# bowang-lab/BioReason

Measured on AMD Instinct MI355X. Metric: GRPO samples/sec (NT-500M+Qwen3-1.7B, DNA 2x1024, prompt 2180, gen 256), higher is better.
Workload: dtype bf16

## Files before the change

### bioreason_amd/csrc/k_gemm.hip

```cpp
#include <type_traits>

#include "bra_device.h"
#include "bra_api_internal.h"

namespace bra {

enum : int {
    EPI_BF16 = 0,
    EPI_F32 = 1,
    EPI_LSE = 2,
    EPI_DLOGIT = 3,
    EPI_ATOMIC = 4,
    EPI_SWIGLU = 5,
};

struct GemmArgs {
    const bf16_t* A;  long lda;
    const bf16_t* B;  long ldb;
    const bf16_t* A2; long lda2;
    const bf16_t* B2; long ldb2;
    void* C;          long ldc;
    int M, N, K, K2;
    float alpha;
    const bf16_t* bias;
    const bf16_t* res;
    long ldres;
    int accumulate;
    int split_k;
    const int* tgt;
    float* part_max;
    float* part_sum;
    float* tgt_logit;
    const float* lse;
    const float* coef;
    int nchunk;
    int swiglu_F;
};

template <int BK>
__device__ __forceinline__ int swz_chunk(int row, int c) {
    return BK == 64 ? (c ^ (row & 7)) : (c ^ ((row >> 2) & 3));
}

#ifdef BRA_EMU
__device__ __forceinline__ void epi_pin(u32x2&) {}
#else
__device__ __forceinline__ void epi_pin(u32x2& v) { asm volatile("" : "+v"(v)); }
#endif
template <bool BIAS>
__device__ __forceinline__ float epi_scale_bias(float a, float alpha, float b) {
    float t = a * alpha;
    if (BIAS) {
#ifndef BRA_EMU
        asm volatile("" : "+v"(t));
#endif
        t = t + b;
    }
    return t;
}
template <int MI, bool BIAS>
__device__ __forceinline__ void epi_bf16_interior_b(const GemmArgs& g, f32x4 (&acc)[4][MI], int mw0, int nw0, int lane) {
    const int fr = lane & 15, fq = lane >> 4;
    const float alpha = g.alpha;
    const int col = nw0 + 4 * fq;
    bf16_t* cp = (bf16_t*)g.C + ((long)(mw0 + fr) * g.ldc + col);
    const long cstep = 16 * g.ldc;
    float bz[4][4];
#pragma unroll
    for (int ni = 0; ni < 4; ++ni)
#pragma unroll
        for (int r = 0; r < 4; ++r) bz[ni][r] = 0.f;
    if (BIAS) {
#pragma unroll
        for (int ni = 0; ni < 4; ++ni) {
            const u32x2 b = ld8(g.bias + col + 16 * ni);
            bz[ni][0] = bf_lo(b.x); bz[ni][1] = bf_hi(b.x); bz[ni][2] = bf_lo(b.y); bz[ni][3] = bf_hi(b.y);
        }
    }
    if (g.res) {
        const bf16_t* rp = g.res + ((long)(mw0 + fr) * g.ldres + col);
        const long rstep = 16 * g.ldres;
        u32x2 rv[MI][4];
#pragma unroll
        for (int mi = 0; mi < MI; ++mi)
#pragma unroll
            for (int ni = 0; ni < 4; ++ni) rv[mi][ni] = ld8(rp + mi * rstep + ni * 16);
#pragma unroll
        for (int mi = 0; mi < MI; ++mi)
#pragma unroll
            for (int ni = 0; ni < 4; ++ni) epi_pin(rv[mi][ni]);
// ... 284 lines not shown
            const bool full = (n + 3 < g.N);
            if (EPI == EPI_BF16 || EPI == EPI_DLOGIT) {
                if (EPI == EPI_BF16) {
                    if (g.bias) {
#pragma unroll
                        for (int r = 0; r < 4; ++r) if (n + r < g.N) v[r] += bf2f(g.bias[n + r]);
                    }
                    if (g.res) {
                        if (full && !(g.ldres & 3)) {
                            const u32x2 rv = ld8(g.res + (long)m * g.ldres + n);
                            v[0] = round_bf(v[0]) + bf_lo(rv.x); v[1] = round_bf(v[1]) + bf_hi(rv.x);
                            v[2] = round_bf(v[2]) + bf_lo(rv.y); v[3] = round_bf(v[3]) + bf_hi(rv.y);
                        } else {
                            for (int r = 0; r < 4; ++r)
                                if (n + r < g.N) v[r] = round_bf(v[r]) + bf2f(g.res[(long)m * g.ldres + n + r]);
                        }
                    }
                } else {
#pragma unroll
                    for (int r = 0; r < 4; ++r) {
                        float p = __expf(round_bf(v[r]) - lse_m);
                        v[r] = coef_m * (((n + r) == tgt_m ? 1.f : 0.f) - p);
                    }
                }
                bf16_t* cp = (bf16_t*)g.C + (long)m * g.ldc + n;
                if (full) {
                    u32x2 o; o.x = pack_bf2(v[0], v[1]); o.y = pack_bf2(v[2], v[3]);
                    st8(cp, o);
                } else {
                    for (int r = 0; r < 4; ++r) if (n + r < g.N) cp[r] = f2bf(v[r]);
                }
            } else if (EPI == EPI_F32) {
                float* cp = (float*)g.C + (long)m * g.ldc + n;
                if (g.bias) {
#pragma unroll
                    for (int r = 0; r < 4; ++r) if (n + r < g.N) v[r] += bf2f(g.bias[n + r]);
                }
                if (full) {
                    f32x4 o = {v[0], v[1], v[2], v[3]};
                    if (g.accumulate) o += *reinterpret_cast<const f32x4*>(cp);
                    *reinterpret_cast<f32x4*>(cp) = o;
                } else {
                    for (int r = 0; r < 4; ++r)
                        if (n + r < g.N) cp[r] = g.accumulate ? cp[r] + v[r] : v[r];
                }
            } else {
                float* cp = (float*)g.C + (long)m * g.ldc + n;
                for (int r = 0; r < 4; ++r) if (n + r < g.N) atomicAdd(cp + r, v[r]);
            }
        }
    }
}

template <int BM, int BK, int EPI, int PF>
__global__ __launch_bounds__(BM * 2) void gemm_nt_kernel(GemmArgs g) {
    constexpr int BN = 128, NT = BM * 2;
    constexpr int CH = BK / 8;
    constexpr int LPTA = (BM * CH) / NT;
    constexpr int LPTB = (BN * CH) / NT;
    constexpr int A_BYTES = BM * BK * 2, B_BYTES = BN * BK * 2, STAGE = A_BYTES + B_BYTES;
    BRA_DYN_SMEM(smem);

    const int tid = (int)threadIdx.x;
    const int lane = tid & 63, wave = tid >> 6;
    const int wm = wave >> 1, wn = wave & 1;

    const int tiles_m = (g.M + BM - 1) / BM, tiles_n = (g.N + BN - 1) / BN;
    const int ntiles = tiles_m * tiles_n;
    int bid = (int)blockIdx.x;
    int kslice = 0;
    if (EPI == EPI_ATOMIC) { kslice = bid / ntiles; bid -= kslice * ntiles; }
    bid = (int)xcd_remap((unsigned)bid, (unsigned)ntiles);
    constexpr int GROUP = 8;
    const int per_group = GROUP * tiles_n;
    const int gid = bid / per_group;
    const int first_m = gid * GROUP;
    const int gsize = (tiles_m - first_m) < GROUP ? (tiles_m - first_m) : GROUP;
    const int tile_m = first_m + (bid % per_group) % gsize;
    const int tile_n = (bid % per_group) / gsize;
    const int m0 = tile_m * BM, n0 = tile_n * BN;

    const int nk1 = g.K / BK, nk2 = g.K2 / BK;
    int kt_begin = 0, kt_end = nk1 + nk2;
    if (EPI == EPI_ATOMIC && g.split_k > 1) {
        int per = (kt_end + g.split_k - 1) / g.split_k;
        kt_begin = kslice * per;
        kt_end = kt_begin + per < kt_end ? kt_begin + per : kt_end;
        if (kt_begin >= kt_end) return;
    }

    u32x4 ra[PF][LPTA], rb[PF][LPTB];

    auto issue_loads = [&](auto S, int kt) {
        constexpr int s = decltype(S)::value;
        const bf16_t* Ap; const bf16_t* Bp; long la, lb; int k0;
        if (kt < nk1) { Ap = g.A; Bp = g.B; la = g.lda; lb = g.ldb; k0 = kt * BK; }
        else { Ap = g.A2; Bp = g.B2; la = g.lda2; lb = g.ldb2; k0 = (kt - nk1) * BK; }
#pragma unroll
        for (int i = 0; i < LPTA; ++i) {
            const int q = tid + NT * i;
            int rm = m0 + q / CH; rm = rm < g.M ? rm : g.M - 1;
            ra[s][i] = ld16(Ap + (long)rm * la + k0 + (q % CH) * 8);
        }
#pragma unroll
        for (int i = 0; i < LPTB; ++i) {
            const int q = tid + NT * i;
            int rn = n0 + q / CH; rn = rn < g.N ? rn : g.N - 1;
            rb[s][i] = ld16(Bp + (long)rn * lb + k0 + (q % CH) * 8);
        }
    };
    auto write_lds = [&](auto S, int buf) {
        constexpr int s = decltype(S)::value;
        char* sa = smem + buf * STAGE;
        char* sb = sa + A_BYTES;
#pragma unroll
        for (int i = 0; i < LPTA; ++i) {
            const int q = tid + NT * i;
            st16(sa + (q / CH) * (BK * 2) + swz_chunk<BK>(q / CH, q % CH) * 16, ra[s][i]);
        }
#pragma unroll
        for (int i = 0; i < LPTB; ++i) {
            const int q = tid + NT * i;
            st16(sb + (q / CH) * (BK * 2) + swz_chunk<BK>(q / CH, q % CH) * 16, rb[s][i]);
        }
    };

    f32x4 acc[4][4];
#pragma unroll
    for (int i = 0; i < 4; ++i)
#pragma unroll
        for (int j = 0; j < 4; ++j) acc[i][j] = f32x4{0.f, 0.f, 0.f, 0.f};

    const int fr = lane & 15, fq = lane >> 4;
    auto compute = [&](int buf) {
        const char* sa = smem + buf * STAGE;
        const char* sb = sa + A_BYTES;
#pragma unroll
        for (int kk = 0; kk < BK / 32; ++kk) {
            u32x4 fa[4], fb[4];
            const int c = kk * 4 + fq;
#pragma unroll
            for (int i = 0; i < 4; ++i) {
                int rowa = wm * 64 + i * 16 + fr;
                int rowb = wn * 64 + i * 16 + fr;
                fa[i] = ld16(sa + rowa * (BK * 2) + swz_chunk<BK>(rowa, c) * 16);
                fb[i] = ld16(sb + rowb * (BK * 2) + swz_chunk<BK>(rowb, c) * 16);
            }
#pragma unroll
            for (int ni = 0; ni < 4; ++ni)
#pragma unroll
                for (int mi = 0; mi < 4; ++mi) acc[ni][mi] = mfma_16x16x32(fb[ni], fa[mi], acc[ni][mi]);
        }
    };
    using S0 = std::integral_constant<int, 0>;
    using S1 = std::integral_constant<int, PF - 1>;
    if (PF == 1) {
        issue_loads(S0{}, kt_begin);
        write_lds(S0{}, 0);
        __syncthreads();
        for (int kt = kt_begin; kt < kt_end; ++kt) {
            const int buf = (kt - kt_begin) & 1;
            const bool more = (kt + 1 < kt_end);
            if (more) issue_loads(S0{}, kt + 1);
            compute(buf);
            if (more) write_lds(S0{}, buf ^ 1);
            __syncthreads();
        }
    } else {
        issue_loads(S0{}, kt_begin);
        if (kt_begin + 1 < kt_end) issue_loads(S1{}, kt_begin + 1);
        write_lds(S0{}, 0);
        __syncthreads();
        for (int kt = kt_begin; kt < kt_end; kt += 2) {
            if (kt + 2 < kt_end) issue_loads(S0{}, kt + 2);
            compute(0);
            if (kt + 1 < kt_end) write_lds(S1{}, 1);
            __syncthreads();
            if (kt + 1 < kt_end) {
                if (kt + 3 < kt_end) issue_loads(S1{}, kt + 3);
                compute(1);
                if (kt + 2 < kt_end) write_lds(S0{}, 0);
                __syncthreads();
            }
        }
    }

    gemm_epilogue<EPI>(g, acc, m0, n0, wm, wn, lane, tile_n);
}

template <int EPI, int SKEW, int MI = 4>
__global__ __launch_bounds__(512, 2) void gemm_glds_kernel(GemmArgs g) {
    constexpr int BM = 64 * MI, BN = 128, BK = 64;
    constexpr int A_BYTES = BM * BK * 2, B_BYTES = BN * BK * 2, STAGE = A_BYTES + B_BYTES;
    BRA_DYN_SMEM(smem);
    const int tid = (int)threadIdx.x;
    const int lane = tid & 63, wave = uniform_i(tid >> 6);
    const int wm = wave >> 1, wn = wave & 1;

    const int tiles_m = (g.M + BM - 1) / BM, tiles_n = (g.N + BN - 1) / BN;
    const int ntiles = tiles_m * tiles_n;
    int bid = (int)blockIdx.x;
    int kslice = 0;
    if (EPI == EPI_ATOMIC) { kslice = bid / ntiles; bid -= kslice * ntiles; }
    bid = (int)xcd_remap((unsigned)bid, (unsigned)ntiles);
    constexpr int GROUP = 8;
    const int per_group = GROUP * tiles_n;
    const int gid = bid / per_group;
    const int first_m = gid * GROUP;
    const int gsize = (tiles_m - first_m) < GROUP ? (tiles_m - first_m) : GROUP;
    const int tile_m = first_m + (bid % per_group) % gsize;
    const int tile_n = (bid % per_group) / gsize;
    const int m0 = tile_m * BM, n0 = tile_n * BN;

    const int nk1 = g.K / BK, nk2 = g.K2 / BK;
    int kt_begin = 0, kt_end = nk1 + nk2;
    if (EPI == EPI_ATOMIC && g.split_k > 1) {
        int per = (kt_end + g.split_k - 1) / g.split_k;
        kt_begin = kslice * per;
        kt_end = kt_begin + per < kt_end ? kt_begin + per : kt_end;
        if (kt_begin >= kt_end) return;
    }
    const int nt = kt_end - kt_begin;

    const int prow = lane >> 3, lchunk = ((lane & 7) ^ (lane >> 3)) * 8;
    int rowA[MI], rowB[2];
#pragma unroll
    for (int j = 0; j < MI; ++j) { int r = m0 + wave * (8 * MI) + j * 8 + prow; rowA[j] = r < g.M ? r : g.M - 1; }
#pragma unroll
    for (int j = 0; j < 2; ++j) { int r = n0 + wave * 16 + j * 8 + prow; rowB[j] = r < g.N ? r : g.N - 1; }
    auto issue = [&](int kt, int stage) {
        char* sa = smem + stage * STAGE + wave * (8 * MI * 128);
        char* sb = smem + stage * STAGE + A_BYTES + wave * (16 * 128);
        const bool main = kt < nk1;
        const bf16_t* Ap = (main ? g.A : g.A2) + (long)(main ? kt : kt - nk1) * BK + lchunk;
        const bf16_t* Bp = (main ? g.B : g.B2) + (long)(main ? kt : kt - nk1) * BK + lchunk;
        const long la = main ? g.lda : g.lda2, lb = main ? g.ldb : g.ldb2;
#pragma unroll
        for (int j = 0; j < MI; ++j) glds16(Ap + (long)rowA[j] * la, sa + j * 1024);
#pragma unroll
        for (int j = 0; j < 2; ++j) glds16(Bp + (long)rowB[j] * lb, sb + j * 1024);
    };
    constexpr int NDMA = MI + 2;

    f32x4 acc[4][MI];
#pragma unroll
    for (int i = 0; i < 4; ++i)
#pragma unroll
        for (int j = 0; j < MI; ++j) acc[i][j] = f32x4{0.f, 0.f, 0.f, 0.f};
    const int fr = lane & 15, fq = lane >> 4;
    auto compute = [&](int stage) {
        const char* sa = smem + stage * STAGE;
        const char* sb = sa + A_BYTES;
#pragma unroll
        for (int kk = 0; kk < BK / 32; ++kk) {
            u32x4 fa[MI], fb[4];
            const int c = kk * 4 + fq;
#pragma unroll
            for (int i = 0; i < MI; ++i) {
                int rowa = wm * (16 * MI) + i * 16 + fr;
                fa[i] = ld16(sa + rowa * 128 + swz_chunk<64>(rowa, c) * 16);
            }
#pragma unroll
            for (int i = 0; i < 4; ++i) {
                int rowb = wn * 64 + i * 16 + fr;
                fb[i] = ld16(sb + rowb * 128 + swz_chunk<64>(rowb, c) * 16);
            }
#pragma unroll
            for (int ni = 0; ni < 4; ++ni)
#pragma unroll
                for (int mi = 0; mi < MI; ++mi) acc[ni][mi] = mfma_16x16x32(fb[ni], fa[mi], acc[ni][mi]);
        }
    };

    issue(kt_begin, 0);
    if (nt > 1) { issue(kt_begin + 1, 1); wait_vmcnt<NDMA>(); } else { wait_vmcnt<0>(); }
    raw_barrier();
    int stage = 0;
    if (!SKEW) {
        for (int t = 0; t < nt; ++t) {
            int s2 = stage + 2; s2 = s2 >= 3 ? s2 - 3 : s2;
            const bool ahead = t + 2 < nt;
            if (ahead) issue(kt_begin + t + 2, s2);
            compute(stage);
            if (ahead) wait_vmcnt<NDMA>(); else wait_vmcnt<0>();
            raw_barrier();
            stage = stage + 1 == 3 ? 0 : stage + 1;
        }
    } else {
        auto read_frags = [&](int stg, int kk, u32x4 (&fa)[MI], u32x4 (&fb)[4]) {
            const char* sa = smem + stg * STAGE;
            const char* sb = sa + A_BYTES;
// ... 125 lines not shown
    int stage = 0;
    u32x4 fa[MI][2], fb0[2][2], fb1[2][2];
    read_a(0, fa);
    read_b(0, 0, fb0);
    for (int t = 0; t < nt; ++t) {
        int s2 = stage + 2; s2 = s2 >= 3 ? s2 - 3 : s2;
        const int s1 = stage + 1 == 3 ? 0 : stage + 1;
        const bool ahead = t + 2 < nt;
        if (ahead) issue(t + 2, s2);
        read_b(stage, 1, fb1);
        mma(0, fa, fb0);
        mma(1, fa, fb1);
        if (ahead) wait_vmcnt<NDMA>(); else wait_vmcnt<0>();
        raw_barrier();
        if (t + 1 < nt) { read_a(s1, fa); read_b(s1, 0, fb0); }
        stage = s1;
    }
    const int mw0 = m0 + wm * (16 * MI), nw0 = n0 + wn * 64;
    float sm[MI];
#pragma unroll
    for (int mi = 0; mi < MI; ++mi) { const int m = mw0 + mi * 16 + fr; sm[mi] = g8.sa[m < g.M ? m : g.M - 1]; }
#pragma unroll
    for (int ni = 0; ni < 4; ++ni) {
        float sn[4];
#pragma unroll
        for (int r = 0; r < 4; ++r) { const int n = nw0 + ni * 16 + 4 * fq + r; sn[r] = g8.sb[n < g.N ? n : g.N - 1]; }
#pragma unroll
        for (int mi = 0; mi < MI; ++mi)
#pragma unroll
            for (int r = 0; r < 4; ++r) acc[ni][mi][r] *= sm[mi] * sn[r];
    }
    gemm_epilogue_w<EPI, MI>(g, acc, mw0, nw0, lane, smem + wave * (16 * MI * EPI_RS));
}

template <int ND, int NR, int NM>
__device__ __forceinline__ void sched_pipe() {
#ifndef BRA_EMU
    static_assert(ND + NR <= NM, "one memory instruction per MFMA gap");
#pragma unroll
    for (int i = 0; i < ND; ++i) {
        __builtin_amdgcn_sched_group_barrier(0x8, 1, 0);
        __builtin_amdgcn_sched_group_barrier(0x20, 1, 0);
        __builtin_amdgcn_sched_group_barrier(0x2, 2, 0);
    }
#pragma unroll
    for (int i = 0; i < NR; ++i) {
        __builtin_amdgcn_sched_group_barrier(0x8, 1, 0);
        __builtin_amdgcn_sched_group_barrier(0x100, 1, 0);
    }
    if constexpr (NM - ND - NR > 0) __builtin_amdgcn_sched_group_barrier(0x8, NM - ND - NR, 0);
#endif
}

template <int EPI, int WM, int WN>
__global__ __launch_bounds__(256) void gemm_w4_kernel(GemmArgs g) {
    static_assert(WN % 4 == 0, "the wave epilogue works on 64-column groups");
    constexpr int BM = 32 * WM, BN = 32 * WN, BK = 64;
    constexpr int A_BYTES = BM * BK * 2, STAGE = (BM + BN) * BK * 2;
    constexpr int NS = (160 * 1024) / STAGE >= 4 ? 4 : 3, LOOK = NS - 1;
    constexpr int NDMA = WM + WN;
    BRA_DYN_SMEM(smem);
    const int tid = (int)threadIdx.x;
    const int lane = tid & 63, wave = uniform_i(tid >> 6);
    const int wm = wave >> 1, wn = wave & 1;

    const int tiles_m = (g.M + BM - 1) / BM, tiles_n = (g.N + BN - 1) / BN;
    const int ntiles = tiles_m * tiles_n;
    int bid = (int)xcd_remap(blockIdx.x, (unsigned)ntiles);
    constexpr int GROUP = 8;
    const int per_group = GROUP * tiles_n;
    const int gid = bid / per_group;
    const int first_m = gid * GROUP;
    const int gsize = (tiles_m - first_m) < GROUP ? (tiles_m - first_m) : GROUP;
    const int tile_m = first_m + (bid % per_group) % gsize;
    const int tile_n = (bid % per_group) / gsize;
    const int m0 = tile_m * BM, n0 = tile_n * BN;

    const int nk1 = g.K / BK, nk2 = g.K2 / BK;
    const int nt = nk1 + nk2;

    const int prow = lane >> 3, lchunk = ((lane & 7) ^ (lane >> 3)) * 8;
    const bf16_t* src[NDMA];
    auto src_init = [&](bool main) {
#pragma unroll
        for (int j = 0; j < NDMA; ++j) {
            const int r = (wave * NDMA + j) * 8 + prow;
            if (r < BM) { int m = m0 + r; m = m < g.M ? m : g.M - 1; src[j] = (main ? g.A : g.A2) + (long)m * (main ? g.lda : g.lda2) + lchunk; }
            else { int n = n0 + r - BM; n = n < g.N ? n : g.N - 1; src[j] = (main ? g.B : g.B2) + (long)n * (main ? g.ldb : g.ldb2) + lchunk; }
        }
    };
    src_init(nk1 > 0);
    auto issue = [&](int kt, int stage) {
        if (kt == nk1 && kt > 0) src_init(false);
        char* dst = smem + stage * STAGE + wave * (NDMA * 1024);
#pragma unroll
        for (int j = 0; j < NDMA; ++j) { glds16(src[j], dst + j * 1024); src[j] += BK; }
    };
    auto wait_tiles = [&](int fly) {
        if (fly >= 2 && LOOK >= 3) wait_vmcnt<2 * NDMA>();
        else if (fly >= 1) wait_vmcnt<NDMA>();
        else wait_vmcnt<0>();
    };

    f32x4 acc[WN][WM];
#pragma unroll
    for (int i = 0; i < WN; ++i)
#pragma unroll
        for (int j = 0; j < WM; ++j) acc[i][j] = f32x4{0.f, 0.f, 0.f, 0.f};
    const int fr = lane & 15, fq = lane >> 4;
    auto read_frags = [&](int stg, int kk, u32x4 (&fa)[WM], u32x4 (&fb)[WN]) {
        const char* sa = smem + stg * STAGE;
        const char* sb = sa + A_BYTES;
        const int c = kk * 4 + fq;
#pragma unroll
        for (int i = 0; i < WM; ++i) {
            const int rowa = wm * (16 * WM) + i * 16 + fr;
            fa[i] = ld16(sa + rowa * 128 + swz_chunk<64>(rowa, c) * 16);
        }
#pragma unroll
        for (int i = 0; i < WN; ++i) {
            const int rowb = wn * (16 * WN) + i * 16 + fr;
            fb[i] = ld16(sb + rowb * 128 + swz_chunk<64>(rowb, c) * 16);
        }
    };
    auto mma = [&](const u32x4 (&fa)[WM], const u32x4 (&fb)[WN]) {
#pragma unroll
        for (int ni = 0; ni < WN; ++ni)
#pragma unroll
            for (int mi = 0; mi < WM; ++mi) acc[ni][mi] = mfma_16x16x32(fb[ni], fa[mi], acc[ni][mi]);
    };

#pragma unroll
    for (int j = 0; j < LOOK; ++j)
        if (j < nt) issue(j, j);
    wait_tiles((nt < LOOK ? nt : LOOK) - 1);
    raw_barrier();
    u32x4 fa0[WM], fb0[WN], fa1[WM], fb1[WN];
    read_frags(0, 0, fa0, fb0);
    int stage = 0;
    auto body = [&](int t, auto ISSUE) {
// ... 17 lines not shown
        sched_fence();
        if (t + 1 < nt) read_frags(s1, 0, fa0, fb0);
        mma(fa1, fb1);
        sched_pipe<0, NDMA, WM * WN>();
        sched_fence();
        stage = s1;
    };
    int t = 0;
    for (; t + LOOK < nt; ++t) body(t, std::true_type{});
    for (; t < nt; ++t) body(t, std::false_type{});
    auto epi_group = [&](auto HC) {
        constexpr int hcol = decltype(HC)::value;
        gemm_epilogue_w<EPI, WM>(g, *reinterpret_cast<f32x4 (*)[4][WM]>(&acc[4 * hcol]), m0 + wm * (16 * WM), n0 + wn * (16 * WN) + 64 * hcol, lane,
                                 smem + wave * (16 * WM * EPI_RS));
    };
    epi_group(std::integral_constant<int, 0>{});
    if constexpr (WN / 4 > 1) epi_group(std::integral_constant<int, 1>{});
    static_assert(WN / 4 <= 2, "two 64-column groups per wave at most");
}

constexpr int SWG_RS = 80;
__device__ __forceinline__ float silu_epi(float x) { return x / (1.f + __expf(-x)); }
__device__ __forceinline__ void ring_epilogue_swiglu(const GemmArgs& g, f32x4 (&acc)[4][8], int mw0, int f0, int lane, char* lw) {
    const int fr = lane & 15, fq = lane >> 4;
    const float alpha = g.alpha;
    char* wp = lw + fr * SWG_RS + 8 * fq;
#pragma unroll
    for (int mi = 0; mi < 8; ++mi)
#pragma unroll
        for (int j = 0; j < 2; ++j) {
            float v[4];
#pragma unroll
            for (int r = 0; r < 4; ++r) {
                const float gb = round_bf(acc[2 * j][mi][r] * alpha), ub = round_bf(acc[2 * j + 1][mi][r] * alpha);
                v[r] = round_bf(silu_epi(gb)) * ub;
            }
            u32x2 o; o.x = pack_bf2(v[0], v[1]); o.y = pack_bf2(v[2], v[3]);
            st8(wp + mi * (16 * SWG_RS) + j * 32, o);
        }
    wave_lds_sync();
    sched_fence();
    const int rrow = lane >> 2, rch = lane & 3;
    const char* rdp = lw + rrow * SWG_RS + 16 * rch;
    bf16_t* cp = (bf16_t*)g.C + ((long)(mw0 + rrow) * g.ldc + f0 + 8 * rch);
    const long cstep = 16 * g.ldc;
    const bool full = mw0 + 128 <= g.M;
#pragma unroll
    for (int jj = 0; jj < 8; ++jj) {
        const u32x4 xv = ld16(rdp + jj * (16 * SWG_RS));
        if (full || mw0 + rrow + 16 * jj < g.M) st16(cp + jj * cstep, xv);
    }
}

template <int EPI, int PH2 = 0>
__global__ __launch_bounds__(512, 2) void gemm_ring_kernel(GemmArgs g) {
    constexpr int BM = 256, BN = 256, BK = 64, HALF = 128 * BK * 2, NSLOT = 10;
    BRA_DYN_SMEM(smem);
    const int tid = (int)threadIdx.x;
    const int lane = tid & 63, wave = uniform_i(tid >> 6);
    const int wr = wave >> 2, wc = wave & 3;

    const int tiles_m = (g.M + BM - 1) / BM, tiles_n = (g.N + BN - 1) / BN;
    const int ntiles = tiles_m * tiles_n;
    int bid = (int)blockIdx.x;
    int kslice = 0;
    if (EPI == EPI_ATOMIC) { kslice = bid / ntiles; bid -= kslice * ntiles; }
    bid = (int)xcd_remap((unsigned)bid, (unsigned)ntiles);
    constexpr int GROUP = 8;
    const int per_group = GROUP * tiles_n;
    const int gid = bid / per_group;
    const int first_m = gid * GROUP;
    const int gsize = (tiles_m - first_m) < GROUP ? (tiles_m - first_m) : GROUP;
    const int tile_m = first_m + (bid % per_group) % gsize;
    const int tile_n = (bid % per_group) / gsize;
    const int m0 = tile_m * BM, n0 = tile_n * BN;

    const int nk1 = g.K / BK, nk2 = g.K2 / BK;
    int kt_begin = 0, kt_end = nk1 + nk2;
    if (EPI == EPI_ATOMIC && g.split_k > 1) {
        int per = (kt_end + g.split_k - 1) / g.split_k;
        kt_begin = kslice * per;
        kt_end = kt_begin + per < kt_end ? kt_begin + per : kt_end;
        if (kt_begin >= kt_end) return;
    }
    const int nt = kt_end - kt_begin;
    const int nstream = 4 * nt;

    const int prow = lane >> 3, lchunk = ((lane & 7) ^ (lane >> 3)) * 8;
    int rowB[4], rowA[4];
#pragma unroll
    for (int i = 0; i < 4; ++i) {
        const int loc = (i >> 1) * 128 + wave * 16 + (i & 1) * 8 + prow;
        int rb = n0 + loc;
        if (EPI == EPI_SWIGLU) rb = tile_n * 128 + (loc >> 5) * 16 + (loc & 15) + ((loc & 16) ? g.swiglu_F : 0);
        rowB[i] = rb < g.N ? rb : g.N - 1;
        int ra = m0 + loc; rowA[i] = ra < g.M ? ra : g.M - 1;
    }
    const bf16_t* src[8];
    auto src_init = [&](int h, int kt) {
        const bool main = kt < nk1;
        const long kcol = (long)(main ? kt : kt - nk1) * BK + lchunk;
#pragma unroll
        for (int pc = 0; pc < 2; ++pc) {
            if (h < 2) src[h * 2 + pc] = (main ? g.B : g.B2) + kcol + (long)rowB[h * 2 + pc] * (main ? g.ldb : g.ldb2);
            else src[h * 2 + pc] = (main ? g.A : g.A2) + kcol + (long)rowA[(h - 2) * 2 + pc] * (main ? g.lda : g.lda2);
        }
    };
#pragma unroll
    for (int h = 0; h < 4; ++h) src_init(h, kt_begin);
    auto issue = [&](int tt, auto H, int slot) {
        constexpr int h = decltype(H)::value;
        if (tt >= nt) return;
        if (kt_begin + tt == nk1 && tt > 0) src_init(h, nk1);
        char* dst = smem + slot * HALF + wave * 2048;
        glds16(src[h * 2], dst);
        glds16(src[h * 2 + 1], dst + 1024);
        src[h * 2] += BK;
        src[h * 2 + 1] += BK;
    };
    auto wrap = [&](int sl) { return sl >= NSLOT ? sl - NSLOT : sl; };
    auto wait_phase = [&](int gph) {
        const int fly = nstream - 5 - gph;
        if (fly >= 3) wait_vmcnt<6>(); else if (fly == 2) wait_vmcnt<4>(); else if (fly == 1) wait_vmcnt<2>(); else wait_vmcnt<0>();
    };

    f32x4 acc[4][8];
#pragma unroll
    for (int i = 0; i < 4; ++i)
#pragma unroll
        for (int j = 0; j < 8; ++j) acc[i][j] = f32x4{0.f, 0.f, 0.f, 0.f};
    const int fr = lane & 15, fq = lane >> 4;
    const int sw0 = ((fq ^ (fr & 7)) * 16), sw1 = (((4 + fq) ^ (fr & 7)) * 16);
    const int offA = fr * 128;
    const int offB = ((wc & 1) * 64 + fr) * 128;
    u32x4 fa[4][2], fb[2][2][2];
    auto read_a = [&](int slotA, int s) {
        const char* base = smem + slotA * HALF + offA + s * (64 * 128);
#pragma unroll
        for (int i = 0; i < 4; ++i) { fa[i][0] = ld16(base + i * 2048 + sw0); fa[i][1] = ld16(base + i * 2048 + sw1); }
    };
    auto read_b = [&](int slotB, auto S) {
        constexpr int s = decltype(S)::value;
        const char* base = smem + slotB * HALF + offB + s * (32 * 128);
#pragma unroll
        for (int i = 0; i < 2; ++i) { fb[s][i][0] = ld16(base + i * 2048 + sw0); fb[s][i][1] = ld16(base + i * 2048 + sw1); }
    };
    auto mma = [&](auto SA, auto SB) {
        constexpr int sa = decltype(SA)::value, sb = decltype(SB)::value;
        setprio(1);
#pragma unroll
        for (int kk = 0; kk < 2; ++kk)
#pragma unroll
            for (int ib = 0; ib < 2; ++ib)
#pragma unroll
                for (int ia = 0; ia < 4; ++ia)
                    acc[sb * 2 + ib][sa * 4 + ia] = mfma_16x16x32(fb[sb][ib][kk], fa[ia][kk], acc[sb * 2 + ib][sa * 4 + ia]);
        setprio(0);
    };
// ... 20 lines not shown
            issue(t + 1, I2{}, wrap(rb2 + 6)); issue(t + 1, I3{}, wrap(rb2 + 7)); wait2(gp); ++gp;
            sched_fence(); bare_barrier(); wait_lds(); sched_fence();
            mma(I0{}, I0{}); mma(I0{}, I1{});
            sched_fence(); bare_barrier();
            read_a(sA, 1);
            issue(t + 2, I0{}, wrap(rb2 + 8)); issue(t + 2, I1{}, wrap(rb2 + 9)); wait2(gp); ++gp;
            sched_fence(); bare_barrier(); wait_lds(); sched_fence();
            mma(I1{}, I1{}); mma(I1{}, I0{});
            sched_fence(); bare_barrier();
            rb2 = rb2 + 4 >= NSLOT ? rb2 + 4 - NSLOT : rb2 + 4;
        }
        if (wr == 0) bare_barrier();
        if constexpr (EPI == EPI_SWIGLU) ring_epilogue_swiglu(g, acc, m0 + wr * 128, tile_n * 128 + wc * 32, lane, smem + wave * (128 * SWG_RS));
        else gemm_epilogue_w<EPI, 8>(g, acc, m0 + wr * 128, n0 + wc * 64, lane, smem + wave * (128 * EPI_RS));
        return;
    }
    issue(0, I0{}, 0); issue(0, I1{}, 1); issue(0, I2{}, 2); issue(0, I3{}, 3);
    issue(1, I0{}, 4); issue(1, I1{}, 5); issue(1, I2{}, 6);
    wait_phase(-1);
    bare_barrier();
    if (wr == 1) bare_barrier();
    int rbase = 0;
    int gph = 0;
#pragma unroll 1
    for (int t = 0; t < nt; ++t) {
        const int sB = wrap(rbase + (wc >> 1)), sA = wrap(rbase + 2 + wr);
        read_b(sB, I0{}); sched_fence(); read_a(sA, 0);
        issue(t + 1, I3{}, wrap(rbase + 7)); wait_phase(gph); ++gph;
        sched_fence(); bare_barrier(); wait_lds(); sched_fence();
        mma(I0{}, I0{});
        sched_fence(); bare_barrier();
        read_b(sB, I1{});
        issue(t + 2, I0{}, wrap(rbase + 8)); wait_phase(gph); ++gph;
        sched_fence(); bare_barrier(); wait_lds(); sched_fence();
        mma(I0{}, I1{});
        sched_fence(); bare_barrier();
        read_a(sA, 1);
        issue(t + 2, I1{}, wrap(rbase + 9)); wait_phase(gph); ++gph;
        sched_fence(); bare_barrier(); wait_lds(); sched_fence();
        mma(I1{}, I1{});
        sched_fence(); bare_barrier();
        issue(t + 2, I2{}, rbase); wait_phase(gph); ++gph;
        sched_fence(); bare_barrier(); sched_fence();
        mma(I1{}, I0{});
        sched_fence(); bare_barrier();
        rbase = rbase + 4 >= NSLOT ? rbase + 4 - NSLOT : rbase + 4;
    }
    if (wr == 0) bare_barrier();

    if constexpr (EPI == EPI_SWIGLU) ring_epilogue_swiglu(g, acc, m0 + wr * 128, tile_n * 128 + wc * 32, lane, smem + wave * (128 * SWG_RS));
    else gemm_epilogue_w<EPI, 8>(g, acc, m0 + wr * 128, n0 + wc * 64, lane, smem + wave * (128 * EPI_RS));
}

template <int OUTF32>
__global__ __launch_bounds__(256) void gemm_skinny_kernel(GemmArgs g) {
    __shared__ float red[4][64][4];
    const int tid = (int)threadIdx.x, lane = tid & 63, wave = tid >> 6;
    const int fr = lane & 15, fq = lane >> 4;
    const int n0 = (int)blockIdx.x * 16;
    int rn = n0 + fr; rn = rn < g.N ? rn : g.N - 1;
    int rm = fr < g.M ? fr : g.M - 1;
    f32x4 acc = {0.f, 0.f, 0.f, 0.f};
    {
        const bf16_t* wp = g.B + (long)rn * g.ldb + fq * 8;
        const bf16_t* xp = g.A + (long)rm * g.lda + fq * 8;
        const int nk = g.K / 32;
        int kt = wave;
        for (; kt + 28 < nk; kt += 32) {
            u32x4 w[8], x[8];
#pragma unroll
            for (int u = 0; u < 8; ++u) { w[u] = ld16(wp + (long)(kt + 4 * u) * 32); x[u] = ld16(xp + (long)(kt + 4 * u) * 32); }
#pragma unroll
            for (int u = 0; u < 8; ++u) acc = mfma_16x16x32(w[u], x[u], acc);
        }
        for (; kt < nk; kt += 4) acc = mfma_16x16x32(ld16(wp + (long)kt * 32), ld16(xp + (long)kt * 32), acc);
    }
    if (g.K2 > 0) {
        const bf16_t* wp = g.B2 + (long)rn * g.ldb2 + fq * 8;
        const bf16_t* xp = g.A2 + (long)rm * g.lda2 + fq * 8;
        const int nk = g.K2 / 32;
        for (int kt = wave; kt < nk; kt += 4) acc = mfma_16x16x32(ld16(wp + (long)kt * 32), ld16(xp + (long)kt * 32), acc);
    }
#pragma unroll
    for (int r = 0; r < 4; ++r) red[wave][lane][r] = acc[r];
    __syncthreads();
    if (wave != 0) return;
    float v[4];
#pragma unroll
    for (int r = 0; r < 4; ++r) v[r] = (red[0][lane][r] + red[1][lane][r] + red[2][lane][r] + red[3][lane][r]) * g.alpha;
    const int m = fr, n = n0 + 4 * fq;
    if (m >= g.M || n >= g.N) return;
    if (g.bias) {
#pragma unroll
        for (int r = 0; r < 4; ++r) if (n + r < g.N) v[r] += bf2f(g.bias[n + r]);
    }
    if (OUTF32) {
        float* cp = (float*)g.C + (long)m * g.ldc + n;
        for (int r = 0; r < 4; ++r) if (n + r < g.N) cp[r] = g.accumulate ? cp[r] + v[r] : v[r];
    } else {
        if (g.res) {
#pragma unroll
            for (int r = 0; r < 4; ++r) if (n + r < g.N) v[r] = round_bf(v[r]) + bf2f(g.res[(long)m * g.ldres + n + r]);
        }
        bf16_t* cp = (bf16_t*)g.C + (long)m * g.ldc + n;
        if (n + 3 < g.N) { u32x2 o; o.x = pack_bf2(v[0], v[1]); o.y = pack_bf2(v[2], v[3]); st8(cp, o); }
        else for (int r = 0; r < 4; ++r) if (n + r < g.N) cp[r] = f2bf(v[r]);
    }
}

static int launch_skinny(const GemmArgs& g, int out_f32, bra_stream_t stream) {
    const int grid = (g.N + 15) / 16;
    if (out_f32) BRA_LAUNCH((gemm_skinny_kernel<1>), dim3(grid), dim3(256), 0, stream, g);
    else BRA_LAUNCH((gemm_skinny_kernel<0>), dim3(grid), dim3(256), 0, stream, g);
    return BRA_LAUNCH_STATUS();
}

#ifdef BRA_EMU
template <typename T> struct knob_t { T v; explicit knob_t(T x) : v(x) {} operator T() const { return v; } knob_t& operator=(T x) { v = x; return *this; } };
#else
template <typename T> struct knob_t {
    std::atomic<T> v;
    explicit knob_t(T x) : v(x) {}
    operator T() const { return v.load(std::memory_order_relaxed); }
    knob_t& operator=(T x) { v.store(x, std::memory_order_relaxed); return *this; }
};
#endif
static knob_t<int> g_forced_variant(-1);
static knob_t<int> g_forced_w4(0);
static knob_t<int> ring_min_fill_pct(60);
static knob_t<int> ring_two_phase(1);
static knob_t<int> ring_row_split(1);

static int pick_variant(const GemmArgs& g) {
    { const int fv = g_forced_variant; if (fv >= 0) return fv >= 6 ? 6 : fv; }
    const long tiles256 = (long)((g.M + 255) / 256) * ((g.N + 127) / 128) * (g.split_k > 1 ? g.split_k : 1);
    if (g.K % 64 == 0 && g.K2 % 64 == 0 && g.split_k <= 1) {
        const long t = (long)((g.M + 255) / 256) * ((g.N + 255) / 256);
        const long rounds = (t + 255) / 256;
        if (t >= 140 && (t <= 256 || 100 * t >= ring_min_fill_pct * rounds * 256)) return 6;
    }
    if (g.K % 64 == 0 && g.K2 % 64 == 0 && tiles256 >= 128) return 5;
    const long tiles128 = (long)((g.M + 127) / 128) * ((g.N + 127) / 128) * (g.split_k > 1 ? g.split_k : 1);
    if (g.K % 64 == 0 && g.K2 % 64 == 0 && tiles128 >= 128) return 5;
    return 0;
}

template <int BM, int BK, int EPI, int PF>
static int launch_gemm_v(const GemmArgs& g, bra_stream_t stream) {
    const int tiles = ((g.M + BM - 1) / BM) * ((g.N + 127) / 128);
    int grid = tiles;
    if (EPI == EPI_ATOMIC) grid = tiles * (g.split_k > 0 ? g.split_k : 1);
    const size_t smem = 2 * (size_t)(BM + 128) * BK * 2;
    BRA_ALLOW_SMEM((gemm_nt_kernel<BM, BK, EPI, PF>), smem);
    BRA_LAUNCH((gemm_nt_kernel<BM, BK, EPI, PF>), dim3(grid), dim3(BM * 2), smem, stream, g);
    return BRA_LAUNCH_STATUS();
}

static knob_t<int> g_forced_glds_rows(0);
static int pick_glds_rows(const GemmArgs& g) {
    { const int fr = g_forced_glds_rows; if (fr) return fr; }
    if (g_forced_variant >= 0) return 256;
    const long tn = (g.N + 127) / 128, sk = g.split_k > 1 ? g.split_k : 1;
    const int bms[3] = {256, 192, 128};
    const double eff[3] = {1.0, 0.95, 0.86};
    int best = 256;
    double best_cost = 1e30;
    for (int i = 0; i < 3; ++i) {
        const long t = ((g.M + bms[i] - 1) / bms[i]) * tn * sk;
        const double cost = (double)((t + 255) / 256) * bms[i] / eff[i];
        if (cost < best_cost * 0.97) { best_cost = cost; best = bms[i]; }
    }
    return best;
}

template <int EPI, int MI>
static int launch_glds_mi(const GemmArgs& g, bra_stream_t stream, bool skew) {
    constexpr int BM = 64 * MI;
    const int tiles = ((g.M + BM - 1) / BM) * ((g.N + 127) / 128);
    int grid = tiles;
    if (EPI == EPI_ATOMIC) grid = tiles * (g.split_k > 0 ? g.split_k : 1);
    const size_t smem = 3 * (size_t)(BM + 128) * 64 * 2;
    if (skew) {
        BRA_ALLOW_SMEM((gemm_glds_kernel<EPI, 1, MI>), smem);
        BRA_LAUNCH((gemm_glds_kernel<EPI, 1, MI>), dim3(grid), dim3(512), smem, stream, g);
    } else {
        BRA_ALLOW_SMEM((gemm_glds_kernel<EPI, 0, MI>), smem);
        BRA_LAUNCH((gemm_glds_kernel<EPI, 0, MI>), dim3(grid), dim3(512), smem, stream, g);
    }
    return BRA_LAUNCH_STATUS();
}

template <int EPI>
static int launch_glds(const GemmArgs& g, bra_stream_t stream) {
    const bool skew = pick_variant(g) >= 5;
    const int rows = pick_glds_rows(g);
    if (rows == 128) return launch_glds_mi<EPI, 2>(g, stream, skew);
    if (rows == 192) return launch_glds_mi<EPI, 3>(g, stream, skew);
    return launch_glds_mi<EPI, 4>(g, stream, skew);
}

static knob_t<int> g_w4_auto(1);
static int pick_w4(const GemmArgs& g) {
    { const int f = g_forced_w4; if (f) return f; }
    if (!g_w4_auto || g_forced_variant >= 0 || g_forced_glds_rows) return 0;
    if (g.K % 64 || g.K2 % 64 || g.split_k > 1 || g.M < 128 || g.N < 128 || g.K + g.K2 < 256) return 0;
    if ((long)((g.M + 255) / 256) * ((g.N + 255) / 256) > 256) return 0;
    struct Cand { int bm, bn; double rate; int w4; };
    static const Cand cands[8] = {{256, 256, 5.9, 0}, {256, 128, 4.27, 0}, {192, 128, 4.56, 0}, {128, 128, 3.75, 0},
                                  {160, 256, 4.5, 1}, {128, 256, 4.5, 2}, {160, 128, 4.5, 3}, {128, 128, 4.5, 4}};
    const double kk = 2.0e-6 * (double)(g.K + g.K2);
    int best = 0;
    double best_t = 1e30;
    for (const Cand& c : cands) {
        const long tiles = (long)((g.M + c.bm - 1) / c.bm) * ((g.N + c.bn - 1) / c.bn);
        const double t = (double)((tiles + 255) / 256) * (kk * c.bm * c.bn / c.rate + 3.5);
        if (t < best_t) { best_t = t; best = c.w4; }
    }
    return best;
}

template <int EPI, int WM, int WN>
static int launch_w4_t(const GemmArgs& g, bra_stream_t stream) {
    constexpr int BM = 32 * WM, BN = 32 * WN, STAGE = (BM + BN) * 128, NS = (160 * 1024) / STAGE >= 4 ? 4 : 3;
    const int tiles = ((g.M + BM - 1) / BM) * ((g.N + BN - 1) / BN);
    const size_t smem = (size_t)NS * STAGE;
    BRA_ALLOW_SMEM((gemm_w4_kernel<EPI, WM, WN>), smem);
    BRA_LAUNCH((gemm_w4_kernel<EPI, WM, WN>), dim3(tiles), dim3(256), smem, stream, g);
    return BRA_LAUNCH_STATUS();
}
template <int EPI>
static int launch_w4(const GemmArgs& g, bra_stream_t stream, int cfg) {
    if constexpr (EPI == EPI_BF16 || EPI == EPI_F32) {
        switch (cfg) {
            case 1: return launch_w4_t<EPI, 5, 8>(g, stream);
            case 2: return launch_w4_t<EPI, 4, 8>(g, stream);
            case 3: return launch_w4_t<EPI, 5, 4>(g, stream);
            default: return launch_w4_t<EPI, 4, 4>(g, stream);
        }
    }
    return BRA_ERR_UNSUPPORTED;
}

template <int EPI>
static int launch_ring(const GemmArgs& g, bra_stream_t stream) {
    const int tiles = ((g.M + 255) / 256) * ((g.N + 255) / 256);
    const size_t smem = 10 * (size_t)128 * 64 * 2;
    if (ring_two_phase) {
        BRA_ALLOW_SMEM((gemm_ring_kernel<EPI, 1>), smem);
        BRA_LAUNCH((gemm_ring_kernel<EPI, 1>), dim3(tiles), dim3(512), smem, stream, g);
    } else {
        BRA_ALLOW_SMEM((gemm_ring_kernel<EPI, 0>), smem);
        BRA_LAUNCH((gemm_ring_kernel<EPI, 0>), dim3(tiles), dim3(512), smem, stream, g);
    }
    return BRA_LAUNCH_STATUS();
}

template <int BK, int EPI>
static int launch_gemm(const GemmArgs& g, bra_stream_t stream) {
    if (BK == 64 && (EPI == EPI_BF16 || EPI == EPI_F32)) { const int w4 = pick_w4(g); if (w4) return launch_w4<EPI>(g, stream, w4); }
    if (BK == 64 && EPI != EPI_ATOMIC && pick_variant(g) == 6) return launch_ring<EPI>(g, stream);
    if (BK == 64 && pick_variant(g) >= 4) return launch_glds<EPI>(g, stream);
    switch (pick_variant(g)) {
        case 1: return launch_gemm_v<128, BK, EPI, 2>(g, stream);
        case 2: return launch_gemm_v<256, BK, EPI, 1>(g, stream);
        case 3: return launch_gemm_v<256, BK, EPI, 2>(g, stream);
        default: return launch_gemm_v<128, BK, EPI, 1>(g, stream);
    }
}

static int ring_split_rows(const GemmArgs& g) {
    if (g_forced_variant >= 0 || !ring_row_split || g.K % 64 || g.K2 % 64 || g.split_k > 1) return 0;
    if (pick_variant(g) != 6 || pick_w4(g)) return 0;
    const long tm = (g.M + 255) / 256, tn = (g.N + 255) / 256, t = tm * tn;
    const long R = t / 256, rem = t - R * 256;
    if (R < 1 || rem == 0 || 2 * rem >= 256) return 0;
    const long rm = (R * 256) / tn;
    if (rm <= 0 || rm >= tm) return 0;
    const long rows2 = g.M - rm * 256;
    const long halves = ((rows2 + 255) / 256) * ((g.N + 127) / 128);
    if (halves < 32) return 0;
    if ((long)g.N * (g.K + g.K2) < 6l * 1024 * 1024) return 0;
    const double cost_split = (double)R + 0.55 * (double)((halves + 255) / 256);
    return cost_split < (double)(R + 1) - 0.15 ? (int)(rm * 256) : 0;
}

template <int EPI>
static int dispatch_bk(const GemmArgs& g, bra_stream_t stream) {
    if (EPI == EPI_BF16 || EPI == EPI_F32) {
        const int m1 = ring_split_rows(g);
        if (m1 > 0) {
            GemmArgs g1 = g, g2 = g;
            g1.M = m1;
            g2.M = g.M - m1;
            g2.A = g.A + (long)m1 * g.lda;
            if (g.A2) g2.A2 = g.A2 + (long)m1 * g.lda2;
            g2.C = EPI == EPI_F32 ? (void*)((float*)g.C + (long)m1 * g.ldc) : (void*)((bf16_t*)g.C + (long)m1 * g.ldc);
            if (g.res) g2.res = g.res + (long)m1 * g.ldres;
            const int e = launch_ring<EPI>(g1, stream);
            if (e) return e;
            return launch_glds<EPI>(g2, stream);
        }
    }
    if (g.K % 64 == 0 && g.K2 % 64 == 0) return launch_gemm<64, EPI>(g, stream);
    return launch_gemm<32, EPI>(g, stream);
}

static int check_common(const GemmArgs& g) {
    if (g.M <= 0 || g.N <= 0) return BRA_ERR_ARG;
    if (g.K < 0 || g.K2 < 0 || (g.K + g.K2) <= 0) return BRA_ERR_ARG;
    if (g.K % 32 || g.K2 % 32) return BRA_ERR_ARG;
    if (g.K && (g.lda % 8 || g.ldb % 8 || !g.A || !g.B)) return BRA_ERR_ARG;
    if (g.K2 && (g.lda2 % 8 || g.ldb2 % 8 || !g.A2 || !g.B2)) return BRA_ERR_ARG;
    return 0;
}

}

using namespace bra;

#ifdef BRA_DEBUG
extern "C" int bra_gemm_set_variant(int v) {
    bra::g_forced_glds_rows = 0;
    bra::g_forced_w4 = 0;
    bra::g_w4_auto = v == -2 ? 0 : 1;
    if (v == -2) v = -1;
    if (v >= 11 && v <= 14) { bra::g_forced_w4 = v - 10; v = 5; }
    if (v == 9 || v == 10) { bra::g_forced_glds_rows = v == 9 ? 192 : 128; v = 5; }
    bra::g_forced_variant = v;
    if (v == 6) bra::ring_two_phase = 0;
    if (v == 7 || v < 0) bra::ring_two_phase = 1;
    return 0;
}
extern "C" int bra_gemm_set_glds_rows(int rows) {
    if (rows != 0 && rows != 128 && rows != 192 && rows != 256) return BRA_ERR_ARG;
    bra::g_forced_glds_rows = rows;
    return 0;
}
extern "C" int bra_gemm_set_ring_fill(int pct) { bra::ring_min_fill_pct = pct; return 0; }
extern "C" int bra_gemm_set_epi_lds(int on) {
#ifndef BRA_EMU
    return (int)hipMemcpyToSymbol(HIP_SYMBOL(bra::epi_via_lds), &on, sizeof(int));
#else
    (void)on;
    return 0;
#endif
}
extern "C" int bra_gemm_set_row_split(int on) { bra::ring_row_split = on; return 0; }
#endif

extern "C" int bra_gemm_bf16_nt(const void* A, long lda, const void* B, long ldb, const void* A2, long lda2,
                                const void* B2, long ldb2, int K2, void* C, long ldc, int M, int N, int K,
                                float alpha, const void* bias, const void* res, long ldres, int out_f32,
                                int accumulate, void* stream) {
    GemmArgs g = {};
    g.A = (const bf16_t*)A; g.lda = lda; g.B = (const bf16_t*)B; g.ldb = ldb;
    g.A2 = (const bf16_t*)A2; g.lda2 = lda2; g.B2 = (const bf16_t*)B2; g.ldb2 = ldb2;
    g.C = C; g.ldc = ldc; g.M = M; g.N = N; g.K = K; g.K2 = K2; g.alpha = alpha;
    g.bias = (const bf16_t*)bias; g.res = (const bf16_t*)res; g.ldres = ldres; g.accumulate = accumulate;
    if (M == 0 || N == 0) return 0;
    int e = check_common(g);
    if (e) return e;
    if (!C || ldc % 4) return BRA_ERR_ARG;
    if (out_f32 && res) return BRA_ERR_ARG;
    if (M <= 16) return launch_skinny(g, out_f32, (bra_stream_t)stream);
    if (out_f32) return dispatch_bk<EPI_F32>(g, (bra_stream_t)stream);
    return dispatch_bk<EPI_BF16>(g, (bra_stream_t)stream);
}

extern "C" int bra_gemm_fp8_nt(const void* A8, long lda, const float* sa, const void* B8, long ldb, const float* sb, void* C, long ldc,
                               int M, int N, int K, const void* res, long ldres, int out_f32, void* stream) {
    if (M == 0 || N == 0) return 0;
    if (M < 0 || N < 0 || K <= 0 || K % 128 || !A8 || !B8 || !sa || !sb || !C || lda % 16 || ldb % 16 || ldc % 4) return BRA_ERR_ARG;
    if (out_f32 && res) return BRA_ERR_ARG;
    Gemm8Args g8 = {};
    g8.A = (const unsigned char*)A8; g8.lda = lda; g8.B = (const unsigned char*)B8; g8.ldb = ldb; g8.sa = sa; g8.sb = sb; g8.K = K;
    g8.e.C = C; g8.e.ldc = ldc; g8.e.M = M; g8.e.N = N; g8.e.K = K; g8.e.alpha = 1.f; g8.e.res = (const bf16_t*)res; g8.e.ldres = ldres;
    const int rows = pick_glds_rows(g8.e);
    bra_stream_t st = (bra_stream_t)stream;
#define BRA_G8(EPI_, MI_)                                                                                             \
    do {                                                                                                              \
        constexpr int BM_ = 64 * MI_;                                                                                 \
        const int tiles = ((M + BM_ - 1) / BM_) * ((N + 127) / 128);                                                  \
        const size_t smem = 3 * (size_t)(BM_ + 128) * 128;                                                            \
        BRA_ALLOW_SMEM((gemm_fp8_kernel<EPI_, MI_>), smem);                                                           \
        BRA_LAUNCH((gemm_fp8_kernel<EPI_, MI_>), dim3(tiles), dim3(512), smem, st, g8);                                \
        return BRA_LAUNCH_STATUS();                                                                                   \
    } while (0)
    if (out_f32) { if (rows == 128) BRA_G8(EPI_F32, 2); if (rows == 192) BRA_G8(EPI_F32, 3); BRA_G8(EPI_F32, 4); }
    if (rows == 128) BRA_G8(EPI_BF16, 2);
    if (rows == 192) BRA_G8(EPI_BF16, 3);
    BRA_G8(EPI_BF16, 4);
#undef BRA_G8
}

extern "C" int bra_gemm_swiglu_bf16_nt(const void* A, long lda, const void* W, long ldw, const void* A2, long lda2, const void* B2, long ldb2,
                                       int K2, void* C, long ldc, int M, int F, int K, float alpha, void* stream) {
    if (M == 0 || F == 0) return 0;
    GemmArgs g = {};
    g.A = (const bf16_t*)A; g.lda = lda; g.B = (const bf16_t*)W; g.ldb = ldw;
    g.A2 = (const bf16_t*)A2; g.lda2 = lda2; g.B2 = (const bf16_t*)B2; g.ldb2 = ldb2;
    g.C = C; g.ldc = ldc; g.M = M; g.N = 2 * F; g.K = K; g.K2 = K2; g.alpha = alpha; g.swiglu_F = F;
    int e = check_common(g);
    if (e) return e;
    if (!C || ldc % 8 || ((size_t)C & 15)) return BRA_ERR_ARG;
    if (K % 64 || K2 % 64 || F % 128 || M <= 16) return BRA_ERR_UNSUPPORTED;
    return launch_ring<EPI_SWIGLU>(g, (bra_stream_t)stream);
}

extern "C" int bra_gemm_bf16_nt_splitk(const void* A, long lda, const void* B, long ldb, void* C, long ldc, int M,
                                       int N, int K, float alpha, int split_k, void* stream) {
    GemmArgs g = {};
    g.A = (const bf16_t*)A; g.lda = lda; g.B = (const bf16_t*)B; g.ldb = ldb;
    g.C = C; g.ldc = ldc; g.M = M; g.N = N; g.K = K; g.alpha = alpha; g.split_k = split_k < 1 ? 1 : split_k;
    if (M == 0 || N == 0) return 0;
    int e = check_common(g);
    if (e) return e;
    if (!C) return BRA_ERR_ARG;
    return dispatch_bk<EPI_ATOMIC>(g, (bra_stream_t)stream);
}

extern "C" int bra_lmhead_lse_partials(const void* H, long ldh, const void* E, long lde, int M, int V, int K,
                                       const int* tgt, float* part_max, float* part_sum, float* tgt_logit,
                                       void* stream) {
    GemmArgs g = {};
    g.A = (const bf16_t*)H; g.lda = ldh; g.B = (const bf16_t*)E; g.ldb = lde;
    g.M = M; g.N = V; g.K = K; g.alpha = 1.f;
    g.tgt = tgt; g.part_max = part_max; g.part_sum = part_sum; g.tgt_logit = tgt_logit;
    g.nchunk = (V + 63) / 64;
    if (M == 0) return 0;
    int e = check_common(g);
    if (e) return e;
    if (!tgt || !part_max || !part_sum || !tgt_logit) return BRA_ERR_ARG;
    return dispatch_bk<EPI_LSE>(g, (bra_stream_t)stream);
}

extern "C" int bra_lmhead_dlogits(const void* H, long ldh, const void* E, long lde, int M, int V, int K,
                                  const int* tgt, const float* lse, const float* coef, void* dlogits, long ldd,
                                  void* stream) {
    GemmArgs g = {};
    g.A = (const bf16_t*)H; g.lda = ldh; g.B = (const bf16_t*)E; g.ldb = lde;
    g.C = dlogits; g.ldc = ldd; g.M = M; g.N = V; g.K = K; g.alpha = 1.f;
    g.tgt = tgt; g.lse = lse; g.coef = coef;
    if (M == 0) return 0;
    int e = check_common(g);
    if (e) return e;
    if (!tgt || !lse || !coef || !dlogits || ldd % 4) return BRA_ERR_ARG;
    return dispatch_bk<EPI_DLOGIT>(g, (bra_stream_t)stream);
}
```

### bioreason_amd/csrc/k_lora.hip

```cpp
#include "bra_device.h"
#include "bra_api_internal.h"
#include "bra_lora_plan.h"

namespace bra {

struct LoraDownArgs {
    const bf16_t* x; long ldx;
    const bf16_t* A; long lda;
    bf16_t* t; long ldt;
    int M, K, R;
    float alpha;
    DropCfg d;
    int nb_live;
    int steps_per;
    float* part;
};

template <int RB, int NL, int TR = 32, int NT = NL>
__global__ __launch_bounds__(256) void lora_down_drop_kernel(LoraDownArgs g) {
    static_assert(TR == 8 || TR == 16 || TR == 32 || TR == 64 || TR == 128, "adapter ranks with dropout");
    static_assert(NL == (NT * TR + 31) / 32 && NL <= RB && NT <= 4, "live blocks = the blocks the targets cover");
    constexpr int KS = 128, XP = KS + 8;
    constexpr int XS_ELEMS = 2 * 32 * XP, AS_ELEMS = 2 * 32 * NL * XP;
    constexpr int RED_BYTES = 3 * NL * 64 * 16 * 4, STAGE_BYTES = (XS_ELEMS + AS_ELEMS) * 2;
    __shared__ __attribute__((aligned(16))) char lds[STAGE_BYTES > RED_BYTES ? STAGE_BYTES : RED_BYTES];
    bf16_t* xs = reinterpret_cast<bf16_t*>(lds);
    bf16_t* as = xs + XS_ELEMS;
    float* red = reinterpret_cast<float*>(lds);
    const int tid = (int)threadIdx.x, lane = tid & 63, wave = tid >> 6, h = lane >> 5;
    const int m0 = (int)blockIdx.x * 32;
    const int nstep = (g.K + KS - 1) / KS;
    const u32x4 zero4 = {0u, 0u, 0u, 0u};
    u32x4 rx[2], ra[2 * NL];
    auto issue = [&](int s) {
#pragma unroll
        for (int i = 0; i < 2; ++i) {
            const int c = tid + 256 * i, row = c >> 4, k = KS * s + 8 * (c & 15);
            int m = m0 + row; m = m < g.M ? m : g.M - 1;
            rx[i] = ld16(g.x + (long)m * g.ldx + (k < g.K ? k : 0));
        }
#pragma unroll
        for (int i = 0; i < 2 * NL; ++i) {
            const int c = tid + 256 * i, row = c >> 4, k = KS * s + 8 * (c & 15);
            ra[i] = ld16(g.A + (long)(row < g.R ? row : g.R - 1) * g.lda + (k < g.K ? k : 0));
        }
    };
    auto commit = [&](int buf, int s) {
#pragma unroll
        for (int i = 0; i < 2; ++i) {
            const int c = tid + 256 * i, k = KS * s + 8 * (c & 15);
            st16(&xs[buf * 32 * XP + (c >> 4) * XP + 8 * (c & 15)], k < g.K ? rx[i] : zero4);
        }
#pragma unroll
        for (int i = 0; i < 2 * NL; ++i) {
            const int c = tid + 256 * i, row = c >> 4, k = KS * s + 8 * (c & 15);
            st16(&as[buf * 32 * NL * XP + (c >> 4) * XP + 8 * (c & 15)], (k < g.K && row < g.R) ? ra[i] : zero4);
        }
    };
    f32x16 acc[NL];
#pragma unroll
    for (int rb = 0; rb < NL; ++rb)
#pragma unroll
        for (int q = 0; q < 16; ++q) acc[rb][q] = 0.f;
    const int s_lo = (int)blockIdx.y * g.steps_per;
    const int s_hi = s_lo + g.steps_per < nstep ? s_lo + g.steps_per : nstep;
    issue(s_lo); commit(s_lo & 1, s_lo);
    __syncthreads();
    const int mrow = m0 + (lane & 31);
    for (int s = s_lo; s < s_hi; ++s) {
        const int buf = s & 1;
        issue(s + 1 < s_hi ? s + 1 : s);
        sched_fence();
        const int lrow = opaque_i(lane & 31);
#pragma unroll
        for (int k2 = 0; k2 < 2; ++k2) {
            const int kk = 2 * wave + k2;
            const u32x4 xf = ld16(&xs[buf * 32 * XP + lrow * XP + 16 * kk + 8 * h]);
            const uint32_t e0 = (uint32_t)mrow * (uint32_t)g.K + (uint32_t)(KS * s + 16 * kk + 8 * h);
            if constexpr (TR == 32) {
#pragma unroll
                for (int rb = 0; rb < NL; ++rb) {
                    const u32x4 af = drop_apply8(xf, g.d.seed[rb], e0, g.d.thr16, g.d.inv_keep);
                    const u32x4 bf = ld16(&as[buf * 32 * NL * XP + (32 * rb + lrow) * XP + 16 * kk + 8 * h]);
                    acc[rb] = mfma_32x32x16(af, bf, acc[rb]);
                }
            } else if constexpr (TR > 32) {
#pragma unroll
                for (int jt = 0; jt < NT; ++jt) {
                    const u32x4 af = drop_apply8(xf, g.d.seed[jt], e0, g.d.thr16, g.d.inv_keep);
#pragma unroll
                    for (int b = 0; b < TR / 32; ++b) {
                        const int rb = jt * (TR / 32) + b;
                        const u32x4 bf = ld16(&as[buf * 32 * NL * XP + (32 * rb + lrow) * XP + 16 * kk + 8 * h]);
                        acc[rb] = mfma_32x32x16(af, bf, acc[rb]);
                    }
                }
            } else {
#pragma unroll
                for (int jt = 0; jt < NT; ++jt) {
                    const int rb = jt * TR / 32;
                    const u32x4 af = drop_apply8(xf, g.d.seed[jt], e0, g.d.thr16, g.d.inv_keep);
                    const u32x4 bf = ld16(&as[buf * 32 * NL * XP + (32 * rb + lrow) * XP + 16 * kk + 8 * h]);
                    acc[rb] = mfma_32x32x16(af, lrow / TR == jt % (32 / TR) ? bf : zero4, acc[rb]);
                }
            }
        }
        if (s + 1 < s_hi) commit(buf ^ 1, s + 1);
        __syncthreads();
    }
    if (wave != 0) {
#pragma unroll
        for (int rb = 0; rb < NL; ++rb)
#pragma unroll
            for (int q = 0; q < 16; ++q) red[(((wave - 1) * NL + rb) * 64 + lane) * 16 + q] = acc[rb][q];
    }
    __syncthreads();
    if (wave != 0) return;
    float* const pbase = g.part ? g.part + ((long)blockIdx.y * g.M + m0 + 4 * h) * g.R + (lane & 31) : nullptr;
    bf16_t* const tbase = g.t ? g.t + (long)(m0 + 4 * h) * g.ldt + (lane & 31) : nullptr;
#pragma unroll
    for (int rb = 0; rb < RB; ++rb) {
        const int r = 32 * rb + (lane & 31);
#pragma unroll
        for (int q = 0; q < 16; ++q) {
            const int mq = (q & 3) + 8 * (q >> 2);
            const int m = m0 + mq + 4 * h;
            float v = 0.f;
            if (rb < NL) {
                v = acc[rb < NL ? rb : 0][q];
#pragma unroll
                for (int w = 0; w < 3; ++w) v += red[((w * NL + (rb < NL ? rb : 0)) * 64 + lane) * 16 + q];
            }
            if (m < g.M && r < g.R) {
                if (g.part) pbase[(long)mq * g.R + 32 * rb] = v;
                else tbase[(long)mq * g.ldt + 32 * rb] = f2bf(g.alpha * v);
            }
        }
    }
}

__global__ __launch_bounds__(256) void lora_partial_reduce_kernel(const float* part, int ks, long MR, int R, float alpha, bf16_t* t, long ldt) {
    const long i4 = ((long)blockIdx.x * 256 + threadIdx.x) * 4;
    if (i4 >= MR) return;
    float a0 = 0.f, a1 = 0.f, a2 = 0.f, a3 = 0.f;
    for (int k = 0; k < ks; ++k) {
        const f32x4 v = *reinterpret_cast<const f32x4*>(part + (long)k * MR + i4);
        a0 += v[0]; a1 += v[1]; a2 += v[2]; a3 += v[3];
    }
    const long m = i4 / R;
    const int r = (int)(i4 - m * R);
    bf16_t* o = t + m * ldt + r;
    o[0] = f2bf(alpha * a0); o[1] = f2bf(alpha * a1); o[2] = f2bf(alpha * a2); o[3] = f2bf(alpha * a3);
}

struct LoraUpArgs {
    const bf16_t* dts; long ldd;
    const bf16_t* AT; long ldat;
    bf16_t* out; long ldo;
    int M, K, R;
    int k_chunk;
    DropCfg d;
    int nb_live;
};

template <int RB, int NL, int TR = 32, int NT = NL>
__global__ __launch_bounds__(256) void lora_up_drop_kernel(LoraUpArgs g) {
    constexpr int NC = TR == 32 ? 2 * NL : (NT * TR + 15) / 16;
    const u32x4 zero4 = {0u, 0u, 0u, 0u};
    const int lane = lane_id(), wave = (int)threadIdx.x >> 6, h = lane >> 5;
    const int m_base = ((int)blockIdx.x * 4 + wave) * 32;
    if (m_base >= g.M) return;
    int mr = m_base + (lane & 31); mr = mr < g.M ? mr : g.M - 1;
    u32x4 df[NC];
#pragma unroll
    for (int c = 0; c < NC; ++c) df[c] = ld16(g.dts + (long)mr * g.ldd + 16 * c + 8 * h);
    uint32_t rowbase[8];
    {
        const uint32_t odd0 = (uint32_t)lane & 1u;
#pragma unroll
        for (int i = 0; i < 8; ++i) {
            const int q = (int)(8 * odd0) + i;
            rowbase[i] = (uint32_t)(m_base + (q & 3) + 8 * (q >> 2) + 4 * h) * (uint32_t)g.K;
        }
    }
    const int k_lo = (int)blockIdx.y * g.k_chunk;
// ... 32 lines not shown
                hh[i] = odd ? other : mine;
                hh[8 + i] = odd ? mine : other;
            }
#pragma unroll
            for (int q = 0; q < 16; ++q) o[q] += ((hh[q] >> fsh) & 0x7fffu) >= g.d.thr16 ? acc[q] : 0.f;
        }
        const int side = ((k0 - k_lo) >> 5) & 1;
#pragma unroll
        for (int q = 0; q < 16; ++q)
            sw[((q & 3) + 8 * (q >> 2) + 4 * h) * UP_SP + 32 * side + (lane & 31)] = kc < g.K ? f2bf(o[q] * g.d.inv_keep) : (bf16_t)0;
        if (side == 1 || k0 + 32 >= k_hi) {
            wave_lds_sync();
            const int kf = k0 - 32 * side;
            const int ncol = 32 * (side + 1);
#pragma unroll
            for (int j = 0; j < 4; ++j) {
                const int row = 8 * j + (lane >> 3), c8 = 8 * (lane & 7);
                const int m = m_base + row;
                const u32x4 v = ld16(&sw[row * UP_SP + c8]);
                if (m < g.M && c8 < ncol) {
                    bf16_t* op = g.out + (long)m * g.ldo + kf + c8;
                    if (vec_ok && kf + c8 + 8 <= g.K) st16(op, v);
                    else {
                        const bf16_t* e = reinterpret_cast<const bf16_t*>(&v);
                        for (int i = 0; i < 8; ++i) if (kf + c8 + i < g.K) op[i] = e[i];
                    }
                }
            }
            wave_lds_sync();
        }
    }
}

__global__ __launch_bounds__(256) void dropout_mask_kernel(uint8_t* out, long n, uint32_t seed, uint32_t thr16) {
    for (long i = (long)blockIdx.x * 256 + threadIdx.x; i < n; i += (long)gridDim.x * 256)
        out[i] = drop_keep1(seed, (uint32_t)i, thr16) ? 1 : 0;
}

}

using namespace bra;

extern "C" int bra_lora_down_splitk_plan(int M, int K) {
    const int gx = (M + 31) / 32, nstep = (K + 127) / 128;
    if (gx >= 192) return nstep >= 32 ? 4 : 1;
    if (gx <= 0 || nstep < 6) return 1;
    int want = 512 / gx, cap = nstep / 3;
    int ks = want < cap ? want : cap;
    if (ks < 2) return 1;
    const int per = (nstep + ks - 1) / ks;
    return (nstep + per - 1) / per;
}

extern "C" int bra_lora_down_drop(const void* x, long ldx, const void* A, long lda, void* t, long ldt, int M, int K, int R,
                                  float alpha, float p, unsigned s0, unsigned s1, unsigned s2, unsigned s3, int r, int nt,
                                  float* part, int ksplit, void* stream) {
    if (M == 0) return 0;
    if (!x || !A || !t || M < 0 || K <= 0 || K % 8 || ldx % 8 || lda % 8 || !lora_drop_ok(p, M, K, r, nt, R)) return BRA_ERR_ARG;
    if (ksplit <= 1) part = nullptr;
    else if (!part || ksplit > (K + 127) / 128 || ldt % 4) return BRA_ERR_ARG;
    const unsigned seeds[4] = {s0, s1, s2, s3};
    const int nstep = (K + 127) / 128;
    const int per = part ? (nstep + ksplit - 1) / ksplit : nstep;
    const int ny = part ? (nstep + per - 1) / per : 1;
    const dim3 grid((M + 31) / 32, ny);
    bra_stream_t st = (bra_stream_t)stream;
    return lora_for_slices(r, nt, R, [&](const LoraSlice& s) {
        float* const ps = part ? part + (long)ksplit * M * s.c0 : nullptr;
        bf16_t* const ts = (bf16_t*)t + s.c0;
        LoraDownArgs g = {(const bf16_t*)x, ldx, (const bf16_t*)A + (long)s.c0 * lda, lda, ts, ldt, M, K, s.Rs, alpha,
                          make_cfg(p, seeds + s.j0, s.nts), 0, per, ps};
#define BRA_LD(C_, RB_, NL_, TR_, NT_) if (C_) BRA_LAUNCH((lora_down_drop_kernel<RB_, NL_, TR_, NT_>), grid, dim3(256), 0, st, g); else
        BRA_LORA_ROWS(BRA_LD) return BRA_ERR_ARG;
#undef BRA_LD
        if (part) {
            const long MR = (long)M * s.Rs;
            BRA_LAUNCH(lora_partial_reduce_kernel, dim3((unsigned)((MR / 4 + 255) / 256)), dim3(256), 0, st, (const float*)ps, ny, MR, s.Rs,
                       alpha, ts, ldt);
        }
        return BRA_LAUNCH_STATUS();
    });
}

extern "C" int bra_lora_up_drop(const void* dts, long ldd, const void* AT, long ldat, void* out, long ldo, int M, int K, int R,
                                float p, unsigned s0, unsigned s1, unsigned s2, unsigned s3, int r, int nt, void* stream) {
    if (M == 0) return 0;
    if (!dts || !AT || !out || M < 0 || K <= 0 || ldd % 8 || ldat % 8 || !lora_drop_ok(p, M, K, r, nt, R)) return BRA_ERR_ARG;
    const int mblk = (M + 127) / 128;
    int splits = (1024 + mblk - 1) / mblk;
    int k_chunk = ((K + splits - 1) / splits + 31) / 32 * 32;
    k_chunk = k_chunk < 128 ? 128 : k_chunk;
    const unsigned seeds[4] = {s0, s1, s2, s3};
    LoraUpArgs g = {(const bf16_t*)dts, ldd, (const bf16_t*)AT, ldat, (bf16_t*)out, ldo, M, K, R, k_chunk, make_cfg(p, seeds, nt), 0};
    const dim3 grid(mblk, (K + k_chunk - 1) / k_chunk);
    bra_stream_t st = (bra_stream_t)stream;
#define BRA_LU(RB_, NL_, TR_, NT_) BRA_LAUNCH((lora_up_drop_kernel<RB_, NL_, TR_, NT_>), grid, dim3(256), 0, st, g)
#define BRA_LUR(TR_, NT_) BRA_LU((NT_ * TR_ + 63) / 64 * 2, (NT_ * TR_ + 31) / 32, TR_, NT_)
#define BRA_LUR3(TR_) do { if (nt == 1) BRA_LUR(TR_, 1); else if (nt == 2) BRA_LUR(TR_, 2); else BRA_LUR(TR_, 3); } while (0)
    if (r == 32 && R == 32) BRA_LU(1, 1, 32, 1);
    else if (r == 32 && R == 64) { if (nt == 1) BRA_LU(2, 1, 32, 1); else BRA_LU(2, 2, 32, 2); }
    else if (r == 32 && nt == 3) BRA_LU(4, 3, 32, 3);
    else if (r == 32) BRA_LU(4, 4, 32, 4);
    else if (r == 8) BRA_LUR3(8);
    else if (r == 16) BRA_LUR3(16);
    else if (r == 64) BRA_LUR3(64);
    else BRA_LUR3(128);
#undef BRA_LUR3
#undef BRA_LUR
#undef BRA_LU
    return BRA_LAUNCH_STATUS();
}

extern "C" int bra_dropout_mask(void* out, int M, int K, float p, unsigned seed, void* stream) {
    if (M <= 0 || K <= 0) return 0;
    if (!out || !(p >= 0.f && p < 1.f) || (long)M * K >= (1l << 32)) return BRA_ERR_ARG;
    const long n = (long)M * K;
    long grid = (n + 255) / 256; grid = grid > 4096 ? 4096 : grid;
    BRA_LAUNCH(dropout_mask_kernel, dim3((unsigned)grid), dim3(256), 0, (bra_stream_t)stream, (uint8_t*)out, n, (uint32_t)seed,
               drop_threshold(p));
    return BRA_LAUNCH_STATUS();
}
```

### bioreason_amd/engine.py

```python
from __future__ import annotations

import math
from dataclasses import dataclass, field
from typing import Dict, List, Optional, Tuple

import torch

from . import ops
from .arena import TrainableArena

BF16 = torch.bfloat16


def rope_tables(npos: int, hd: int, theta: float, device, round_bf16: bool = True) -> Tuple[torch.Tensor, torch.Tensor]:
    inv = 1.0 / (theta ** (torch.arange(0, hd, 2, dtype=torch.float32) / hd))
    fr = torch.arange(npos, dtype=torch.float32)[:, None] * inv[None, :]
    c, s = fr.cos(), fr.sin()
    if round_bf16:
        c, s = c.to(BF16).float(), s.to(BF16).float()
    return c.contiguous().to(device), s.contiguous().to(device)


class LoraGroup:

# ... 15 lines not shown
        am, bm = a.mask_view(self.key + ".A"), a.mask_view(self.key + ".B")
        off = 0
        active = getattr(self, "active", None)
        for j, n in enumerate(self.n_sizes):
            if active is None or active[j]:
                am[j * self.r:(j + 1) * self.r, :] = 1
                bm[off:off + n, j * self.r:(j + 1) * self.r] = 1
            off += n
        self.A = torch.zeros(self.r_pad, self.K, dtype=BF16, device=dev)
        self.AT = torch.zeros(self.K, self.r_pad, dtype=BF16, device=dev)
        self.B = torch.zeros(self.N, self.r_pad, dtype=BF16, device=dev)
        self.BT = torch.zeros(self.r_pad, self.N, dtype=BF16, device=dev)
        a.register_pack(self.A_master, self.A, False)
        a.register_pack(self.A_master, self.AT, True)
        a.register_pack(self.B_master, self.B, False)
        a.register_pack(self.B_master, self.BT, True)
        for fn in self.on_views:
            fn()

    def target_views(self, j: int):
        off = sum(self.n_sizes[:j])
        n = self.n_sizes[j]
        rs = slice(j * self.r, (j + 1) * self.r)
        return (self.A_master[rs, :], self.B_master[off:off + n, rs], self.A_grad[rs, :], self.B_grad[off:off + n, rs])


@dataclass
class QwenLayerW:
    ln1: torch.Tensor = None
    ln2: torch.Tensor = None
    qn: torch.Tensor = None
    kn: torch.Tensor = None
    Wqkv: torch.Tensor = None
    Wo: torch.Tensor = None
    Wgu: torch.Tensor = None
    Wd: torch.Tensor = None
    WqkvT: torch.Tensor = None
    WoT: torch.Tensor = None
    WguT: torch.Tensor = None
    WdT: torch.Tensor = None
    lora: Dict[str, Optional[LoraGroup]] = field(default_factory=lambda: {"qkv": None, "o": None, "gu": None, "d": None})


@dataclass
class SeqMeta:
    B: int
    S: int
    pos: torch.Tensor
    kmask: Optional[torch.Tensor]
    lora_on: bool = True
    max_pos: int = 0
    drop_p: float = 0.0
    drop_seed: int = 0


def _mix32(a: int, b: int) -> int:
    h = (a * 0x9E3779B1 + b * 0x85EBCA6B + 0x165667B1) & 0xFFFFFFFF
    h ^= h >> 15
    h = (h * 0x2C1B3C6D) & 0xFFFFFFFF
    h ^= h >> 12
    h = (h * 0x297A2D39) & 0xFFFFFFFF
    h ^= h >> 15
    return h


import contextlib as _contextlib
import os as _os
FUSE_SWIGLU = _os.environ.get("BRA_FUSE_SWIGLU", "1") == "1"

_nullctx = _contextlib.nullcontext

LORA_GROUP_INDEX = {"qkv": 0, "o": 1, "gu": 2, "d": 3}


def lora_drop_seeds(pass_seed: int, layer: int, group: str, n_targets: int):
    base = (layer * 4 + LORA_GROUP_INDEX[group]) * 4
    return [_mix32(pass_seed, base + j) for j in range(n_targets)]


class QwenEngine:
    def __init__(self, cfg, device):
        self.cfg = cfg
        self.device = device
        self.H = cfg.hidden_size
        self.Hq, self.Hkv, self.hd = cfg.num_attention_heads, cfg.num_key_value_heads, cfg.head_dim
        self.F = cfg.intermediate_size
        self.L = cfg.num_hidden_layers
        self.V = cfg.vocab_size
        self.eps = cfg.rms_norm_eps
        self.Nq, self.Nkv = self.Hq * self.hd, self.Hkv * self.hd
        self.scale = self.hd ** -0.5
        self.layers: List[QwenLayerW] = [QwenLayerW() for _ in range(self.L)]
        self.norm_w: torch.Tensor = None
        self.E: torch.Tensor = None
        self.ET: Optional[torch.Tensor] = None
        self._rope = None
        self._rope_len = 0
        self.layer_done_hook = None

    def rope(self, npos: int):
        if self._rope is None or self._rope_len < npos:
            n = max(npos, 512)
            theta = self.cfg.rope_parameters["rope_theta"] if hasattr(self.cfg, "rope_parameters") else self.cfg.rope_theta
            self._rope = rope_tables(n, self.hd, theta, self.device)
            self._rope_len = n
        return self._rope

    def ensure_transposed(self):
        for L in self.layers:
            if L.WqkvT is None:
                L.WqkvT = ops.transpose2d(L.Wqkv)
                L.WoT = ops.transpose2d(L.Wo)
                L.WguT = ops.transpose2d(L.Wgu)
                L.WdT = ops.transpose2d(L.Wd)
        if self.ET is None:
            self.ET = ops.transpose2d(self.E)

    SMALL_M = 8192

    @staticmethod
    def _down(x2d, A, scaling, live_rows):
        if x2d.shape[0] < QwenEngine.SMALL_M and A.shape[0] in (32, 64, 128):
            return ops.lora_down_drop(x2d, A, scaling, 0.0, [0] * min(A.shape[0] // 32, (live_rows + 31) // 32), rank=32)
        return ops.gemm_nt(x2d, A, alpha=scaling)

    @staticmethod
    def _lora_fwd(x2d, W, G: Optional[LoraGroup], on: bool, res=None, out=None, drop=None):
        if G is not None and on:
            if drop is not None:
                t = ops.lora_down_drop(x2d, G.A, G.scaling, drop[0], drop[1], drop[2])
            else:
                t = QwenEngine._down(x2d, G.A, G.scaling, len(G.n_sizes) * G.r)
            return ops.gemm_nt(x2d, W, a2=t, b2=G.B, res=res, out=out), t
        return ops.gemm_nt(x2d, W, res=res, out=out), None

    @staticmethod
    def _lora_bwd(dy, WT, G: Optional[LoraGroup], on: bool, x2d, t, drop=None):
        if G is not None and on:
            dts = QwenEngine._down(dy, G.BT, G.scaling, len(G.n_sizes) * G.r)
            if drop is not None:
                dxl = ops.lora_up_drop(dts, G.AT, drop[0], drop[1], drop[2])
                dx = ops.gemm_nt(dy, WT, res=dxl)
            else:
                dx = ops.gemm_nt(dy, WT, a2=dts, b2=G.AT)
            ops.wgrad_tn(dy, t, G.B_grad)
            ops.wgrad_tn(x2d, dts, G.A_grad, transposed_out=True, drop=drop[:2] if drop is not None else None,
                         rank=drop[2] if drop is not None else 32)
            return dx
        return ops.gemm_nt(dy, WT)

    def _drop(self, m: "SeqMeta", li: int, group: str):
        G = self.layers[li].lora[group]
        if G is None or not m.lora_on or m.drop_p <= 0.0:
            return None
        if G.r not in ops.LORA_DROP_RANKS:
            raise NotImplementedError(f"LoRA dropout needs an adapter rank in {list(ops.LORA_DROP_RANKS)} (one mask stream per target "
                                      f"module, built for these ranks), not r = {G.r}")
        return (m.drop_p, lora_drop_seeds(m.drop_seed, li, group, len(G.n_sizes)), G.r)

    def use_fp8(self, W8):
        eng = self

        class _Ctx:
            def __enter__(self_):
                self_.prev = getattr(eng, "_fp8", None)
                eng._fp8 = W8

            def __exit__(self_, *a):
                eng._fp8 = self_.prev
        return _Ctx()

    def fp8_supported(self) -> bool:
        return self.H % 128 == 0 and self.F % 128 == 0 and self.Nq % 128 == 0

    def fp8_weight_images(self, merged=None):
        out = []
        for li, L in enumerate(self.layers):
            W = merged[li] if merged is not None else {"Wqkv": L.Wqkv, "Wo": L.Wo, "Wgu": L.Wgu, "Wd": L.Wd}
            out.append({"Wqkv": ops.quant_rows_fp8(W["Wqkv"], colw=L.ln1), "Wo": ops.quant_rows_fp8(W["Wo"]),
                        "Wgu": ops.quant_rows_fp8(W["Wgu"], colw=L.ln2), "Wd": ops.quant_rows_fp8(W["Wd"])})
        return out

    def _layer_fwd_fp8(self, li: int, x: torch.Tensor, m: SeqMeta, kv_out, R):
        L = self.layers[li]
        B, S, T = m.B, m.S, m.B * m.S
        cosT, sinT = self.rope(m.max_pos or m.S)
        xq, xs = ops.quant_rows_fp8(x, rms_eps=self.eps)
        qkv = ops.gemm_fp8_nt(xq, xs, R["Wqkv"][0], R["Wqkv"][1])
        q = torch.empty((B, S, self.Hq, self.hd), dtype=BF16, device=x.device)
        if kv_out is None:
            k = torch.empty((B, S, self.Hkv, self.hd), dtype=BF16, device=x.device)
            v = torch.empty((B, S, self.Hkv, self.hd), dtype=BF16, device=x.device)
            s_off = 0
        else:
            kc, vc, s_off = kv_out[:3]
            k, v = kc.permute(0, 2, 1, 3), vc.permute(0, 2, 1, 3)
        ops.qk_norm_rope_fwd(qkv, L.qn, L.kn, cosT, sinT, m.pos, S, self.Hq, self.Hkv, self.hd, self.eps, 1.0, q, k, v, s_off)
        if kv_out is not None:
            k, v = k[:, :s_off + S], v[:, :s_off + S]
        vt = ops.head_transpose(v)
        if kv_out is not None and len(kv_out) > 3 and kv_out[3] is not None:
            kv_out[3].append(vt)
        o, _ = ops.attn_fwd(q, k, vt, m.kmask, True, self.scale, need_lse=False)
        oq, os_ = ops.quant_rows_fp8(o.view(T, self.Nq))
        h = ops.gemm_fp8_nt(oq, os_, R["Wo"][0], R["Wo"][1], res=x)
        hq, hs = ops.quant_rows_fp8(h, rms_eps=self.eps)
        gu = ops.gemm_fp8_nt(hq, hs, R["Wgu"][0], R["Wgu"][1])
        aq, as_ = ops.swiglu_quant_fp8(gu)
        return ops.gemm_fp8_nt(aq, as_, R["Wd"][0], R["Wd"][1], res=h)

    def layer_fwd(self, li: int, x: torch.Tensor, m: SeqMeta, save: bool, kv_out=None):
        w8 = getattr(self, "_fp8", None)
        if w8 is not None and not save:
            return self._layer_fwd_fp8(li, x, m, kv_out, w8[li]), None
        L = self.layers[li]
        B, S, T = m.B, m.S, m.B * m.S
        cosT, sinT = self.rope(m.max_pos or m.S)
        xn = ops.rmsnorm_fwd(x, L.ln1, self.eps)
        qkv, t1 = self._lora_fwd(xn, L.Wqkv, L.lora["qkv"], m.lora_on, drop=self._drop(m, li, "qkv"))
        q = torch.empty((B, S, self.Hq, self.hd), dtype=BF16, device=x.device)
        if kv_out is None:
            k = torch.empty((B, S, self.Hkv, self.hd), dtype=BF16, device=x.device)
            v = torch.empty((B, S, self.Hkv, self.hd), dtype=BF16, device=x.device)
            s_off = 0
        else:
            kc, vc, s_off = kv_out[:3]
            k, v = kc.permute(0, 2, 1, 3), vc.permute(0, 2, 1, 3)
        ops.qk_norm_rope_fwd(qkv, L.qn, L.kn, cosT, sinT, m.pos, S, self.Hq, self.Hkv, self.hd, self.eps, 1.0, q, k, v, s_off)
        if kv_out is not None:
            k, v = k[:, :s_off + S], v[:, :s_off + S]
        vt = ops.head_transpose(v)
        if kv_out is not None and len(kv_out) > 3 and kv_out[3] is not None:
            kv_out[3].append(vt)
        o, lse = ops.attn_fwd(q, k, vt, m.kmask, True, self.scale, need_lse=save)
        o2 = o.view(T, self.Nq)
        h, t2 = self._lora_fwd(o2, L.Wo, L.lora["o"], m.lora_on, res=x, drop=self._drop(m, li, "o"))
        hn = ops.rmsnorm_fwd(h, L.ln2, self.eps)
        gu = t3 = act = None
        if not save and FUSE_SWIGLU:
            G3, d3 = L.lora["gu"], self._drop(m, li, "gu")
            if G3 is not None and m.lora_on:
                t3 = ops.lora_down_drop(hn, G3.A, G3.scaling, d3[0], d3[1], d3[2]) if d3 is not None else self._down(hn, G3.A, G3.scaling, len(G3.n_sizes) * G3.r)
                act = ops.gemm_swiglu(hn, L.Wgu, a2=t3, b2=G3.B)
            else:
                act = ops.gemm_swiglu(hn, L.Wgu)
        if act is None:
            if t3 is not None:
                gu = ops.gemm_nt(hn, L.Wgu, a2=t3, b2=L.lora["gu"].B)
            else:
                gu, t3 = self._lora_fwd(hn, L.Wgu, L.lora["gu"], m.lora_on, drop=self._drop(m, li, "gu"))
            act = ops.swiglu_fwd(gu)
        y, t4 = self._lora_fwd(act, L.Wd, L.lora["d"], m.lora_on, res=h, drop=self._drop(m, li, "d"))
        saved = (x, xn, t1, qkv, q, k, v, o, lse, t2, h, hn, t3, gu, act, t4) if save else None
        return y, saved

    def layer_bwd(self, li: int, dy: torch.Tensor, saved, m: SeqMeta, prefix: int = 0, extra_dkv=None):
        L = self.layers[li]
        (x, xn, t1, qkv, q, k, v, o, lse, t2, h, hn, t3, gu, act, t4) = saved
        B, S, T = m.B, m.S, m.B * m.S
        cosT, sinT = self.rope(m.max_pos or m.S)
        on = m.lora_on
        dact = self._lora_bwd(dy, L.WdT, L.lora["d"], on, act, t4, drop=self._drop(m, li, "d"))
        dgu = ops.swiglu_bwd(gu, dact)
        dhn = self._lora_bwd(dgu, L.WguT, L.lora["gu"], on, hn, t3, drop=self._drop(m, li, "gu"))
        dh = ops.rmsnorm_bwd(dhn, h, L.ln2, self.eps, dres=dy)
        do = self._lora_bwd(dh, L.WoT, L.lora["o"], on, o.view(T, self.Nq), t2, drop=self._drop(m, li, "o"))
        dq, dk, dv = ops.attn_bwd(q, k, v, o, do.view(B, S, self.Hq, self.hd), lse, m.kmask, True, self.scale)
        pre = None
        if prefix > 0:
            pre = (dk[:, :prefix], dv[:, :prefix])
            dk, dv = dk[:, prefix:], dv[:, prefix:]
        if extra_dkv is not None:
            dk = ops.group_sum(extra_dkv[0], extra_dkv[2], add=dk)
            dv = ops.group_sum(extra_dkv[1], extra_dkv[2], add=dv)
        dqkv = ops.qk_norm_rope_bwd(qkv, L.qn, L.kn, cosT, sinT, m.pos, S, self.Hq, self.Hkv, self.hd, self.eps, 1.0, dq, dk, dv)
        dxn = self._lora_bwd(dqkv, L.WqkvT, L.lora["qkv"], on, xn, t1, drop=self._drop(m, li, "qkv"))
        dx = ops.rmsnorm_bwd(dxn, x, L.ln1, self.eps, dres=dh)
        return (dx, pre) if prefix > 0 else dx

    def forward_hidden(self, x: torch.Tensor, m: SeqMeta, save: bool):
        tape = []
        for li in range(self.L):
            x, saved = self.layer_fwd(li, x, m, save)
            tape.append(saved)
        hid = ops.rmsnorm_fwd(x, self.norm_w, self.eps)
        return hid, (tape, x) if save else None

    def backward_hidden(self, dhid: torch.Tensor, tape_x, m: SeqMeta):
        tape, xlast = tape_x
        dx = ops.rmsnorm_bwd(dhid, xlast, self.norm_w, self.eps)
        for li in reversed(range(self.L)):
            dx = self.layer_bwd(li, dx, tape[li], m)
            tape[li] = None
            if self.layer_done_hook is not None:
                self.layer_done_hook(li)
        return dx


    def forward_hidden_shared(self, xp: torch.Tensor, mp: SeqMeta, xc: torch.Tensor, mc: SeqMeta, copies: int, save: bool, side=None):
        R, P, B, C = mp.B, mp.S, mc.B, mc.S
        assert B == R * copies
        dev = xp.device
        tape_p, tape_c = [], []
        main = torch.cuda.current_stream(dev) if side is not None else None
        if side is not None:
            side.wait_stream(main)
            xc.record_stream(side)
        for li in range(self.L):
            kc_r = torch.empty((R, self.Hkv, P, self.hd), dtype=BF16, device=dev)
            vc_r = torch.empty((R, self.Hkv, P, self.hd), dtype=BF16, device=dev)
            xp, sp = self.layer_fwd(li, xp, mp, save, kv_out=(kc_r, vc_r, 0))
            tape_p.append(sp)
            if side is not None:
                ev = torch.cuda.Event()
                ev.record(main)
                kc_r.record_stream(side)
                vc_r.record_stream(side)
            with (torch.cuda.stream(side) if side is not None else _nullctx()):
                if side is not None:
                    side.wait_event(ev)
                kc = torch.empty((B, self.Hkv, P + C, self.hd), dtype=BF16, device=dev)
                vc = torch.empty((B, self.Hkv, P + C, self.hd), dtype=BF16, device=dev)
                ops.group_broadcast(kc_r, kc, copies)
                ops.group_broadcast(vc_r, vc, copies)
                xc, sc = self.layer_fwd(li, xc, mc, save, kv_out=(kc, vc, P))
                tape_c.append(sc)
        last = torch.arange(R, device=dev, dtype=torch.int32) * P + (P - 1)
        xp_last = ops.gather_rows(last, xp)
        hid_last = ops.rmsnorm_fwd(xp_last, self.norm_w, self.eps)
        with (torch.cuda.stream(side) if side is not None else _nullctx()):
            hid_c = ops.rmsnorm_fwd(xc, self.norm_w, self.eps)
        if side is not None:
            main.wait_stream(side)
            for t_ in (hid_c, xc):
                t_.record_stream(main)
        return hid_last, hid_c, ((tape_p, tape_c, xp_last, xc, last) if save else None)

    def backward_hidden_shared(self, dhid_last: torch.Tensor, dhid_c: torch.Tensor, tape, mp: SeqMeta, mc: SeqMeta, copies: int, side=None):
        tape_p, tape_c, xp_last, xc, last = tape
        dev = dhid_c.device
        main = torch.cuda.current_stream(dev) if side is not None else None
        if side is not None:
            side.wait_stream(main)
            dhid_c.record_stream(side)
        with (torch.cuda.stream(side) if side is not None else _nullctx()):
            dxc = ops.rmsnorm_bwd(dhid_c, xc, self.norm_w, self.eps)
        dxp = ops.scatter_rows(last, ops.rmsnorm_bwd(dhid_last, xp_last, self.norm_w, self.eps), mp.B * mp.S)
        for li in reversed(range(self.L)):
            with (torch.cuda.stream(side) if side is not None else _nullctx()):
                dxc, pre = self.layer_bwd(li, dxc, tape_c[li], mc, prefix=mp.S)
                tape_c[li] = None
                if side is not None:
                    ev = torch.cuda.Event()
                    ev.record(side)
            if side is not None:
                main.wait_event(ev)
                pre[0].record_stream(main)
                pre[1].record_stream(main)
            dxp = self.layer_bwd(li, dxp, tape_p[li], mp, extra_dkv=(pre[0], pre[1], copies))
            tape_p[li] = None
            if self.layer_done_hook is not None:
                self.layer_done_hook(li)
        if side is not None:
            main.wait_stream(side)
            dxc.record_stream(main)
        return dxp, dxc


@dataclass
class EsmLayerW:
    ln1_w: torch.Tensor = None
    ln1_b: torch.Tensor = None
    Wqkv: torch.Tensor = None
    bqkv: torch.Tensor = None
    Wo: torch.Tensor = None
    bo: torch.Tensor = None
    ln2_w: torch.Tensor = None
    ln2_b: torch.Tensor = None
    Wup: torch.Tensor = None
    Wdown: torch.Tensor = None


class EsmEngine:
    def __init__(self, cfg, device):
        self.cfg, self.device = cfg, device
        self.H = cfg.hidden_size
        self.nh = cfg.num_attention_heads
        self.hd = self.H // self.nh
# ... 44 lines not shown
```

### bioreason_amd/grpo.py

```python
from __future__ import annotations

from dataclasses import dataclass
from typing import Callable, Dict, List, Optional, Sequence, Tuple

import torch

from . import ops


def completion_mask(completion_ids: torch.Tensor, eos_token_id: int) -> torch.Tensor:
    mask, _ = ops.eos_mask(completion_ids.to(torch.int32).contiguous(), int(eos_token_id))
    return mask


def per_token_logps(model, prompt_ids: torch.Tensor, prompt_mask: torch.Tensor, completion_ids: torch.Tensor,
                    completion_mask_: torch.Tensor, **multimodal) -> torch.Tensor:
    B, P = prompt_ids.shape
    C = completion_ids.shape[1]
    ids = torch.cat([prompt_ids, completion_ids.to(prompt_ids.dtype)], dim=1)
    mask = torch.cat([prompt_mask, completion_mask_.to(prompt_mask.dtype)], dim=1)
    embeds = model._inputs_embeds(ids, multimodal.get("dna_tokenized"), multimodal.get("batch_idx_map"),
                                  multimodal.get("dna_alias"), multimodal.get("dna_enc"))
    hid = model.text_model.hidden_states(embeds, mask)
    S = P + C
    dev = ids.device
    rows = (torch.arange(B, device=dev, dtype=torch.int32)[:, None] * S
            + torch.arange(P - 1, S - 1, device=dev, dtype=torch.int32)[None, :]).reshape(-1).contiguous()
    tgt = completion_ids.to(torch.int32).reshape(-1).contiguous()
    return model.text_model.token_logprobs(hid, rows, tgt).view(B, C)


class _GrpoLossFn(torch.autograd.Function):
    @staticmethod
    def forward(ctx, logp, old_logp, ref_logp, adv, mask, eps_lo, eps_hi, beta):
        out3, dlogp = ops.grpo_loss(logp.contiguous(), old_logp, ref_logp, adv.contiguous().float(), mask.contiguous(),
                                    eps_lo, eps_hi, beta, need_grad=True)
        ctx.save_for_backward(dlogp)
        ctx.mark_non_differentiable(out3)
        return out3[0].clone(), out3

    @staticmethod
    def backward(ctx, g, _g3):
        (dlogp,) = ctx.saved_tensors
        return dlogp * g, None, None, None, None, None, None, None


def grpo_loss(logp, old_logp, ref_logp, advantages, mask, epsilon_low=0.2, epsilon_high=0.2, beta=0.04):
    rl = ref_logp.contiguous() if (ref_logp is not None and beta != 0.0) else None
    ol = old_logp.contiguous() if old_logp is not None else None
    return _GrpoLossFn.apply(logp, ol, rl, advantages, mask.to(torch.int32), epsilon_low, epsilon_high, beta)


def group_advantages(rewards_per_func: torch.Tensor, num_generations: int, rank: int = 0, local_n: Optional[int] = None):
    adv, gm, gs = ops.group_advantage(rewards_per_func.contiguous().float(), num_generations)
    if local_n is not None:
        adv = adv[rank * local_n:(rank + 1) * local_n]
    return adv, gm, gs


def repeat_sampler_indices(num_samples: int, mini_repeat_count: int, batch_size: int = 1, repeat_count: int = 1, seed: int = 0) -> List[int]:
    from .grpo_trainer import RepeatRandomSampler
    return list(RepeatRandomSampler(range(num_samples), mini_repeat_count, batch_size, repeat_count, seed))


def per_token_logps_shared_policy(model, prompt_ids: torch.Tensor, prompt_mask: torch.Tensor, completion_ids: torch.Tensor,
                                  completion_mask_: torch.Tensor, prompt_alias: Sequence[int], side=None, **multimodal) -> Optional[torch.Tensor]:
    from .generation import _uniform_groups
    grp = _uniform_groups(list(prompt_alias))
    if grp is None or grp[1] < 2:
        return None
    R, copies = grp
    tm = model.text_model
    B, P = prompt_ids.shape
    C = completion_ids.shape[1]
    dev = prompt_ids.device
    sel = torch.arange(R, device=dev) * copies
    embeds = model._inputs_embeds(prompt_ids, multimodal.get("dna_tokenized"), multimodal.get("batch_idx_map"),
                                  multimodal.get("dna_alias"), multimodal.get("dna_enc"))
    hid_last, hid_c = tm.hidden_states_shared(embeds.index_select(0, sel), prompt_mask.index_select(0, sel), completion_ids,
                                              completion_mask_, copies, side=side)
    from .modeling import _ExpandGroupsFn, _LogProbFn
    H = hid_c.shape[-1]
    first = _ExpandGroupsFn.apply(hid_last, copies)
    hsel = torch.cat([first[:, None, :], hid_c.view(B, C, H)[:, : C - 1, :]], dim=1).reshape(B * C, H).contiguous()
    tgt = completion_ids.to(torch.int32).reshape(-1).contiguous()
    return _LogProbFn.apply(hsel, tm, tgt).view(B, C)


@torch.no_grad()
def per_token_logps_shared_prefix(model, prompt_ids: torch.Tensor, prompt_mask: torch.Tensor, completion_ids: torch.Tensor,
                                  completion_mask_: torch.Tensor, prompt_alias: Sequence[int], side=None, **multimodal) -> torch.Tensor:
    from . import ops
    from .engine import BF16, SeqMeta
    from .generation import KVCache

    tm = model.text_model
    eng = tm.ensure_packed()
    B, P = prompt_ids.shape
    C = completion_ids.shape[1]
    S = P + C
    dev = prompt_ids.device
    from .generation import _uniform_groups
    grp = _uniform_groups(list(prompt_alias))
    if grp is not None and grp[1] >= 2:
        R, copies = grp
        sel = torch.arange(R, device=dev) * copies
        embeds = model._inputs_embeds(prompt_ids, multimodal.get("dna_tokenized"), multimodal.get("batch_idx_map"), multimodal.get("dna_alias"),
                                      multimodal.get("dna_enc"))
        mp = SeqMeta(B=R, S=P, pos=torch.arange(P, dtype=torch.int32, device=dev).repeat(R),
                     kmask=prompt_mask.index_select(0, sel).to(torch.uint8).contiguous(), lora_on=tm._lora_enabled, max_pos=S)
        kfull = torch.cat([prompt_mask, completion_mask_.to(prompt_mask.dtype)], dim=1).to(torch.uint8).contiguous()
        mc = SeqMeta(B=B, S=C, pos=(torch.arange(C, dtype=torch.int32, device=dev) + P).repeat(B), kmask=kfull,
                     lora_on=tm._lora_enabled, max_pos=S)
        ids32 = completion_ids.to(torch.int32).reshape(-1).contiguous()
        xc = torch.empty((B * C, eng.H), dtype=BF16, device=dev)
        ops.embed_scatter_fwd(ids32, None, eng.E, None, xc)
        xp = embeds.index_select(0, sel).reshape(R * P, -1).to(BF16).contiguous()
        hid_last, hid_c, _ = eng.forward_hidden_shared(xp, mp, xc, mc, copies, save=False, side=side)
        first = hid_last.repeat_interleave(copies, dim=0)
        hsel = torch.cat([first[:, None, :], hid_c.view(B, C, -1)[:, : C - 1, :]], dim=1).reshape(B * C, -1).contiguous()
        logp, _ = ops.lmhead_logprob(hsel, eng.E, ids32)
        return logp.view(B, C)
    reps = sorted(set(prompt_alias))
    where = {r: i for i, r in enumerate(reps)}
    sel = torch.tensor(reps, device=dev)
    gmap = torch.tensor([where[a] for a in prompt_alias], device=dev)
    R = len(reps)
    embeds = model._inputs_embeds(prompt_ids, multimodal.get("dna_tokenized"), multimodal.get("batch_idx_map"), multimodal.get("dna_alias"),
                                  multimodal.get("dna_enc"))
    cache_r = KVCache(eng, R, S, dev)
    meta = SeqMeta(B=R, S=P, pos=torch.arange(P, dtype=torch.int32, device=dev).repeat(R),
                   kmask=prompt_mask[sel].to(torch.uint8).contiguous(), lora_on=tm._lora_enabled, max_pos=S)
    x = embeds[sel].reshape(R * P, -1).to(BF16).contiguous()
    for li in range(eng.L):
        x, _ = eng.layer_fwd(li, x, meta, save=False, kv_out=(cache_r.k[li], cache_r.v[li], 0))
    last = torch.arange(R, device=dev, dtype=torch.int32) * P + (P - 1)
    hid_last = ops.rmsnorm_fwd(ops.gather_rows(last, x), eng.norm_w, eng.eps).index_select(0, gmap)
    kfull = torch.cat([prompt_mask, completion_mask_.to(prompt_mask.dtype)], dim=1).to(torch.uint8).contiguous()
# ... 14 lines not shown
```

### bioreason_amd/modeling.py

```python
from __future__ import annotations

import contextlib
from types import SimpleNamespace
from typing import Dict, List, Optional, Tuple

import torch
import torch.nn as nn

from . import ops
from .arena import TrainableArena
from .engine import BF16, EsmEngine, LoraGroup, QwenEngine, SeqMeta

LORA_TARGETS = ("q_proj", "k_proj", "v_proj", "o_proj", "gate_proj", "up_proj", "down_proj")


class HipLinear(nn.Linear):

    def forward(self, x):
        w = self.weight if self.weight.dtype == BF16 else self.weight.to(BF16)
        b = None if self.bias is None else self.bias.to(BF16)
        y = ops.gemm_nt(x.reshape(-1, x.shape[-1]).to(BF16).contiguous(), w.contiguous(), bias=b)
        return y.view(*x.shape[:-1], self.out_features)


# ... 47 lines not shown


class Qwen3MLP(nn.Module):
    def __init__(self, c, dev, dt):
        super().__init__()
        self.gate_proj = HipLinear(c.hidden_size, c.intermediate_size, bias=False, device=dev, dtype=dt)
        self.up_proj = HipLinear(c.hidden_size, c.intermediate_size, bias=False, device=dev, dtype=dt)
        self.down_proj = HipLinear(c.intermediate_size, c.hidden_size, bias=False, device=dev, dtype=dt)


class Qwen3DecoderLayer(nn.Module):
    def __init__(self, c, dev, dt):
        super().__init__()
        self.self_attn = Qwen3Attention(c, dev, dt)
        self.mlp = Qwen3MLP(c, dev, dt)
        self.input_layernorm = HipRMSNorm(c.hidden_size, c.rms_norm_eps, dev, dt)
        self.post_attention_layernorm = HipRMSNorm(c.hidden_size, c.rms_norm_eps, dev, dt)


class Qwen3Model(nn.Module):
    def __init__(self, c, dev, dt):
        super().__init__()
        self.embed_tokens = nn.Embedding(c.vocab_size, c.hidden_size, device=dev, dtype=dt)
        self.layers = nn.ModuleList([Qwen3DecoderLayer(c, dev, dt) for _ in range(c.num_hidden_layers)])
        self.norm = HipRMSNorm(c.hidden_size, c.rms_norm_eps, dev, dt)


def _unwrap(mod):
    return mod.base_layer if isinstance(mod, LoraLinear) else mod


class _StackFn(torch.autograd.Function):

    @staticmethod
    def forward(ctx, x, anchor, model, meta, grad_mode=True):
        eng = model.engine
        need = bool(grad_mode and (ctx.needs_input_grad[0] or ctx.needs_input_grad[1]))
        hid, tape = eng.forward_hidden(x, meta, save=need)
        ctx.model, ctx.meta, ctx.tape = model, meta, tape
        return hid

    @staticmethod
    def backward(ctx, dhid):
        eng = ctx.model.engine
        eng.ensure_transposed()
        dx = eng.backward_hidden(dhid.contiguous(), ctx.tape, ctx.meta)
        ctx.tape = None
        return dx, None, None, None, None


class _SharedStackFn(torch.autograd.Function):

    @staticmethod
    def forward(ctx, xp, xc, anchor, model, mp, mc, copies, side, grad_mode=True):
        eng = model.engine
        need = bool(grad_mode and (ctx.needs_input_grad[0] or ctx.needs_input_grad[2]))
        hid_last, hid_c, tape = eng.forward_hidden_shared(xp, mp, xc, mc, copies, save=need, side=side)
        ctx.model, ctx.mp, ctx.mc, ctx.copies, ctx.tape, ctx.side = model, mp, mc, copies, tape, side
        return hid_last, hid_c

    @staticmethod
    def backward(ctx, dlast, dc):
        eng = ctx.model.engine
        eng.ensure_transposed()
        dxp, dxc = eng.backward_hidden_shared(dlast.contiguous(), dc.contiguous(), ctx.tape, ctx.mp, ctx.mc, ctx.copies, side=ctx.side)
        ctx.tape = None
        return dxp, None, None, None, None, None, None, None, None


class _ExpandGroupsFn(torch.autograd.Function):

    @staticmethod
    def forward(ctx, x, copies):
        ctx.copies = copies
        return x.repeat_interleave(copies, dim=0)

    @staticmethod
    def backward(ctx, dy):
        return ops.group_sum(dy.contiguous(), ctx.copies), None


class _LogProbFn(torch.autograd.Function):

    @staticmethod
    def forward(ctx, h, model, tgt):
        eng = model.engine
        logp, lse = ops.lmhead_logprob(h, eng.E, tgt)
        ctx.save_for_backward(h, tgt, lse)
        ctx.model = model
        return logp

    @staticmethod
    def backward(ctx, dlogp):
        h, tgt, lse = ctx.saved_tensors
        eng = ctx.model.engine
        eng.ensure_transposed()
        dlogits = ops.lmhead_dlogits(h, eng.E, tgt, lse, dlogp.contiguous().float())
        dh = ops.gemm_nt(dlogits, eng.ET[:, :eng.V] if eng.ET.shape[1] != eng.V else eng.ET)
        return dh, None, None


class _LogitsFn(torch.autograd.Function):
    @staticmethod
    def forward(ctx, h, model):
        ctx.model = model
        return ops.gemm_nt(h, model.engine.E)

    @staticmethod
    def backward(ctx, dlogits):
        eng = ctx.model.engine
        eng.ensure_transposed()
        return ops.gemm_nt(dlogits.contiguous().to(BF16), eng.ET), None


class Qwen3ForCausalLM(nn.Module):

    def __init__(self, config, device=None, dtype=BF16):
        super().__init__()
        self.config = config
        self.model = Qwen3Model(config, device, dtype)
        self.lm_head = HipLinear(config.hidden_size, config.vocab_size, bias=False, device=device, dtype=dtype)
        self.lm_head.weight = self.model.embed_tokens.weight
        self.engine: Optional[QwenEngine] = None
        self.arena: Optional[TrainableArena] = None
        self._packed_sig = None
        self._lora_enabled = True
        self.warnings_issued: Dict[str, bool] = {}
        self.generation_config = SimpleNamespace()

    def get_input_embeddings(self):
        return self.model.embed_tokens

    def gradient_checkpointing_enable(self, *a, **k):
        return None

    def enable_input_require_grads(self):
        return None

    def tie_weights(self):
        self.lm_head.weight = self.model.embed_tokens.weight

    @property
    def device(self):
        return self.model.embed_tokens.weight.device

    @torch.no_grad()
    def init_weights(self, std: float = 0.02, seed: int = 0):
        g = torch.Generator(device=self.device).manual_seed(seed)
        for n, p in self.named_parameters():
            if "lora_" in n:
                continue
            if p.dim() >= 2:
# ... 134 lines not shown
                if W is None:
                    continue
                off = 0
                for mod in mods:
                    p = _unwrap(mod).weight
                    n = p.shape[0]
                    if p.dtype != BF16:
                        p.data.copy_(W[off:off + n].to(p.dtype))
                    off += n
        self._packed_sig = None
        self.ensure_packed()
        return self

    @contextlib.contextmanager
    def disable_adapter(self):
        prev = self._lora_enabled
        self._lora_enabled = False
        try:
            yield
        finally:
            self._lora_enabled = prev

    def set_dropout_seed(self, seed: int) -> None:
        self._dropout_seed = int(seed) & 0xFFFFFFFF
        self._dropout_calls = 0

    def hidden_states(self, inputs_embeds: torch.Tensor, attention_mask: Optional[torch.Tensor],
                      position_ids: Optional[torch.Tensor] = None) -> torch.Tensor:
        eng = self.ensure_packed()
        if self.arena is not None:
            self.arena.pack_if_stale()
        B, S, H = inputs_embeds.shape
        dev = inputs_embeds.device
        if position_ids is None:
            pos = torch.arange(S, dtype=torch.int32, device=dev).repeat(B)
            max_pos = S
        else:
            pos = position_ids.to(torch.int32).reshape(-1).contiguous()
            max_pos = self.config.max_position_embeddings
        kmask = None if attention_mask is None else attention_mask.to(torch.uint8).contiguous()
        meta = SeqMeta(B=B, S=S, pos=pos, kmask=kmask, lora_on=self._lora_enabled, max_pos=max_pos)
        p_drop = getattr(self, "lora_dropout_p", 0.0)
        if p_drop > 0.0 and self.training and self._lora_enabled:
            self._dropout_calls = getattr(self, "_dropout_calls", 0) + 1
            meta.drop_p = p_drop
            meta.drop_seed = (getattr(self, "_dropout_seed", 0x5EED) * 0x9E3779B1 + self._dropout_calls * 0x85EBCA6B) & 0xFFFFFFFF
        x = inputs_embeds.reshape(B * S, H)
        if x.dtype != BF16:
            x = x.to(BF16)
        anchor = self.arena.anchor if self.arena is not None else x.new_zeros(1, dtype=torch.float32)
        return _StackFn.apply(x.contiguous(), anchor, self, meta, torch.is_grad_enabled())

    def hidden_states_shared(self, prompt_embeds: torch.Tensor, prompt_mask: torch.Tensor, completion_ids: torch.Tensor,
                             completion_mask: torch.Tensor, copies: int, side=None):
        eng = self.ensure_packed()
        if self.arena is not None:
            self.arena.pack_if_stale()
        R, P, H = prompt_embeds.shape
        B, C = completion_ids.shape
        assert B == R * copies
        dev = prompt_embeds.device
        S = P + C
        kfull = torch.cat([prompt_mask.to(torch.uint8).repeat_interleave(copies, dim=0), completion_mask.to(torch.uint8)], dim=1).contiguous()
        mp = SeqMeta(B=R, S=P, pos=torch.arange(P, dtype=torch.int32, device=dev).repeat(R), kmask=prompt_mask.to(torch.uint8).contiguous(),
                     lora_on=self._lora_enabled, max_pos=S)
        mc = SeqMeta(B=B, S=C, pos=(torch.arange(C, dtype=torch.int32, device=dev) + P).repeat(B), kmask=kfull,
                     lora_on=self._lora_enabled, max_pos=S)
        p_drop = getattr(self, "lora_dropout_p", 0.0)
        if p_drop > 0.0 and self.training and self._lora_enabled:
            self._dropout_calls = getattr(self, "_dropout_calls", 0) + 1
            seed = (getattr(self, "_dropout_seed", 0x5EED) * 0x9E3779B1 + self._dropout_calls * 0x85EBCA6B) & 0xFFFFFFFF
            mp.drop_p = mc.drop_p = p_drop
            mp.drop_seed = seed
            mc.drop_seed = (seed * 0x2C1B3C6D + 0x5BD1E995) & 0xFFFFFFFF
        xp = prompt_embeds.reshape(R * P, H)
        if xp.dtype != BF16:
            xp = xp.to(BF16)
        xc = torch.empty((B * C, H), dtype=BF16, device=dev)
        ops.embed_scatter_fwd(completion_ids.to(torch.int32).reshape(-1).contiguous(), None, eng.E, None, xc)
        anchor = self.arena.anchor if self.arena is not None else xp.new_zeros(1, dtype=torch.float32)
        return _SharedStackFn.apply(xp.contiguous(), xc, anchor, self, mp, mc, copies, side, torch.is_grad_enabled())

    def forward(self, input_ids=None, attention_mask=None, inputs_embeds=None, labels=None, position_ids=None,
                return_logits: bool = True, **unused):
        from transformers.modeling_outputs import CausalLMOutputWithPast
        if inputs_embeds is None:
            eng = self.ensure_packed()
            ids32 = input_ids.to(torch.int32).reshape(-1).contiguous()
            x = torch.empty((ids32.numel(), eng.H), dtype=BF16, device=ids32.device)
            ops.embed_scatter_fwd(ids32, None, eng.E, None, x)
            inputs_embeds = x.view(*input_ids.shape, eng.H)
        B, S, H = inputs_embeds.shape
        rows = tgt = None
        if labels is not None:
            shift = labels[:, 1:].reshape(-1)
            valid = torch.nonzero(shift != -100, as_tuple=False).reshape(-1)
            b_idx, s_idx = valid // (S - 1), valid % (S - 1)
            rows = (b_idx * S + s_idx).to(torch.int32)
            tgt = shift[valid].to(torch.int32)
        hid = self.hidden_states(inputs_embeds, attention_mask, position_ids)
        loss = None
        if labels is not None and rows.numel() == 0:
            loss = _NanLossFn.apply(hid)
        elif labels is not None:
            hsel = _GatherRowsFn.apply(hid, rows)
            logp = _LogProbFn.apply(hsel, self, tgt)
            loss = _neg_mean(logp)
        logits = None
        if return_logits:
            logits = _LogitsFn.apply(hid, self).view(B, S, -1)
        return CausalLMOutputWithPast(loss=loss, logits=logits)

    def token_logprobs(self, hid: torch.Tensor, rows: torch.Tensor, targets: torch.Tensor) -> torch.Tensor:
        return _LogProbFn.apply(_GatherRowsFn.apply(hid, rows), self, targets)


class _GatherRowsFn(torch.autograd.Function):
    @staticmethod
    def forward(ctx, x, rows):
        ctx.save_for_backward(rows)
        ctx.n = x.shape[0]
        return ops.gather_rows(rows, x)

    @staticmethod
    def backward(ctx, dy):
        (rows,) = ctx.saved_tensors
        return ops.scatter_rows(rows, dy.contiguous(), ctx.n), None


class _NanLossFn(torch.autograd.Function):

    @staticmethod
    def forward(ctx, hid):
        ctx.meta = (hid.shape, hid.dtype, hid.device)
# ... 141 lines not shown
```

### bioreason_amd/ops.py

```python
from __future__ import annotations

import math
import os
from typing import Optional, Tuple

import torch

from ._lib import current_stream, get_lib

BF16 = torch.bfloat16


def _ld(t: torch.Tensor) -> int:
    assert t.stride(-1) == 1, "last dim must be contiguous"
    return t.stride(-2) if t.dim() >= 2 else t.shape[-1]


def _rows(t: torch.Tensor) -> int:
    return t.numel() // t.shape[-1]


def _as2d(t: torch.Tensor) -> torch.Tensor:
    return t.reshape(-1, t.shape[-1]) if t.dim() != 2 else t


def gemm_nt(
    a: torch.Tensor,
    b: torch.Tensor,
    *,
    a2: Optional[torch.Tensor] = None,
    b2: Optional[torch.Tensor] = None,
    bias: Optional[torch.Tensor] = None,
    res: Optional[torch.Tensor] = None,
    out: Optional[torch.Tensor] = None,
    alpha: float = 1.0,
    out_f32: bool = False,
    accumulate: bool = False,
) -> torch.Tensor:
    a = _as2d(a)
    M, K = a.shape
    N = b.shape[0]
    assert b.shape[1] == K and a.dtype == BF16 and b.dtype == BF16
    K2 = 0
    if a2 is not None:
        a2 = _as2d(a2)
        K2 = a2.shape[1]
        assert b2 is not None and b2.shape == (N, K2) and a2.shape[0] == M
    if out is None:
        out = torch.empty((M, N), dtype=torch.float32 if out_f32 else BF16, device=a.device)
    else:
        assert out.shape == (M, N) and out.dtype == (torch.float32 if out_f32 else BF16)
    if res is not None:
        res = _as2d(res)
        assert res.shape == (M, N) and res.dtype == BF16
    prof = GEMM_PROFILE
    timed = prof is not None and a.is_cuda and prof.wants(M, N, K, K2)
    if timed:
        e0 = torch.cuda.Event(enable_timing=True)
        e0.record()
    get_lib().call(
        "bra_gemm_bf16_nt", a, _ld(a), b, _ld(b), a2, _ld(a2) if a2 is not None else 0, b2,
        _ld(b2) if b2 is not None else 0, K2, out, _ld(out), M, N, K, alpha, bias, res,
        _ld(res) if res is not None else 0, int(out_f32), int(accumulate), current_stream(a),
    )
    if timed:
        e1 = torch.cuda.Event(enable_timing=True)
        e1.record()
        nbytes = 2.0 * (M * K + N * K + (M + N) * K2 + (M * N if res is not None else 0)) + M * N * (4.0 if out_f32 else 2.0)
        prof.records.append((2.0 * M * N * (K + K2), e0, e1, nbytes, (M, N, K, K2, res is not None)))
    return out


class GemmProfile:

    def __init__(self, min_m: int = 1024, dominant_only: bool = True):
        self.min_m = min_m
        self.dominant_only = dominant_only
        self.records = []

    def wants(self, M: int, N: int, K: int, K2: int) -> bool:
        if not self.dominant_only:
            return M >= self.min_m
        if K % 64 or K2 % 64:
            return False
        t = ((M + 255) // 256) * ((N + 255) // 256)
        rounds = (t + 255) // 256
        if t >= 140 and (t <= 256 or 100 * t >= 75 * rounds * 256):
            return True
        if ((M + 255) // 256) * ((N + 127) // 128) >= 128:
            return True
        return ((M + 127) // 128) * ((N + 127) // 128) >= 128

    def summary(self):
        torch.cuda.synchronize()
        fl = sum(r[0] for r in self.records)
        ms = sum(r[1].elapsed_time(r[2]) for r in self.records)
        n = len(self.records)
        by = sum(r[3] for r in self.records)
        return {"launches": n, "flops": fl, "ms": ms, "avg_launch_ms": ms / max(n, 1), "tflops": fl / max(ms, 1e-9) / 1e9,
                "flops_per_launch": fl / max(n, 1), "bytes_per_launch": by / max(n, 1)}


def gemm_profile_by_shape(prof: "GemmProfile"):
    torch.cuda.synchronize()
    agg = {}
    for r in prof.records:
        a = agg.setdefault(r[4], [0, 0.0, 0.0])
        a[0] += 1
        a[1] += r[1].elapsed_time(r[2])
        a[2] += r[0]
    return sorted(((k, n, ms, fl / max(ms, 1e-9) / 1e9) for k, (n, ms, fl) in agg.items()), key=lambda t: -t[2])


GEMM_PROFILE: Optional[GemmProfile] = None


def gemm_nt_splitk(a: torch.Tensor, b: torch.Tensor, out: torch.Tensor, alpha: float = 1.0, split_k: int = 0) -> torch.Tensor:
    M, K = a.shape
    N = b.shape[0]
    assert b.shape[1] == K and out.shape == (M, N) and out.dtype == torch.float32
    if split_k <= 0:
        tiles = ((M + 127) // 128) * ((N + 127) // 128)
        split_k = max(1, min(K // 256 if K >= 256 else 1, (512 + tiles - 1) // tiles))
    get_lib().call("bra_gemm_bf16_nt_splitk", a, _ld(a), b, _ld(b), out, _ld(out), M, N, K, alpha, split_k, current_stream(a))
    return out


def wgrad_tn(y: torch.Tensor, t: torch.Tensor, out: torch.Tensor, transposed_out: bool = False, alpha: float = 1.0,
             m_chunk: int = 0, drop=None, rank: int = 32) -> torch.Tensor:
    M, N = y.shape
    R = t.shape[1]
    assert t.shape[0] == M and out.dtype == torch.float32 and out.shape == ((R, N) if transposed_out else (N, R))
    c_sn, c_sr = (1, _ld(out)) if transposed_out else (_ld(out), 1)
    if drop is not None:
        get_lib().call("bra_wgrad_tn_drop", y, _ld(y), t, _ld(t), out, c_sn, c_sr, M, N, R, alpha, m_chunk, drop[0],
                       *_group(drop[1], rank, R), current_stream(y))
        return out
    get_lib().call("bra_wgrad_tn", y, _ld(y), t, _ld(t), out, c_sn, c_sr, M, N, R, alpha, m_chunk, current_stream(y))
    return out


LORA_DROP_RANKS = (8, 16, 32, 64, 128)


def _group(seeds, rank, R):
    if rank not in LORA_DROP_RANKS:
        raise NotImplementedError(f"LoRA dropout is built for adapter ranks {list(LORA_DROP_RANKS)}, not r = {rank}")
    if rank == 32:
        seeds = seeds[:max(R // 32, 1)]
    elif not 1 <= len(seeds) <= 3:
        raise ValueError(f"a fused LoRA group has 1 to 3 targets, got {len(seeds)} seeds")
    s = [int(x) & 0xFFFFFFFF for x in seeds]
    return (*(s + [0, 0, 0, 0])[:4], rank, len(s))


def dropout_mask(M: int, K: int, p: float, seed: int, device) -> torch.Tensor:
    out = torch.empty((M, K), dtype=torch.uint8, device=device)
    get_lib().call("bra_dropout_mask", out, M, K, p, int(seed) & 0xFFFFFFFF, current_stream(out))
    return out


LORA_DOWN_SPLITK = os.environ.get("BRA_LORA_SPLITK", "1") != "0"


def lora_down_drop(x: torch.Tensor, A: torch.Tensor, alpha: float, p: float, seeds, rank: int = 32) -> torch.Tensor:
    M, K = x.shape
    R = A.shape[0]
    t = torch.empty((M, R), dtype=BF16, device=x.device)
    lib = get_lib()
    ks = int(lib._dll.bra_lora_down_splitk_plan(int(M), int(K))) if LORA_DOWN_SPLITK else 1
    part = torch.empty((ks, M, R), dtype=torch.float32, device=x.device) if ks > 1 else None
    lib.call("bra_lora_down_drop", x, _ld(x), A, _ld(A), t, _ld(t), M, K, R, alpha, p, *_group(seeds, rank, R), part, ks,
             current_stream(x))
    return t


def lora_up_drop(dts: torch.Tensor, AT: torch.Tensor, p: float, seeds, rank: int = 32) -> torch.Tensor:
    M, R = dts.shape
    K = AT.shape[0]
    out = torch.empty((M, K), dtype=BF16, device=dts.device)
    get_lib().call("bra_lora_up_drop", dts, _ld(dts), AT, _ld(AT), out, _ld(out), M, K, R, p, *_group(seeds, rank, R),
                   current_stream(dts))
    return out


def lmhead_logprob(h: torch.Tensor, emb: torch.Tensor, tgt: torch.Tensor) -> Tuple[torch.Tensor, torch.Tensor]:
    M, K = h.shape
    V = emb.shape[0]
    nchunk = (V + 63) // 64
    dev = h.device
    pm = torch.empty((M, nchunk), dtype=torch.float32, device=dev)
    ps = torch.empty((M, nchunk), dtype=torch.float32, device=dev)
    tl = torch.zeros((M,), dtype=torch.float32, device=dev)
    lse = torch.empty((M,), dtype=torch.float32, device=dev)
    logp = torch.empty((M,), dtype=torch.float32, device=dev)
    st = current_stream(h)
    lib = get_lib()
    lib.call("bra_lmhead_lse_partials", h, _ld(h), emb, _ld(emb), M, V, K, tgt, pm, ps, tl, st)
    lib.call("bra_lse_merge", pm, ps, tl, lse, logp, M, nchunk, st)
    return logp, lse


def lmhead_dlogits(h: torch.Tensor, emb: torch.Tensor, tgt: torch.Tensor, lse: torch.Tensor, coef: torch.Tensor) -> torch.Tensor:
    M, K = h.shape
    V = emb.shape[0]
    out = torch.empty((M, V), dtype=BF16, device=h.device)
    get_lib().call("bra_lmhead_dlogits", h, _ld(h), emb, _ld(emb), M, V, K, tgt, lse, coef, out, _ld(out), current_stream(h))
    return out


def rmsnorm_fwd(x: torch.Tensor, w: torch.Tensor, eps: float) -> torch.Tensor:
    x2 = _as2d(x)
    y = torch.empty_like(x2)
    get_lib().call("bra_rmsnorm_fwd", x2, _ld(x2), w, y, _ld(y), None, x2.shape[0], x2.shape[1], eps, current_stream(x))
    return y.view(x.shape)


def rmsnorm_bwd(dy: torch.Tensor, x: torch.Tensor, w: torch.Tensor, eps: float, dres: Optional[torch.Tensor] = None) -> torch.Tensor:
    x2, dy2 = _as2d(x), _as2d(dy)
    dx = torch.empty_like(x2)
    d2 = _as2d(dres) if dres is not None else None
    get_lib().call("bra_rmsnorm_bwd", dy2, _ld(dy2), x2, _ld(x2), w, d2, _ld(d2) if d2 is not None else 0, dx, _ld(dx),
                   x2.shape[0], x2.shape[1], eps, current_stream(x))
    return dx.view(x.shape)


def layernorm_fwd(x: torch.Tensor, w: torch.Tensor, b: torch.Tensor, eps: float) -> torch.Tensor:
    x2 = _as2d(x)
    y = torch.empty_like(x2)
    get_lib().call("bra_layernorm_fwd", x2, _ld(x2), w, b, y, _ld(y), x2.shape[0], x2.shape[1], eps, current_stream(x))
    return y.view(x.shape)


def gemm_swiglu(x: torch.Tensor, W: torch.Tensor, a2: Optional[torch.Tensor] = None, b2: Optional[torch.Tensor] = None) -> Optional[torch.Tensor]:
    M, K = x.shape
    F = W.shape[0] // 2
    K2 = a2.shape[1] if a2 is not None else 0
    if M <= 16 or K % 64 or K2 % 64 or F % 128 or W.shape[0] != 2 * F:
        return None
    act = torch.empty((M, F), dtype=BF16, device=x.device)
    rc = get_lib().call_rc("bra_gemm_swiglu_bf16_nt", x, _ld(x), W, _ld(W), a2, _ld(a2) if a2 is not None else 0, b2,
                           _ld(b2) if b2 is not None else 0, K2, act, _ld(act), M, F, K, 1.0, current_stream(x))
    return None if rc != 0 else act


def swiglu_fwd(gu: torch.Tensor) -> torch.Tensor:
    gu2 = _as2d(gu)
    F = gu2.shape[1] // 2
    act = torch.empty((gu2.shape[0], F), dtype=BF16, device=gu.device)
    get_lib().call("bra_swiglu_fwd", gu2, _ld(gu2), act, _ld(act), gu2.shape[0], F, current_stream(gu))
    return act


def swiglu_bwd(gu: torch.Tensor, dact: torch.Tensor) -> torch.Tensor:
    gu2, d2 = _as2d(gu), _as2d(dact)
    F = gu2.shape[1] // 2
    dgu = torch.empty_like(gu2)
    get_lib().call("bra_swiglu_bwd", gu2, _ld(gu2), d2, _ld(d2), dgu, _ld(dgu), gu2.shape[0], F, current_stream(gu))
    return dgu


def _bsh_strides(t: torch.Tensor) -> Tuple[int, int, int]:
    assert t.dim() == 4 and t.stride(3) == 1
    return t.stride(0), t.stride(1), t.stride(2)


def qk_norm_rope_fwd(qkv, qw, kw, cosT, sinT, pos, S, Hq, Hkv, hd, eps, qscale, q, k, v, s_off=0):
    T = qkv.shape[0]
    get_lib().call("bra_qk_norm_rope_fwd", qkv, _ld(qkv), qw, kw, cosT, sinT, pos, T, S, Hq, Hkv, hd, eps, qscale,
                   q, *_bsh_strides(q), k, *_bsh_strides(k), v, *_bsh_strides(v), s_off, current_stream(qkv))


def qk_norm_rope_bwd(qkv, qw, kw, cosT, sinT, pos, S, Hq, Hkv, hd, eps, qscale, dq, dk, dv):
    T = qkv.shape[0]
    dqkv = torch.empty_like(qkv)
    get_lib().call("bra_qk_norm_rope_bwd", qkv, _ld(qkv), qw, kw, cosT, sinT, pos, T, S, Hq, Hkv, hd, eps, qscale,
                   dq, *_bsh_strides(dq), dk, *_bsh_strides(dk), dv, *_bsh_strides(dv), dqkv, _ld(dqkv), current_stream(qkv))
    return dqkv


def pad64(n: int) -> int:
    return (n + 63) // 64 * 64


def head_transpose(x: torch.Tensor) -> torch.Tensor:
    B, S, H, hd = x.shape
    out = torch.empty((B, H, hd, pad64(S)), dtype=BF16, device=x.device)
    sb, ss, sh = _bsh_strides(x)
    get_lib().call("bra_head_transpose", x, sb, ss, sh, out, out.stride(0), out.stride(1), out.stride(2), B, S, H, hd, current_stream(x))
    return out


def attn_fwd(q, k, vt, kmask, causal: bool, scale: float, q_off: Optional[int] = None, need_lse: bool = True,
# ... 456 lines not shown
```

### bioreason_amd/trainer.py

```python
from __future__ import annotations

import os
from dataclasses import dataclass
from typing import Callable, Dict, List, Optional

import torch
import torch.distributed as dist

from . import grpo, ops

METRIC_SLOT = "__dp_metrics__"


@dataclass
class GRPOConfig:
    num_generations: int = 8
    max_completion_length: int = 256
    temperature: float = 0.6
    top_p: float = 0.95
    top_k: int = 20
    repetition_penalty: float = 1.0
    min_p: Optional[float] = None
    beta: float = 0.04
    epsilon: float = 0.2
    epsilon_high: Optional[float] = None
    num_iterations: int = 1
    gradient_accumulation_steps: int = 1
    learning_rate: float = 1e-5
    weight_decay: float = 0.0
    adam_beta1: float = 0.9
    adam_beta2: float = 0.999
    adam_epsilon: float = 1e-8
    max_grad_norm: float = 1.0
    eos_token_id: Optional[int] = None
    pad_token_id: Optional[int] = None
    seed: int = 42
    rollout_graph: Optional[bool] = None
    rollout_shared_prefix: bool = True
    rollout_fp8: bool = False
    ref_fp8: bool = False
    grad_buckets: int = 4
    grad_allreduce_dtype: str = "fp32"
    share_dna_encoding: bool = True
    share_policy_prompt: Optional[bool] = None
    overlap_ref_pass: bool = True
    overlap_policy_chains: bool = True
    overlap_ref_chains: bool = False
    overlap_rollout_weights: bool = True


def token_stat_rewards(completion_ids: torch.Tensor, completion_mask: torch.Tensor) -> torch.Tensor:
    m = completion_mask.float()
    n = m.sum(1).clamp(min=1)
    r0 = ((completion_ids % 7 == 0).float() * m).sum(1) / n * 2.0
    r1 = ((completion_ids % 2 == 0).float() * m).sum(1) / n * 0.5
    return torch.stack([r0, r1], dim=1)


from .rewards import reward_hop as text_reward_fn


class _DataParallelStep:

    def __init__(self, model, n_buckets: int = 4, grad_dtype: str = "fp32"):
        self.model = model
        if grad_dtype not in ("fp32", "bf16"):
            raise ValueError("grad_allreduce_dtype must be 'fp32' or 'bf16'")
        self._grad_bf16 = grad_dtype == "bf16"
        self._bf_images: List = []
        self._bf_cache: Dict[tuple, torch.Tensor] = {}
        self.rank = dist.get_rank() if dist.is_initialized() else 0
        self.world = dist.get_world_size() if dist.is_initialized() else 1
        self.dp = dist.is_initialized() and (self.world > 1 or os.environ.get("BRA_DP_SINGLE_RANK") == "1")
        self.timers: Dict[str, float] = {}
        self._handles: List = []
        self.trace_buckets = False
        self._trace: List[dict] = []
        self._trace_t0 = None
        self._cuts: Dict[int, tuple] = {}
        self._n_buckets = max(1, int(n_buckets))
        arena = model.arena
        if self.dp and METRIC_SLOT not in arena._shapes:
            arena.add(METRIC_SLOT, 1, 64)
            arena.commit()
            arena.pack()
        self._plan_buckets()

    def _plan_buckets(self):
        a = self.model.arena
        eng = self.model.text_model.ensure_packed()
        L = eng.L
        starts = []
        for li in range(L):
            offs = [a._offsets[k] for k in a._offsets if k.startswith(f"text.layers.{li}.")]
            starts.append(min(offs) if offs else None)
        self._cuts = {}
        if not self.dp or any(s is None for s in starts) or sorted(starts) != starts:
            return
        nb = min(self._n_buckets, L)
# ... 78 lines not shown

    def bucket_report(self) -> List[dict]:
        if not self._trace or self._trace_t0 is None:
            return []
        torch.cuda.synchronize()
        end = self._trace_t0.elapsed_time(self._trace_join)
        return [{"range": [t["lo"], t["hi"]], "bytes": t["bytes"], "issued_at_ms": round(self._trace_t0.elapsed_time(t["issue"]), 3),
                 "joined_at_ms": round(self._trace_t0.elapsed_time(t["done"]), 3) if "done" in t else None,
                 "backward_end_ms": round(end, 3)} for t in self._trace]

    def _marks(self, timing: bool, dev):
        marks: List = []

        def mark(name):
            if timing and dev.type == "cuda":
                e = torch.cuda.Event(enable_timing=True)
                e.record()
                marks.append((name, e))
        return marks, mark

    def _close_marks(self, marks):
        if marks:
            torch.cuda.synchronize()
            for (n0, e0), (n1, e1) in zip(marks[:-1], marks[1:]):
                self.timers[n1] = self.timers.get(n1, 0.0) + e0.elapsed_time(e1)


class GRPOStepRunner(_DataParallelStep):
    metric_names = ["completion_length", "reward", "reward_std", "loss", "kl", "clip_ratio"]

    def __init__(self, model, cfg: GRPOConfig, reward_fn: Callable = token_stat_rewards):
        super().__init__(model, cfg.grad_buckets, getattr(cfg, "grad_allreduce_dtype", "fp32"))
        self.cfg, self.reward_fn = cfg, reward_fn
        self.global_step = 0
        self._step = 0
        self.step_idx = 0
        self._buffered_inputs: List[Optional[Dict]] = [None] * max(1, cfg.gradient_accumulation_steps)
        if hasattr(model.text_model, "set_dropout_seed"):
            model.text_model.set_dropout_seed(cfg.seed * 1000003 + self.rank)
        self.rollout_profile: Dict[str, float] = {}
        self.loop_events: Optional[list] = None
        self.lr_schedule: Optional[Callable[[int], float]] = None
        self.last_lr = cfg.learning_rate

    def _side_stream(self, dev, which: int = 0):
        if dev.type != "cuda":
            return None
        if getattr(self, "_side", None) is None:
            self._side = {}
        if which not in self._side:
            self._side[which] = torch.cuda.Stream(device=dev)
        return self._side[which]

    def generate_and_score(self, batch: Dict, timing: bool = False, mark=lambda n: None, defer_ref_join: bool = False) -> Dict:
        tm = self.model.text_model
        had, prev = hasattr(tm, "rollout_fp8"), getattr(tm, "rollout_fp8", False)
        tm.rollout_fp8 = bool(prev) or bool(self.cfg.rollout_fp8)
        try:
            return self._generate_and_score(batch, timing, mark, defer_ref_join)
        finally:
            if had:
                tm.rollout_fp8 = prev
            else:
                try:
                    delattr(tm, "rollout_fp8")
                except AttributeError:
                    pass

    def _generate_and_score(self, batch: Dict, timing: bool = False, mark=lambda n: None, defer_ref_join: bool = False) -> Dict:
        m, c = self.model, self.cfg
        dev = batch["input_ids"].device
        mm = {"dna_tokenized": batch["dna_tokenized"], "batch_idx_map": batch["batch_idx_map"], "dna_alias": batch.get("dna_alias")}
        wside = None
        if (c.overlap_rollout_weights and dev.type == "cuda" and not timing and c.rollout_shared_prefix
                and batch.get("prompt_alias") is not None):
            from . import generation as _gen
            wside = self._side_stream(dev, 2)
            wside.wait_stream(torch.cuda.current_stream(dev))
            with torch.cuda.stream(wside):
                _gen.rollout_weights(m.text_model, rows=int(batch["input_ids"].shape[0]))
        if c.share_dna_encoding and batch["dna_tokenized"] is not None and batch["batch_idx_map"]:
            mm["dna_enc"] = m.encode_dna(batch["dna_tokenized"], batch.get("dna_alias"))
        prompt_ids, prompt_mask = batch["input_ids"], batch["attention_mask"]
        B = prompt_ids.shape[0]
        if wside is not None:
            torch.cuda.current_stream(dev).wait_stream(wside)
        sched = batch.get("eos_schedule")
        completion_ids = m.generate(input_ids=prompt_ids, attention_mask=prompt_mask, **mm,
                                    max_new_tokens=c.max_completion_length, do_sample=True, temperature=c.temperature,
                                    top_k=c.top_k, top_p=c.top_p, repetition_penalty=c.repetition_penalty, min_p=c.min_p,
                                    eos_token_id=c.eos_token_id, pad_token_id=c.pad_token_id,
                                    seed=c.seed + 1000003 * self.step_idx + self.rank, return_full_length=sched is None,
                                    prompt_alias=batch.get("prompt_alias"), use_graph=c.rollout_graph,
                                    shared_prefix_decode=c.rollout_shared_prefix, eos_schedule=sched,
                                    profile=self.rollout_profile if timing else None, loop_events=self.loop_events)
        self.step_idx += 1
        mark("rollout")
        if c.eos_token_id is not None:
            cmask = grpo.completion_mask(completion_ids, c.eos_token_id)
        else:
            cmask = torch.ones(completion_ids.shape, dtype=torch.int32, device=dev)
        old_lp = None
        if c.num_iterations > 1:
            with torch.no_grad():
                old_lp = grpo.per_token_logps(m, prompt_ids, prompt_mask, completion_ids, cmask, **mm).detach()
        ref_lp = None
        ref_join = None
        if c.beta != 0.0:
            def ref_pass():
                eng_ = m.text_model.ensure_packed()
                w8 = None
                if c.ref_fp8 and eng_.fp8_supported():
                    sig = getattr(m.text_model, "_packed_sig", None)
                    cached = getattr(eng_, "_ref_fp8", None)
                    if cached is None or cached[0] != sig:
                        cached = eng_._ref_fp8 = (sig, eng_.fp8_weight_images())
                    w8 = cached[1]
                with torch.no_grad(), m.text_model.disable_adapter(), eng_.use_fp8(w8):
                    if batch.get("prompt_alias") is not None:
                        return grpo.per_token_logps_shared_prefix(m, prompt_ids, prompt_mask, completion_ids, cmask,
                                                                  batch["prompt_alias"], side=ref_side2, **mm)
                    return grpo.per_token_logps(m, prompt_ids, prompt_mask, completion_ids, cmask, **mm)
            side = self._side_stream(dev) if (c.overlap_ref_pass and not timing) else None
            ref_side2 = self._side_stream(dev, 3) if (side is not None and c.overlap_ref_chains) else None
            if side is not None:
                side.wait_stream(torch.cuda.current_stream(dev))
                with torch.cuda.stream(side):
                    ref_lp = ref_pass()
                ref_join = side
            else:
                ref_lp = ref_pass()
        mark("ref_logps")
        rewards = self.reward_fn(completion_ids, cmask).float()
        packed = torch.cat([rewards, cmask.sum(1, keepdim=True).float()], dim=1).contiguous()
        if self.dp:
            gathered = [torch.empty_like(packed) for _ in range(self.world)]
            dist.all_gather(gathered, packed)
            packed_all = torch.cat(gathered, dim=0)
        else:
            packed_all = packed
        F = rewards.shape[1]
        all_rewards = packed_all[:, :F].contiguous()
        adv, gmean, gstd = grpo.group_advantages(all_rewards, c.num_generations, self.rank, B)
        roll_metrics = torch.stack([packed_all[:, F].mean(), all_rewards.sum(1).mean(), gstd.mean()])
        mark("rewards")
        if ref_join is not None and not defer_ref_join:
            torch.cuda.current_stream(dev).wait_stream(ref_join)
            ref_lp.record_stream(torch.cuda.current_stream(dev))
            ref_join = None
        return {"prompt_ids": prompt_ids, "prompt_mask": prompt_mask, "completion_ids": completion_ids, "completion_mask": cmask,
                "old_per_token_logps": old_lp, "ref_per_token_logps": ref_lp, "advantages": adv, "multimodal_inputs": mm,
                "prompt_alias": batch.get("prompt_alias"), "ref_join": ref_join,
                "rewards_per_func": all_rewards.mean(0), "roll_metrics": roll_metrics}

    def shares_policy_prompt(self) -> bool:
        want = self.cfg.share_policy_prompt
        if want is None:
            return float(getattr(self.model.text_model, "lora_dropout_p", 0.0) or 0.0) == 0.0
        return bool(want)

    def compute_loss(self, inputs: Dict):
        m, c = self.model, self.cfg
        lp = None
        if self.shares_policy_prompt() and inputs.get("prompt_alias") is not None:
            side2 = self._side_stream(inputs["prompt_ids"].device, 1) if c.overlap_policy_chains else None
            lp = grpo.per_token_logps_shared_policy(m, inputs["prompt_ids"], inputs["prompt_mask"], inputs["completion_ids"],
                                                    inputs["completion_mask"], inputs["prompt_alias"], side=side2,
                                                    **inputs["multimodal_inputs"])
        if lp is None:
            lp = grpo.per_token_logps(m, inputs["prompt_ids"], inputs["prompt_mask"], inputs["completion_ids"],
                                      inputs["completion_mask"], **inputs["multimodal_inputs"])
        eps_hi = c.epsilon_high if c.epsilon_high is not None else c.epsilon
        old = inputs["old_per_token_logps"] if c.num_iterations > 1 else None
        if inputs.get("ref_join") is not None:
            torch.cuda.current_stream(lp.device).wait_stream(inputs["ref_join"])
            inputs["ref_join"] = None
        return grpo.grpo_loss(lp, old, inputs["ref_per_token_logps"], inputs["advantages"], inputs["completion_mask"],
                              c.epsilon, eps_hi, c.beta)

    def step(self, batch: Dict, timing: bool = False) -> Dict[str, torch.Tensor]:
        m, c = self.model, self.cfg
        dev = batch["input_ids"].device
        marks, mark = self._marks(timing, dev)
        if timing:
            self.rollout_profile.clear()
            self.timers.clear()
        ga = max(1, c.gradient_accumulation_steps)
        slot = self._step % ga
        mark("start")
        if self.global_step % c.num_iterations == 0:
            inputs = self.generate_and_score(batch, timing, mark, defer_ref_join=True)
            self._buffered_inputs[slot] = inputs
        else:
            inputs = self._buffered_inputs[slot]
        self._step += 1
        if slot == 0:
            m.arena.zero_grad()
        if slot == ga - 1:
            self.begin_backward()
        loss, stats = self.compute_loss(inputs)
        mark("policy_fwd")
        if self.dp:
            m.arena.grad(METRIC_SLOT).view(-1)[:3].add_(stats / ga)
        (loss / ga if ga > 1 else loss).backward()
        mark("policy_bwd")
        out = {"loss_t": loss.detach(), "stats_t": stats, "reward_mean_t": inputs["roll_metrics"][1]}
        if slot == ga - 1:
            scale = self.reduce_gradients()
            if self.dp:
                local3 = m.arena.grad(METRIC_SLOT).view(-1)[:3] * scale
            else:
                local3 = stats
            lr = c.learning_rate if self.lr_schedule is None else float(self.lr_schedule(self.global_step))
            self.last_lr = lr
            m.arena.adamw_step(lr, (c.adam_beta1, c.adam_beta2), c.adam_epsilon, c.weight_decay,
                               max_grad_norm=c.max_grad_norm, grad_scale=scale)
            self.global_step += 1
            out["metrics_t"] = torch.cat([inputs["roll_metrics"], local3.detach().clone()])
            out["rewards_per_func_t"] = inputs["rewards_per_func"]
        mark("optimizer")
        if timing:
            self._close_marks(marks)
        return out


def cosine_schedule_with_warmup(base_lr: float, total_steps: int, warmup_ratio: float = 0.1) -> Callable[[int], float]:
    import math
    total = max(1, int(total_steps))
    warm = int(warmup_ratio * total)

    def rate(i: int) -> float:
        if i < warm:
            return base_lr * float(i) / float(max(1, warm))
        prog = float(i - warm) / float(max(1, total - warm))
        return base_lr * max(0.0, 0.5 * (1.0 + math.cos(math.pi * prog)))
    return rate


class SFTStepRunner(_DataParallelStep):

    def __init__(self, model, learning_rate: float = 1e-4, weight_decay: float = 0.01, max_grad_norm: float = 1.0,
                 n_buckets: int = 4, return_logits: bool = True, gradient_accumulation_steps: int = 1,
                 lr_schedule: Optional[Callable[[int], float]] = None):
        super().__init__(model, n_buckets)
        self.lr, self.wd, self.max_grad_norm, self.return_logits = learning_rate, weight_decay, max_grad_norm, return_logits
        self.ga = max(1, int(gradient_accumulation_steps))
        self.lr_schedule = lr_schedule
        self.global_step = 0
        self._micro = 0
        self.last_lr = learning_rate
        if hasattr(model.text_model, "set_dropout_seed"):
            model.text_model.set_dropout_seed(23 * 1000003 + self.rank)

    def step(self, batch: Dict, timing: bool = False) -> Dict[str, torch.Tensor]:
        m = self.model
        dev = batch["input_ids"].device
        marks, mark = self._marks(timing, dev)
        if timing:
            self.timers.clear()
# ... 25 lines not shown
```

### include/bioreason_hip.h

```cpp
#ifndef BIOREASON_HIP_H
#define BIOREASON_HIP_H
#ifdef __cplusplus
extern "C" {
#endif

#define BRA_ERR_ARG (-1)
#define BRA_ERR_UNSUPPORTED (-2)

int bra_gemm_bf16_nt(const void* A, long lda, const void* B, long ldb, const void* A2, long lda2, const void* B2,
                     long ldb2, int K2, void* C, long ldc, int M, int N, int K, float alpha, const void* bias,
                     const void* res, long ldres, int out_f32, int accumulate, void* stream);

int bra_gemm_bf16_nt_splitk(const void* A, long lda, const void* B, long ldb, void* C, long ldc, int M, int N, int K,
                            float alpha, int split_k, void* stream);

int bra_wgrad_tn(const void* Y, long ldy, const void* T, long ldt, float* C, long c_sn, long c_sr, int M, int N, int R,
                 float alpha, int m_chunk, void* stream);

int bra_lora_down_splitk_plan(int M, int K);
int bra_lora_down_drop(const void* x, long ldx, const void* A, long lda, void* t, long ldt, int M, int K, int R, float alpha,
                       float p, unsigned s0, unsigned s1, unsigned s2, unsigned s3, int r, int nt, float* part, int ksplit,
                       void* stream);
int bra_lora_up_drop(const void* dts, long ldd, const void* AT, long ldat, void* out, long ldo, int M, int K, int R, float p,
                     unsigned s0, unsigned s1, unsigned s2, unsigned s3, int r, int nt, void* stream);
int bra_wgrad_tn_drop(const void* Y, long ldy, const void* T, long ldt, float* C, long c_sn, long c_sr, int M, int N, int R,
                      float alpha, int m_chunk, float p, unsigned s0, unsigned s1, unsigned s2, unsigned s3, int r, int nt,
                      void* stream);
int bra_dropout_mask(void* out, int M, int K, float p, unsigned seed, void* stream);

int bra_lmhead_lse_partials(const void* H, long ldh, const void* E, long lde, int M, int V, int K, const int* tgt,
                            float* part_max, float* part_sum, float* tgt_logit, void* stream);
int bra_lse_merge(const float* part_max, const float* part_sum, const float* tgt_logit, float* lse, float* logp,
                  int rows, int nchunk, void* stream);
int bra_lmhead_dlogits(const void* H, long ldh, const void* E, long lde, int M, int V, int K, const int* tgt,
                       const float* lse, const float* coef, void* dlogits, long ldd, void* stream);

int bra_rmsnorm_fwd(const void* x, long ldx, const void* w, void* y, long ldy, float* rstd, int rows, int cols,
                    float eps, void* stream);
int bra_rmsnorm_bwd(const void* dy, long lddy, const void* x, long ldx, const void* w, const void* dres, long lddres,
                    void* dx, long lddx, int rows, int cols, float eps, void* stream);
int bra_layernorm_fwd(const void* x, long ldx, const void* w, const void* b, void* y, long ldy, int rows, int cols,
                      float eps, void* stream);
int bra_swiglu_fwd(const void* gu, long ldgu, void* act, long ldact, int rows, int F, void* stream);
int bra_swiglu_bwd(const void* gu, long ldgu, const void* dact, long lddact, void* dgu, long lddgu, int rows, int F,
                   void* stream);
int bra_qk_norm_rope_fwd(const void* qkv, long ldqkv, const void* qw, const void* kw, const float* cosT,
                         const float* sinT, const int* pos, int T, int S, int Hq, int Hkv, int hd, float eps,
                         float qscale, void* q, long q_sb, long q_ss, long q_sh, void* k, long k_sb, long k_ss,
                         long k_sh, void* v, long v_sb, long v_ss, long v_sh, int s_off, void* stream);
int bra_qk_norm_rope_bwd(const void* qkv, long ldqkv, const void* qw, const void* kw, const float* cosT,
                         const float* sinT, const int* pos, int T, int S, int Hq, int Hkv, int hd, float eps,
                         float qscale, const void* dq, long q_sb, long q_ss, long q_sh, const void* dk, long k_sb,
                         long k_ss, long k_sh, const void* dv, long v_sb, long v_ss, long v_sh, void* dqkv,
                         long lddqkv, void* stream);

int bra_attn_fwd(const void* q, long q_sb, long q_ss, long q_sh, const void* k, long k_sb, long k_ss, long k_sh,
                 const void* vt, long vt_sb, long vt_sh, long vt_sd, void* o, long o_sb, long o_ss, long o_sh,
                 float* lse, const void* kmask, int B, int Hq, int Hkv, int Sq, int Sk, int hd, int causal,
                 int q_off, float scale, void* stream);
int bra_attn_fwd_split(const void* q, long q_sb, long q_ss, long q_sh, const void* k, long k_sb, long k_ss, long k_sh,
                       const void* vt, long vt_sb, long vt_sh, long vt_sd, void* o, long o_sb, long o_ss, long o_sh,
                       float* lse, const void* kmask, int B, int Hq, int Hkv, int Sq, int Sk, int hd, int causal,
                       int q_off, float scale, int nsplit, float* part_o, float* part_ml, void* stream);
int bra_attn_bwd(const void* q, long q_sb, long q_ss, long q_sh, const void* k, long k_sb, long k_ss, long k_sh,
                 const void* v, long v_sb, long v_ss, long v_sh, const void* dout, long do_sb, long do_ss, long do_sh,
                 const void* kt, long kt_sb, long kt_sh, long kt_sd, const void* qt, long qt_sb, long qt_sh,
                 long qt_sd, const void* dot, long dot_sb, long dot_sh, long dot_sd, const float* lse,
                 const float* delta, const void* kmask, void* dq, long dq_sb, long dq_ss, long dq_sh, void* dk,
                 long dk_sb, long dk_ss, long dk_sh, void* dv, long dv_sb, long dv_ss, long dv_sh, int B, int Hq,
                 int Hkv, int Sq, int Sk, int hd, int causal, int q_off, float scale, void* stream);
int bra_attn_bwd_split(const void* q, long q_sb, long q_ss, long q_sh, const void* k, long k_sb, long k_ss, long k_sh,
                 const void* v, long v_sb, long v_ss, long v_sh, const void* dout, long do_sb, long do_ss, long do_sh,
                 const void* kt, long kt_sb, long kt_sh, long kt_sd, const void* qt, long qt_sb, long qt_sh,
                 long qt_sd, const void* dot, long dot_sb, long dot_sh, long dot_sd, const float* lse,
                 const float* delta, const void* kmask, void* dq, long dq_sb, long dq_ss, long dq_sh, void* dk,
                 long dk_sb, long dk_ss, long dk_sh, void* dv, long dv_sb, long dv_ss, long dv_sh, int B, int Hq,
                 int Hkv, int Sq, int Sk, int hd, int causal, int q_off, float scale, int nsplit_dq, float* part_dq, int nsplit_kv, float* part_dk, float* part_dv, void* stream);
int bra_attn_decode_nchunk(int len);
int bra_attn_decode(const void* q, const void* kc, const void* vc, const void* kmask, float* part_o, float* part_ml,
                    void* o, int B, int Hq, int Hkv, int hd, int Smax, int len, float scale, void* stream);

int bra_qwen_layer_desc_size(void);
int bra_qwen_decode_step(const void* layers_host, int L, int B, int H, int Hq, int Hkv, int hd, int F, int Smax,
                         float eps, float scale, const void* E, const void* norm_w, const float* cosT,
                         const float* sinT, const int* tok, const int* pos, const void* kmask, int cur_len,
                         int lora_on, void* x, void* xn, void* qkv, void* q, void* o, void* h, void* hn, void* gu,
                         void* act, void* t, float* part_o, float* part_ml, void* hid, void* stream);

int bra_dec_gemm(const void* x, long ldx, const void* norm_w, float eps, const void* W, long ldw, const void* res,
                 long ldres, void* out, long ldo, int M, int N, int K, int act, int out_f32, void* stream);
int bra_dec_attn_partial(const void* qkv, long ldqkv, const void* qw, const void* kw, const float* cosT,
                         const float* sinT, const int* pos, void* kc, void* vc, const void* kmask, float* part_o,
                         float* part_ml, int B, int Hq, int Hkv, int hd, int Smax, int cur_len, float eps, float scale,
                         int chunk_off, int nchunk_tot, const int* t_dev, void* stream);
int bra_dec_gemm2(const void* x, long ldx, const float* ss_in, int nss_in, const void* norm_w, float eps, const void* W,
                  long ldw, const void* res, long ldres, void* out, long ldo, float* ss_out, int nss_out, int M, int N,
                  int K, int act, int out_f32, void* stream);
int bra_dec_gemm2_packed(const void* x, long ldx, const float* ss_in, int nss_in, const void* norm_w, float eps, const void* W,
                         long ldw, const void* res, long ldres, void* out, long ldo, float* ss_out, int nss_out, int M, int N,
                         int K, int act, int out_f32, int packed, void* stream);
int bra_dec_pack_weights_fp8(const void* W, long ldw, int N, int K, int act, int out_f32, const void* norm_w, void* out_q,
                             float* out_scale, void* stream);
int bra_dec_gemm2_fp8(const void* x, long ldx, const float* ss_in, int nss_in, float eps, const void* Wq, const float* wscale,
                      const void* res, long ldres, void* out, long ldo, float* ss_out, int nss_out, int M, int N, int K, int act,
                      int out_f32, int norm_folded, void* stream);
int bra_dec_pack_weights_fp8_rows(const void* W, long ldw, int N, int K, int act, int out_f32, const void* norm_w, int rows,
                                  void* out_q, float* out_scale, void* stream);
int bra_dec_gemm2_fp8_rows(const void* x, long ldx, const float* ss_in, int nss_in, float eps, const void* Wq, const float* wscale,
                           const void* res, long ldres, void* out, long ldo, float* ss_out, int nss_out, int M, int N, int K, int act,
                           int out_f32, int norm_folded, int image_rows, void* stream);
int bra_dec_pack_weights_fp8_anyk(const void* W, long ldw, int N, int K, void* out_q, float* out_scale, void* stream);
int bra_dec_gemm2_fp8_anyk(const void* x, long ldx, const void* Wq, const float* wscale, const void* res, long ldres, void* out, long ldo,
                           float* ss_out, int nss_out, int M, int N, int K, void* stream);
int bra_dec_gemm2_fp8_anyk_ok(int N, int K);
int bra_gemm_swiglu_bf16_nt(const void* A, long lda, const void* W, long ldw, const void* A2, long lda2, const void* B2, long ldb2, int K2,
                            void* C, long ldc, int M, int F, int K, float alpha, void* stream);
int bra_quant_rows_fp8(const void* x, long ldx, int M, int K, const void* colw, void* q, long ldq, float* scale, int rms, float eps,
                       void* stream);
int bra_swiglu_quant_fp8(const void* gu, long ldgu, int M, int F, void* q, long ldq, float* scale, void* stream);
int bra_gemm_fp8_nt(const void* A8, long lda, const float* sa, const void* B8, long ldb, const float* sb, void* C, long ldc, int M, int N,
                    int K, const void* res, long ldres, int out_f32, void* stream);
int bra_dec_pack_weights(const void* W, long ldw, int N, int K, int act, int out_f32, const void* norm_w, void* out, void* stream);
int bra_dec_pack_weights_rows(const void* W, long ldw, int N, int K, int act, int out_f32, const void* norm_w, int rows, void* out,
                              void* stream);
int bra_row_sumsq(const void* x, long ldx, int M, int K, float* ss, int nss, void* stream);
int bra_dec_stat_cols(int H);
int bra_dec_gemm2_rows32_ok(int K, int normed, int packed);
int bra_dec_gemm2_fp8_rows32_ok(int K, int normed);
int bra_dec_attn_shared(const void* qkv, long ldqkv, const void* qw, const float* cosT, const float* sinT, const int* pos,
                        const void* kp, long kp_sr, long kp_sh, long kp_ss, const void* vtp, long vt_sr, long vt_sh,
                        long vt_sd, const void* pmask, float* part_o, float* part_ml, int R, int copies, int Hq, int Hkv,
                        int hd, int P, int nchunk_tot, float eps, float scale, const int* t_dev, void* stream);
int bra_dec_attn_both(const void* qkv, long ldqkv, const void* qw, const void* kw, const float* cosT, const float* sinT,
                      const int* pos, const void* kp, long kp_sr, long kp_sh, long kp_ss, const void* vtp, long vt_sr,
                      long vt_sh, long vt_sd, const void* pmask, void* kc, void* vc, float* part_o, float* part_ml, int R,
                      int copies, int Hq, int Hkv, int hd, int P, int C, int t, float eps, float scale, const int* t_dev,
                      const float* rope_rows, void* stream);
int bra_attn_decode_merge(const float* part_o, const float* part_ml, void* o, int B, int Hq, int hd, int nchunk,
                          const int* t_dev, int npc, void* stream);
int bra_qwen_decode_step_fused(const void* layers_host, int L, int B, int H, int Hq, int Hkv, int hd, int F, int Smax,
                               int V, float eps, float scale, const void* E, const void* norm_w, const float* cosT,
                               const float* sinT, const int* tok, const int* pos, const void* kmask, int cur_len,
                               const int* len_dev, int embed_done, void* x, void* qkv, void* o, void* h, void* act, float* ss_ws,
                               int nss, float* part_o, float* part_ml, float* logits, void* stream);

int bra_qwen_decode_step_shared(const void* layers_host, int L, int R, int copies, int H, int Hq, int Hkv, int hd, int F,
                                int P, long vt_pitch, int C, int V, float eps, float scale, const void* E,
                                const void* norm_w, const float* cosT, const float* sinT, const int* tok, const int* pos,
                                const void* pmask, int t, const int* t_dev, int embed_done, void* x, void* qkv, void* o, void* h,
                                void* act, float* ss_ws, int nss, float* part_o, float* part_ml, float* logits, void* stream);

int bra_dec_attn_one(const void* qkv, long ldqkv, const void* qw, const void* kw, const float* cosT, const float* sinT,
                     const int* pos, const float* rope_rows, const void* kp, long kp_sr, long kp_sh, long kp_ss,
                     const void* vtp, long vt_sr, long vt_sh, long vt_sd, const void* pmask, void* kc, void* vct, long cp,
                     float* part_o, float* part_ml, int nslot, void* o, long ldo, int R, int copies,
                     int Hq, int Hkv, int hd, int P, int C, int t, float eps, float scale, const int* t_dev, void* stream);
int bra_qwen_decode_step_one(const void* layers_host, int L, int R, int copies, int H, int Hq, int Hkv, int hd, int F,
                             int P, long vt_pitch, int C, long cp, int V, float eps, float scale, const void* E,
                             const void* norm_w, const float* cosT, const float* sinT, const int* tok, const int* pos,
                             const void* pmask, int t, const int* t_dev, int embed_done, void* x, void* qkv, void* o, void* h,
                             void* act, float* ss_ws, int nss, float* part_o, float* part_ml, int nslot, float* logits,
                             void* stream);

int bra_head_transpose(const void* x, long sb, long ss, long sh, void* xt, long t_sb, long t_sh, long pitch, int B,
                       int S, int H, int hd, void* stream);
int bra_attn_delta(const void* dout, long do_sb, long do_ss, long do_sh, const void* o, long o_sb, long o_ss,
                   long o_sh, float* delta, int B, int S, int H, int hd, void* stream);
int bra_dna_scatter_plan(const int* ids, int ntok, int dna_id, const void* dna_mask, int nseq, int Sd,
                         const int* seq_order, int* tok_src, int* counts, void* stream);
// ... 66 lines not shown
```

Baseline: 19.57.

## Compute reference logprobs inside the shared policy pass using row-bounded LoRA GEMMs

New measurement: 19.55. About the same (-0.1%).

```diff
diff --git a/bioreason_amd/csrc/k_gemm.hip b/bioreason_amd/csrc/k_gemm.hip
--- a/bioreason_amd/csrc/k_gemm.hip
+++ b/bioreason_amd/csrc/k_gemm.hip
@@ -11,6 +11,7 @@
     EPI_LSE = 2,
     EPI_DLOGIT = 3,
     EPI_ATOMIC = 4,
+    EPI_ROWS = 16,
     EPI_SWIGLU = 5,
 };
 
@@ -22,6 +23,7 @@
     void* C;          long ldc;
     int M, N, K, K2;
     float alpha;
+    int a2_rows;
     const bf16_t* bias;
     const bf16_t* res;
     long ldres;
@@ -36,6 +38,9 @@
     int nchunk;
     int swiglu_F;
 };
+
+constexpr int A2_ZERO_ELEMS = 4096;
+__device__ __attribute__((aligned(128))) bf16_t a2_zero_row[A2_ZERO_ELEMS];
 
 template <int BK>
 __device__ __forceinline__ int swz_chunk(int row, int c) {
@@ -426,8 +431,10 @@
     }
 }
 
-template <int BM, int BK, int EPI, int PF>
+template <int BM, int BK, int EPIX, int PF>
 __global__ __launch_bounds__(BM * 2) void gemm_nt_kernel(GemmArgs g) {
+    constexpr int EPI = EPIX & (EPI_ROWS - 1);
+    constexpr bool A2R = (EPIX & EPI_ROWS) != 0;
     constexpr int BN = 128, NT = BM * 2;
     constexpr int CH = BK / 8;
     constexpr int LPTA = (BM * CH) / NT;
@@ -454,7 +461,7 @@
     const int tile_n = (bid % per_group) / gsize;
     const int m0 = tile_m * BM, n0 = tile_n * BN;
 
-    const int nk1 = g.K / BK, nk2 = g.K2 / BK;
+    const int nk1 = g.K / BK, nk2 = (A2R && m0 >= g.a2_rows) ? 0 : g.K2 / BK;
     int kt_begin = 0, kt_end = nk1 + nk2;
     if (EPI == EPI_ATOMIC && g.split_k > 1) {
         int per = (kt_end + g.split_k - 1) / g.split_k;
@@ -474,7 +481,12 @@
         for (int i = 0; i < LPTA; ++i) {
             const int q = tid + NT * i;
             int rm = m0 + q / CH; rm = rm < g.M ? rm : g.M - 1;
-            ra[s][i] = ld16(Ap + (long)rm * la + k0 + (q % CH) * 8);
+            if constexpr (A2R) {
+                const bf16_t* ap = (kt >= nk1 && rm >= g.a2_rows) ? a2_zero_row : Ap + (long)rm * la;
+                ra[s][i] = ld16(ap + k0 + (q % CH) * 8);
+            } else {
+                ra[s][i] = ld16(Ap + (long)rm * la + k0 + (q % CH) * 8);
+            }
         }
 #pragma unroll
         for (int i = 0; i < LPTB; ++i) {
@@ -562,8 +574,10 @@
     gemm_epilogue<EPI>(g, acc, m0, n0, wm, wn, lane, tile_n);
 }
 
-template <int EPI, int SKEW, int MI = 4>
+template <int EPIX, int SKEW, int MI = 4>
 __global__ __launch_bounds__(512, 2) void gemm_glds_kernel(GemmArgs g) {
+    constexpr int EPI = EPIX & (EPI_ROWS - 1);
+    constexpr bool A2R = (EPIX & EPI_ROWS) != 0;
     constexpr int BM = 64 * MI, BN = 128, BK = 64;
     constexpr int A_BYTES = BM * BK * 2, B_BYTES = BN * BK * 2, STAGE = A_BYTES + B_BYTES;
     BRA_DYN_SMEM(smem);
@@ -586,7 +600,7 @@
     const int tile_n = (bid % per_group) / gsize;
     const int m0 = tile_m * BM, n0 = tile_n * BN;
 
-    const int nk1 = g.K / BK, nk2 = g.K2 / BK;
+    const int nk1 = g.K / BK, nk2 = (A2R && m0 >= g.a2_rows) ? 0 : g.K2 / BK;
     int kt_begin = 0, kt_end = nk1 + nk2;
     if (EPI == EPI_ATOMIC && g.split_k > 1) {
         int per = (kt_end + g.split_k - 1) / g.split_k;
@@ -610,7 +624,14 @@
         const bf16_t* Bp = (main ? g.B : g.B2) + (long)(main ? kt : kt - nk1) * BK + lchunk;
         const long la = main ? g.lda : g.lda2, lb = main ? g.ldb : g.ldb2;
 #pragma unroll
-        for (int j = 0; j < MI; ++j) glds16(Ap + (long)rowA[j] * la, sa + j * 1024);
+        for (int j = 0; j < MI; ++j) {
+            if constexpr (A2R) {
+                const bf16_t* zp = a2_zero_row + (long)(kt - nk1) * BK + lchunk;
+                glds16((!main && rowA[j] >= g.a2_rows) ? zp : Ap + (long)rowA[j] * la, sa + j * 1024);
+            } else {
+                glds16(Ap + (long)rowA[j] * la, sa + j * 1024);
+            }
+        }
 #pragma unroll
         for (int j = 0; j < 2; ++j) glds16(Bp + (long)rowB[j] * lb, sb + j * 1024);
     };
@@ -842,8 +863,10 @@
 #endif
 }
 
-template <int EPI, int WM, int WN>
+template <int EPIX, int WM, int WN>
 __global__ __launch_bounds__(256) void gemm_w4_kernel(GemmArgs g) {
+    constexpr int EPI = EPIX & (EPI_ROWS - 1);
+    constexpr bool A2R = (EPIX & EPI_ROWS) != 0;
     static_assert(WN % 4 == 0, "the wave epilogue works on 64-column groups");
     constexpr int BM = 32 * WM, BN = 32 * WN, BK = 64;
     constexpr int A_BYTES = BM * BK * 2, STAGE = (BM + BN) * BK * 2;
@@ -866,7 +889,7 @@
     const int tile_n = (bid % per_group) / gsize;
     const int m0 = tile_m * BM, n0 = tile_n * BN;
 
-    const int nk1 = g.K / BK, nk2 = g.K2 / BK;
+    const int nk1 = g.K / BK, nk2 = (A2R && m0 >= g.a2_rows) ? 0 : g.K2 / BK;
     const int nt = nk1 + nk2;
 
     const int prow = lane >> 3, lchunk = ((lane & 7) ^ (lane >> 3)) * 8;
@@ -875,7 +898,11 @@
 #pragma unroll
         for (int j = 0; j < NDMA; ++j) {
             const int r = (wave * NDMA + j) * 8 + prow;
-            if (r < BM) { int m = m0 + r; m = m < g.M ? m : g.M - 1; src[j] = (main ? g.A : g.A2) + (long)m * (main ? g.lda : g.lda2) + lchunk; }
+            if (r < BM) {
+                int m = m0 + r; m = m < g.M ? m : g.M - 1;
+                src[j] = (main ? g.A : g.A2) + (long)m * (main ? g.lda : g.lda2) + lchunk;
+                if (A2R && !main && m >= g.a2_rows) src[j] = a2_zero_row + lchunk;
+            }
             else { int n = n0 + r - BM; n = n < g.N ? n : g.N - 1; src[j] = (main ? g.B : g.B2) + (long)n * (main ? g.ldb : g.ldb2) + lchunk; }
         }
     };
@@ -999,8 +1026,10 @@
     }
 }
 
-template <int EPI, int PH2 = 0>
+template <int EPIX, int PH2 = 0>
 __global__ __launch_bounds__(512, 2) void gemm_ring_kernel(GemmArgs g) {
+    constexpr int EPI = EPIX & (EPI_ROWS - 1);
+    constexpr bool A2R = (EPIX & EPI_ROWS) != 0;
     constexpr int BM = 256, BN = 256, BK = 64, HALF = 128 * BK * 2, NSLOT = 10;
     BRA_DYN_SMEM(smem);
     const int tid = (int)threadIdx.x;
@@ -1022,7 +1051,7 @@
     const int tile_n = (bid % per_group) / gsize;
     const int m0 = tile_m * BM, n0 = tile_n * BN;
 
-    const int nk1 = g.K / BK, nk2 = g.K2 / BK;
+    const int nk1 = g.K / BK, nk2 = (A2R && m0 >= g.a2_rows) ? 0 : g.K2 / BK;
     int kt_begin = 0, kt_end = nk1 + nk2;
     if (EPI == EPI_ATOMIC && g.split_k > 1) {
         int per = (kt_end + g.split_k - 1) / g.split_k;
@@ -1050,7 +1079,10 @@
 #pragma unroll
         for (int pc = 0; pc < 2; ++pc) {
             if (h < 2) src[h * 2 + pc] = (main ? g.B : g.B2) + kcol + (long)rowB[h * 2 + pc] * (main ? g.ldb : g.ldb2);
-            else src[h * 2 + pc] = (main ? g.A : g.A2) + kcol + (long)rowA[(h - 2) * 2 + pc] * (main ? g.lda : g.lda2);
+            else {
+                src[h * 2 + pc] = (main ? g.A : g.A2) + kcol + (long)rowA[(h - 2) * 2 + pc] * (main ? g.lda : g.lda2);
+                if (A2R && !main && rowA[(h - 2) * 2 + pc] >= g.a2_rows) src[h * 2 + pc] = a2_zero_row + kcol;
+            }
         }
     };
 #pragma unroll
@@ -1177,8 +1209,10 @@
     else gemm_epilogue_w<EPI, 8>(g, acc, m0 + wr * 128, n0 + wc * 64, lane, smem + wave * (128 * EPI_RS));
 }
 
-template <int OUTF32>
+template <int OUTX>
 __global__ __launch_bounds__(256) void gemm_skinny_kernel(GemmArgs g) {
+    constexpr int OUTF32 = OUTX & 1;
+    constexpr bool A2R = (OUTX & EPI_ROWS) != 0;
     __shared__ float red[4][64][4];
     const int tid = (int)threadIdx.x, lane = tid & 63, wave = tid >> 6;
     const int fr = lane & 15, fq = lane >> 4;
@@ -1203,6 +1237,7 @@
     if (g.K2 > 0) {
         const bf16_t* wp = g.B2 + (long)rn * g.ldb2 + fq * 8;
         const bf16_t* xp = g.A2 + (long)rm * g.lda2 + fq * 8;
+        if (A2R && rm >= g.a2_rows) xp = a2_zero_row + fq * 8;
         const int nk = g.K2 / 32;
         for (int kt = wave; kt < nk; kt += 4) acc = mfma_16x16x32(ld16(wp + (long)kt * 32), ld16(xp + (long)kt * 32), acc);
     }
@@ -1233,8 +1268,15 @@
     }
 }
 
+static inline bool a2_bounded(const GemmArgs& g) { return g.K2 > 0 && g.a2_rows < g.M; }
+
 static int launch_skinny(const GemmArgs& g, int out_f32, bra_stream_t stream) {
     const int grid = (g.N + 15) / 16;
+    if (a2_bounded(g)) {
+        if (out_f32) return BRA_ERR_UNSUPPORTED;
+        BRA_LAUNCH((gemm_skinny_kernel<EPI_ROWS>), dim3(grid), dim3(256), 0, stream, g);
+        return BRA_LAUNCH_STATUS();
+    }
     if (out_f32) BRA_LAUNCH((gemm_skinny_kernel<1>), dim3(grid), dim3(256), 0, stream, g);
     else BRA_LAUNCH((gemm_skinny_kernel<0>), dim3(grid), dim3(256), 0, stream, g);
     return BRA_LAUNCH_STATUS();
@@ -1276,6 +1318,14 @@
     int grid = tiles;
     if (EPI == EPI_ATOMIC) grid = tiles * (g.split_k > 0 ? g.split_k : 1);
     const size_t smem = 2 * (size_t)(BM + 128) * BK * 2;
+    if (a2_bounded(g)) {
+        if constexpr (EPI == EPI_BF16) {
+            BRA_ALLOW_SMEM((gemm_nt_kernel<BM, BK, EPI | EPI_ROWS, PF>), smem);
+            BRA_LAUNCH((gemm_nt_kernel<BM, BK, EPI | EPI_ROWS, PF>), dim3(grid), dim3(BM * 2), smem, stream, g);
+            return BRA_LAUNCH_STATUS();
+        }
+        return BRA_ERR_UNSUPPORTED;
+    }
     BRA_ALLOW_SMEM((gemm_nt_kernel<BM, BK, EPI, PF>), smem);
     BRA_LAUNCH((gemm_nt_kernel<BM, BK, EPI, PF>), dim3(grid), dim3(BM * 2), smem, stream, g);
     return BRA_LAUNCH_STATUS();
@@ -1305,6 +1355,19 @@
     int grid = tiles;
     if (EPI == EPI_ATOMIC) grid = tiles * (g.split_k > 0 ? g.split_k : 1);
     const size_t smem = 3 * (size_t)(BM + 128) * 64 * 2;
+    if (a2_bounded(g)) {
+        if constexpr (EPI == EPI_BF16) {
+            if (skew) {
+                BRA_ALLOW_SMEM((gemm_glds_kernel<EPI | EPI_ROWS, 1, MI>), smem);
+                BRA_LAUNCH((gemm_glds_kernel<EPI | EPI_ROWS, 1, MI>), dim3(grid), dim3(512), smem, stream, g);
+            } else {
+                BRA_ALLOW_SMEM((gemm_glds_kernel<EPI | EPI_ROWS, 0, MI>), smem);
+                BRA_LAUNCH((gemm_glds_kernel<EPI | EPI_ROWS, 0, MI>), dim3(grid), dim3(512), smem, stream, g);
+            }
+            return BRA_LAUNCH_STATUS();
+        }
+        return BRA_ERR_UNSUPPORTED;
+    }
     if (skew) {
         BRA_ALLOW_SMEM((gemm_glds_kernel<EPI, 1, MI>), smem);
         BRA_LAUNCH((gemm_glds_kernel<EPI, 1, MI>), dim3(grid), dim3(512), smem, stream, g);
@@ -1349,6 +1412,14 @@
     constexpr int BM = 32 * WM, BN = 32 * WN, STAGE = (BM + BN) * 128, NS = (160 * 1024) / STAGE >= 4 ? 4 : 3;
     const int tiles = ((g.M + BM - 1) / BM) * ((g.N + BN - 1) / BN);
     const size_t smem = (size_t)NS * STAGE;
+    if (a2_bounded(g)) {
+        if constexpr (EPI == EPI_BF16) {
+            BRA_ALLOW_SMEM((gemm_w4_kernel<EPI | EPI_ROWS, WM, WN>), smem);
+            BRA_LAUNCH((gemm_w4_kernel<EPI | EPI_ROWS, WM, WN>), dim3(tiles), dim3(256), smem, stream, g);
+            return BRA_LAUNCH_STATUS();
+        }
+        return BRA_ERR_UNSUPPORTED;
+    }
     BRA_ALLOW_SMEM((gemm_w4_kernel<EPI, WM, WN>), smem);
     BRA_LAUNCH((gemm_w4_kernel<EPI, WM, WN>), dim3(tiles), dim3(256), smem, stream, g);
     return BRA_LAUNCH_STATUS();
@@ -1370,6 +1441,19 @@
 static int launch_ring(const GemmArgs& g, bra_stream_t stream) {
     const int tiles = ((g.M + 255) / 256) * ((g.N + 255) / 256);
     const size_t smem = 10 * (size_t)128 * 64 * 2;
+    if (a2_bounded(g)) {
+        if constexpr (EPI == EPI_BF16 || EPI == EPI_SWIGLU) {
+            if (ring_two_phase) {
+                BRA_ALLOW_SMEM((gemm_ring_kernel<EPI | EPI_ROWS, 1>), smem);
+                BRA_LAUNCH((gemm_ring_kernel<EPI | EPI_ROWS, 1>), dim3(tiles), dim3(512), smem, stream, g);
+            } else {
+                BRA_ALLOW_SMEM((gemm_ring_kernel<EPI | EPI_ROWS, 0>), smem);
+                BRA_LAUNCH((gemm_ring_kernel<EPI | EPI_ROWS, 0>), dim3(tiles), dim3(512), smem, stream, g);
+            }
+            return BRA_LAUNCH_STATUS();
+        }
+        return BRA_ERR_UNSUPPORTED;
+    }
     if (ring_two_phase) {
         BRA_ALLOW_SMEM((gemm_ring_kernel<EPI, 1>), smem);
         BRA_LAUNCH((gemm_ring_kernel<EPI, 1>), dim3(tiles), dim3(512), smem, stream, g);
@@ -1419,6 +1503,8 @@
             g2.M = g.M - m1;
             g2.A = g.A + (long)m1 * g.lda;
             if (g.A2) g2.A2 = g.A2 + (long)m1 * g.lda2;
+            g1.a2_rows = g.a2_rows < m1 ? g.a2_rows : m1;
+            g2.a2_rows = g.a2_rows - m1 < 0 ? 0 : g.a2_rows - m1;
             g2.C = EPI == EPI_F32 ? (void*)((float*)g.C + (long)m1 * g.ldc) : (void*)((bf16_t*)g.C + (long)m1 * g.ldc);
             if (g.res) g2.res = g.res + (long)m1 * g.ldres;
             const int e = launch_ring<EPI>(g1, stream);
@@ -1473,10 +1559,17 @@
 extern "C" int bra_gemm_set_row_split(int on) { bra::ring_row_split = on; return 0; }
 #endif
 
-extern "C" int bra_gemm_bf16_nt(const void* A, long lda, const void* B, long ldb, const void* A2, long lda2,
-                                const void* B2, long ldb2, int K2, void* C, long ldc, int M, int N, int K,
-                                float alpha, const void* bias, const void* res, long ldres, int out_f32,
-                                int accumulate, void* stream) {
+static int bound_a2(GemmArgs& g, int a2_rows, bool f32_out) {
+    g.a2_rows = a2_rows < g.M ? a2_rows : g.M;
+    if (g.K2 > 0 && g.a2_rows <= 0) { g.K2 = 0; g.A2 = nullptr; g.B2 = nullptr; g.lda2 = g.ldb2 = 0; g.a2_rows = g.M; }
+    if (a2_bounded(g) && (f32_out || g.K2 > A2_ZERO_ELEMS - 64)) return BRA_ERR_UNSUPPORTED;
+    return 0;
+}
+
+extern "C" int bra_gemm_bf16_nt_rows(const void* A, long lda, const void* B, long ldb, const void* A2, long lda2,
+                                     const void* B2, long ldb2, int K2, void* C, long ldc, int M, int N, int K,
+                                     float alpha, const void* bias, const void* res, long ldres, int out_f32,
+                                     int accumulate, int a2_rows, void* stream) {
     GemmArgs g = {};
     g.A = (const bf16_t*)A; g.lda = lda; g.B = (const bf16_t*)B; g.ldb = ldb;
     g.A2 = (const bf16_t*)A2; g.lda2 = lda2; g.B2 = (const bf16_t*)B2; g.ldb2 = ldb2;
@@ -1485,11 +1578,21 @@
     if (M == 0 || N == 0) return 0;
     int e = check_common(g);
     if (e) return e;
+    e = bound_a2(g, a2_rows, out_f32 != 0);
+    if (e) return e;
     if (!C || ldc % 4) return BRA_ERR_ARG;
     if (out_f32 && res) return BRA_ERR_ARG;
     if (M <= 16) return launch_skinny(g, out_f32, (bra_stream_t)stream);
     if (out_f32) return dispatch_bk<EPI_F32>(g, (bra_stream_t)stream);
     return dispatch_bk<EPI_BF16>(g, (bra_stream_t)stream);
+}
+
+extern "C" int bra_gemm_bf16_nt(const void* A, long lda, const void* B, long ldb, const void* A2, long lda2,
+                                const void* B2, long ldb2, int K2, void* C, long ldc, int M, int N, int K,
+                                float alpha, const void* bias, const void* res, long ldres, int out_f32,
+                                int accumulate, void* stream) {
+    return bra_gemm_bf16_nt_rows(A, lda, B, ldb, A2, lda2, B2, ldb2, K2, C, ldc, M, N, K, alpha, bias, res, ldres, out_f32, accumulate,
+                                 M, stream);
 }
 
 extern "C" int bra_gemm_fp8_nt(const void* A8, long lda, const float* sa, const void* B8, long ldb, const float* sb, void* C, long ldc,
@@ -1518,8 +1621,8 @@
 #undef BRA_G8
 }
 
-extern "C" int bra_gemm_swiglu_bf16_nt(const void* A, long lda, const void* W, long ldw, const void* A2, long lda2, const void* B2, long ldb2,
-                                       int K2, void* C, long ldc, int M, int F, int K, float alpha, void* stream) {
+extern "C" int bra_gemm_swiglu_bf16_nt_rows(const void* A, long lda, const void* W, long ldw, const void* A2, long lda2, const void* B2,
+                                            long ldb2, int K2, void* C, long ldc, int M, int F, int K, float alpha, int a2_rows, void* stream) {
     if (M == 0 || F == 0) return 0;
     GemmArgs g = {};
     g.A = (const bf16_t*)A; g.lda = lda; g.B = (const bf16_t*)W; g.ldb = ldw;
@@ -1529,7 +1632,14 @@
     if (e) return e;
     if (!C || ldc % 8 || ((size_t)C & 15)) return BRA_ERR_ARG;
     if (K % 64 || K2 % 64 || F % 128 || M <= 16) return BRA_ERR_UNSUPPORTED;
+    e = bound_a2(g, a2_rows, false);
+    if (e) return e;
     return launch_ring<EPI_SWIGLU>(g, (bra_stream_t)stream);
+}
+
+extern "C" int bra_gemm_swiglu_bf16_nt(const void* A, long lda, const void* W, long ldw, const void* A2, long lda2, const void* B2, long ldb2,
+                                       int K2, void* C, long ldc, int M, int F, int K, float alpha, void* stream) {
+    return bra_gemm_swiglu_bf16_nt_rows(A, lda, W, ldw, A2, lda2, B2, ldb2, K2, C, ldc, M, F, K, alpha, M, stream);
 }
 
 extern "C" int bra_gemm_bf16_nt_splitk(const void* A, long lda, const void* B, long ldb, void* C, long ldc, int M,
diff --git a/bioreason_amd/csrc/k_lora.hip b/bioreason_amd/csrc/k_lora.hip
--- a/bioreason_amd/csrc/k_lora.hip
+++ b/bioreason_amd/csrc/k_lora.hip
@@ -14,6 +14,7 @@
     int nb_live;
     int steps_per;
     float* part;
+    int live_m;
 };
 
 template <int RB, int NL, int TR = 32, int NT = NL>
@@ -31,12 +32,22 @@
     const int m0 = (int)blockIdx.x * 32;
     const int nstep = (g.K + KS - 1) / KS;
     const u32x4 zero4 = {0u, 0u, 0u, 0u};
+    if (m0 >= g.live_m) {
+        for (int i = tid; i < 32 * g.R; i += 256) {
+            const int m = m0 + i / g.R, r = i % g.R;
+            if (m < g.M) {
+                if (g.part) g.part[((long)blockIdx.y * g.M + m) * g.R + r] = 0.f;
+                else g.t[(long)m * g.ldt + r] = (bf16_t)0;
+            }
+        }
+        return;
+    }
     u32x4 rx[2], ra[2 * NL];
     auto issue = [&](int s) {
 #pragma unroll
         for (int i = 0; i < 2; ++i) {
             const int c = tid + 256 * i, row = c >> 4, k = KS * s + 8 * (c & 15);
-            int m = m0 + row; m = m < g.M ? m : g.M - 1;
+            int m = m0 + row; m = m < g.live_m ? m : g.live_m - 1;
             rx[i] = ld16(g.x + (long)m * g.ldx + (k < g.K ? k : 0));
         }
 #pragma unroll
@@ -131,6 +142,7 @@
 #pragma unroll
                 for (int w = 0; w < 3; ++w) v += red[((w * NL + (rb < NL ? rb : 0)) * 64 + lane) * 16 + q];
             }
+            if (m >= g.live_m) v = 0.f;
             if (m < g.M && r < g.R) {
                 if (g.part) pbase[(long)mq * g.R + 32 * rb] = v;
                 else tbase[(long)mq * g.ldt + 32 * rb] = f2bf(g.alpha * v);
@@ -269,11 +281,12 @@
     return (nstep + per - 1) / per;
 }
 
-extern "C" int bra_lora_down_drop(const void* x, long ldx, const void* A, long lda, void* t, long ldt, int M, int K, int R,
-                                  float alpha, float p, unsigned s0, unsigned s1, unsigned s2, unsigned s3, int r, int nt,
-                                  float* part, int ksplit, void* stream) {
+extern "C" int bra_lora_down_drop_rows(const void* x, long ldx, const void* A, long lda, void* t, long ldt, int M, int K, int R,
+                                       float alpha, float p, unsigned s0, unsigned s1, unsigned s2, unsigned s3, int r, int nt,
+                                       float* part, int ksplit, int live_m, void* stream) {
     if (M == 0) return 0;
     if (!x || !A || !t || M < 0 || K <= 0 || K % 8 || ldx % 8 || lda % 8 || !lora_drop_ok(p, M, K, r, nt, R)) return BRA_ERR_ARG;
+    if (live_m < 0 || live_m > M) return BRA_ERR_ARG;
     if (ksplit <= 1) part = nullptr;
     else if (!part || ksplit > (K + 127) / 128 || ldt % 4) return BRA_ERR_ARG;
     const unsigned seeds[4] = {s0, s1, s2, s3};
@@ -286,7 +299,7 @@
         float* const ps = part ? part + (long)ksplit * M * s.c0 : nullptr;
         bf16_t* const ts = (bf16_t*)t + s.c0;
         LoraDownArgs g = {(const bf16_t*)x, ldx, (const bf16_t*)A + (long)s.c0 * lda, lda, ts, ldt, M, K, s.Rs, alpha,
-                          make_cfg(p, seeds + s.j0, s.nts), 0, per, ps};
+                          make_cfg(p, seeds + s.j0, s.nts), 0, per, ps, live_m};
 #define BRA_LD(C_, RB_, NL_, TR_, NT_) if (C_) BRA_LAUNCH((lora_down_drop_kernel<RB_, NL_, TR_, NT_>), grid, dim3(256), 0, st, g); else
         BRA_LORA_ROWS(BRA_LD) return BRA_ERR_ARG;
 #undef BRA_LD
@@ -297,6 +310,12 @@
         }
         return BRA_LAUNCH_STATUS();
     });
+}
+
+extern "C" int bra_lora_down_drop(const void* x, long ldx, const void* A, long lda, void* t, long ldt, int M, int K, int R,
+                                  float alpha, float p, unsigned s0, unsigned s1, unsigned s2, unsigned s3, int r, int nt,
+                                  float* part, int ksplit, void* stream) {
+    return bra_lora_down_drop_rows(x, ldx, A, lda, t, ldt, M, K, R, alpha, p, s0, s1, s2, s3, r, nt, part, ksplit, M, stream);
 }
 
 extern "C" int bra_lora_up_drop(const void* dts, long ldd, const void* AT, long ldat, void* out, long ldo, int M, int K, int R,
diff --git a/bioreason_amd/engine.py b/bioreason_amd/engine.py
--- a/bioreason_amd/engine.py
+++ b/bioreason_amd/engine.py
@@ -91,6 +91,7 @@
     max_pos: int = 0
     drop_p: float = 0.0
     drop_seed: int = 0
+    lora_rows: Optional[int] = None
 
 
 def _mix32(a: int, b: int) -> int:
@@ -164,7 +165,21 @@
         return ops.gemm_nt(x2d, A, alpha=scaling)
 
     @staticmethod
-    def _lora_fwd(x2d, W, G: Optional[LoraGroup], on: bool, res=None, out=None, drop=None):
+    def _down_rows(x2d, G: LoraGroup, drop, rows: int):
+        if drop is not None:
+            return ops.lora_down_drop(x2d, G.A, G.scaling, drop[0], drop[1], drop[2], live_m=rows)
+        live = len(G.n_sizes) * G.r
+        if G.A.shape[0] in (32, 64, 128):
+            return ops.lora_down_drop(x2d, G.A, G.scaling, 0.0, [0] * min(G.A.shape[0] // 32, (live + 31) // 32), rank=32, live_m=rows)
+        t = torch.zeros((x2d.shape[0], G.A.shape[0]), dtype=BF16, device=x2d.device)
+        ops.gemm_nt(x2d[:rows], G.A, alpha=G.scaling, out=t[:rows])
+        return t
+
+    @staticmethod
+    def _lora_fwd(x2d, W, G: Optional[LoraGroup], on: bool, res=None, out=None, drop=None, rows: Optional[int] = None):
+        if G is not None and on and rows is not None:
+            t = QwenEngine._down_rows(x2d, G, drop, rows)
+            return ops.gemm_nt(x2d, W, a2=t, b2=G.B, res=res, out=out, a2_rows=rows), t
         if G is not None and on:
             if drop is not None:
                 t = ops.lora_down_drop(x2d, G.A, G.scaling, drop[0], drop[1], drop[2])
@@ -256,7 +271,8 @@
         B, S, T = m.B, m.S, m.B * m.S
         cosT, sinT = self.rope(m.max_pos or m.S)
         xn = ops.rmsnorm_fwd(x, L.ln1, self.eps)
-        qkv, t1 = self._lora_fwd(xn, L.Wqkv, L.lora["qkv"], m.lora_on, drop=self._drop(m, li, "qkv"))
+        lr = m.lora_rows
+        qkv, t1 = self._lora_fwd(xn, L.Wqkv, L.lora["qkv"], m.lora_on, drop=self._drop(m, li, "qkv"), rows=lr)
         q = torch.empty((B, S, self.Hq, self.hd), dtype=BF16, device=x.device)
         if kv_out is None:
             k = torch.empty((B, S, self.Hkv, self.hd), dtype=BF16, device=x.device)
@@ -271,26 +287,37 @@
         vt = ops.head_transpose(v)
         if kv_out is not None and len(kv_out) > 3 and kv_out[3] is not None:
             kv_out[3].append(vt)
-        o, lse = ops.attn_fwd(q, k, vt, m.kmask, True, self.scale, need_lse=save)
+        ns = None if lr is None else ops.attn_fwd_split_parts(B // 2, self.Hq, S, k.shape[1], self.hd, True)
+        o, lse = ops.attn_fwd(q, k, vt, m.kmask, True, self.scale, need_lse=save, nsplit=ns)
         o2 = o.view(T, self.Nq)
-        h, t2 = self._lora_fwd(o2, L.Wo, L.lora["o"], m.lora_on, res=x, drop=self._drop(m, li, "o"))
+        h, t2 = self._lora_fwd(o2, L.Wo, L.lora["o"], m.lora_on, res=x, drop=self._drop(m, li, "o"), rows=lr)
         hn = ops.rmsnorm_fwd(h, L.ln2, self.eps)
         gu = t3 = act = None
         if not save and FUSE_SWIGLU:
             G3, d3 = L.lora["gu"], self._drop(m, li, "gu")
-            if G3 is not None and m.lora_on:
+            if G3 is not None and m.lora_on and lr is not None:
+                t3 = self._down_rows(hn, G3, d3, lr)
+                act = ops.gemm_swiglu(hn, L.Wgu, a2=t3, b2=G3.B, a2_rows=lr)
+            elif G3 is not None and m.lora_on:
                 t3 = ops.lora_down_drop(hn, G3.A, G3.scaling, d3[0], d3[1], d3[2]) if d3 is not None else self._down(hn, G3.A, G3.scaling, len(G3.n_sizes) * G3.r)
                 act = ops.gemm_swiglu(hn, L.Wgu, a2=t3, b2=G3.B)
             else:
                 act = ops.gemm_swiglu(hn, L.Wgu)
         if act is None:
             if t3 is not None:
-                gu = ops.gemm_nt(hn, L.Wgu, a2=t3, b2=L.lora["gu"].B)
+                gu = ops.gemm_nt(hn, L.Wgu, a2=t3, b2=L.lora["gu"].B, a2_rows=lr)
             else:
-                gu, t3 = self._lora_fwd(hn, L.Wgu, L.lora["gu"], m.lora_on, drop=self._drop(m, li, "gu"))
+                gu, t3 = self._lora_fwd(hn, L.Wgu, L.lora["gu"], m.lora_on, drop=self._drop(m, li, "gu"), rows=lr)
             act = ops.swiglu_fwd(gu)
-        y, t4 = self._lora_fwd(act, L.Wd, L.lora["d"], m.lora_on, res=h, drop=self._drop(m, li, "d"))
+        y, t4 = self._lora_fwd(act, L.Wd, L.lora["d"], m.lora_on, res=h, drop=self._drop(m, li, "d"), rows=lr)
         saved = (x, xn, t1, qkv, q, k, v, o, lse, t2, h, hn, t3, gu, act, t4) if save else None
+        if save and lr is not None:
+            nb = B // 2
+            assert lr == nb * S
+            rowwise = lambda t_: None if t_ is None else t_[:lr]
+            seqwise = lambda t_: None if t_ is None else t_[:nb]
+            saved = (x[:lr], xn[:lr], rowwise(t1), qkv[:lr], q[:nb], k[:nb], v[:nb], o[:nb], seqwise(lse), rowwise(t2), h[:lr], hn[:lr],
+                     rowwise(t3), gu[:lr], act[:lr], rowwise(t4))
         return y, saved
 
     def layer_bwd(self, li: int, dy: torch.Tensor, saved, m: SeqMeta, prefix: int = 0, extra_dkv=None):
@@ -336,9 +363,18 @@
         return dx
 
 
-    def forward_hidden_shared(self, xp: torch.Tensor, mp: SeqMeta, xc: torch.Tensor, mc: SeqMeta, copies: int, save: bool, side=None):
+    def forward_hidden_shared(self, xp: torch.Tensor, mp: SeqMeta, xc: torch.Tensor, mc: SeqMeta, copies: int, save: bool, side=None,
+                              with_ref: bool = False):
         R, P, B, C = mp.B, mp.S, mc.B, mc.S
         assert B == R * copies
+        if with_ref:
+            assert mp.lora_on and mc.lora_on and mp.lora_rows is None, "the reference half is the pass WITHOUT the adapters the policy half has"
+            import dataclasses
+            xp, xc = torch.cat([xp, xp.detach()], dim=0), torch.cat([xc, xc], dim=0)
+            two = lambda t_: None if t_ is None else torch.cat([t_, t_], dim=0)
+            mp = dataclasses.replace(mp, B=2 * R, pos=two(mp.pos), kmask=two(mp.kmask), lora_rows=R * P)
+            mc = dataclasses.replace(mc, B=2 * B, pos=two(mc.pos), kmask=two(mc.kmask), lora_rows=B * C)
+            R, B = 2 * R, 2 * B
         dev = xp.device
         tape_p, tape_c = [], []
         main = torch.cuda.current_stream(dev) if side is not None else None
@@ -373,6 +409,10 @@
             main.wait_stream(side)
             for t_ in (hid_c, xc):
                 t_.record_stream(main)
+        if with_ref:
+            R, B = R // 2, B // 2
+            tape = (tape_p, tape_c, xp_last[:R], xc[:B * C], last[:R]) if save else None
+            return hid_last[:R], hid_c[:B * C], tape, (hid_last[R:].detach(), hid_c[B * C:].detach())
         return hid_last, hid_c, ((tape_p, tape_c, xp_last, xc, last) if save else None)
 
     def backward_hidden_shared(self, dhid_last: torch.Tensor, dhid_c: torch.Tensor, tape, mp: SeqMeta, mc: SeqMeta, copies: int, side=None):
diff --git a/bioreason_amd/grpo.py b/bioreason_amd/grpo.py
--- a/bioreason_amd/grpo.py
+++ b/bioreason_amd/grpo.py
@@ -64,7 +64,8 @@
 
 
 def per_token_logps_shared_policy(model, prompt_ids: torch.Tensor, prompt_mask: torch.Tensor, completion_ids: torch.Tensor,
-                                  completion_mask_: torch.Tensor, prompt_alias: Sequence[int], side=None, **multimodal) -> Optional[torch.Tensor]:
+                                  completion_mask_: torch.Tensor, prompt_alias: Sequence[int], side=None, with_ref: bool = False,
+                                  **multimodal):
     from .generation import _uniform_groups
     grp = _uniform_groups(list(prompt_alias))
     if grp is None or grp[1] < 2:
@@ -77,13 +78,19 @@
     sel = torch.arange(R, device=dev) * copies
     embeds = model._inputs_embeds(prompt_ids, multimodal.get("dna_tokenized"), multimodal.get("batch_idx_map"),
                                   multimodal.get("dna_alias"), multimodal.get("dna_enc"))
-    hid_last, hid_c = tm.hidden_states_shared(embeds.index_select(0, sel), prompt_mask.index_select(0, sel), completion_ids,
-                                              completion_mask_, copies, side=side)
-    from .modeling import _ExpandGroupsFn, _LogProbFn
+    out = tm.hidden_states_shared(embeds.index_select(0, sel), prompt_mask.index_select(0, sel), completion_ids,
+                                  completion_mask_, copies, side=side, with_ref=with_ref)
+    hid_last, hid_c = out[0], out[1]
+    from .modeling import _ExpandGroupsFn, _LogProbFn, _LogProbWithRefFn
     H = hid_c.shape[-1]
     first = _ExpandGroupsFn.apply(hid_last, copies)
     hsel = torch.cat([first[:, None, :], hid_c.view(B, C, H)[:, : C - 1, :]], dim=1).reshape(B * C, H).contiguous()
     tgt = completion_ids.to(torch.int32).reshape(-1).contiguous()
+    if with_ref:
+        first_r = out[2].repeat_interleave(copies, dim=0)
+        hsel_r = torch.cat([first_r[:, None, :], out[3].view(B, C, H)[:, : C - 1, :]], dim=1).reshape(B * C, H)
+        lp, ref = _LogProbWithRefFn.apply(hsel, hsel_r, tm, tgt)
+        return lp.view(B, C), ref.detach().view(B, C)
     return _LogProbFn.apply(hsel, tm, tgt).view(B, C)
 
 
diff --git a/bioreason_amd/modeling.py b/bioreason_amd/modeling.py
--- a/bioreason_amd/modeling.py
+++ b/bioreason_amd/modeling.py
@@ -123,20 +123,24 @@
 class _SharedStackFn(torch.autograd.Function):
 
     @staticmethod
-    def forward(ctx, xp, xc, anchor, model, mp, mc, copies, side, grad_mode=True):
+    def forward(ctx, xp, xc, anchor, model, mp, mc, copies, side, grad_mode=True, with_ref=False):
         eng = model.engine
         need = bool(grad_mode and (ctx.needs_input_grad[0] or ctx.needs_input_grad[2]))
-        hid_last, hid_c, tape = eng.forward_hidden_shared(xp, mp, xc, mc, copies, save=need, side=side)
-        ctx.model, ctx.mp, ctx.mc, ctx.copies, ctx.tape, ctx.side = model, mp, mc, copies, tape, side
+        ctx.model, ctx.mp, ctx.mc, ctx.copies, ctx.side = model, mp, mc, copies, side
+        if with_ref:
+            hid_last, hid_c, ctx.tape, (ref_last, ref_c) = eng.forward_hidden_shared(xp, mp, xc, mc, copies, save=need, side=side, with_ref=True)
+            ctx.mark_non_differentiable(ref_last, ref_c)
+            return hid_last, hid_c, ref_last, ref_c
+        hid_last, hid_c, ctx.tape = eng.forward_hidden_shared(xp, mp, xc, mc, copies, save=need, side=side)
         return hid_last, hid_c
 
     @staticmethod
-    def backward(ctx, dlast, dc):
+    def backward(ctx, dlast, dc, *_ref):
         eng = ctx.model.engine
         eng.ensure_transposed()
         dxp, dxc = eng.backward_hidden_shared(dlast.contiguous(), dc.contiguous(), ctx.tape, ctx.mp, ctx.mc, ctx.copies, side=ctx.side)
         ctx.tape = None
-        return dxp, None, None, None, None, None, None, None, None
+        return dxp, None, None, None, None, None, None, None, None, None
 
 
 class _ExpandGroupsFn(torch.autograd.Function):
@@ -169,6 +173,29 @@
         dlogits = ops.lmhead_dlogits(h, eng.E, tgt, lse, dlogp.contiguous().float())
         dh = ops.gemm_nt(dlogits, eng.ET[:, :eng.V] if eng.ET.shape[1] != eng.V else eng.ET)
         return dh, None, None
+
+
+class _LogProbWithRefFn(torch.autograd.Function):
+
+    @staticmethod
+    def forward(ctx, h, h_ref, model, tgt):
+        eng = model.engine
+        n = h.shape[0]
+        logp, lse = ops.lmhead_logprob(torch.cat([h, h_ref], dim=0), eng.E, torch.cat([tgt, tgt]))
+        ctx.save_for_backward(h, tgt, lse[:n])
+        ctx.model = model
+        ref = logp[n:]
+        ctx.mark_non_differentiable(ref)
+        return logp[:n], ref
+
+    @staticmethod
+    def backward(ctx, dlogp, _dref):
+        h, tgt, lse = ctx.saved_tensors
+        eng = ctx.model.engine
+        eng.ensure_transposed()
+        dlogits = ops.lmhead_dlogits(h, eng.E, tgt, lse.contiguous(), dlogp.contiguous().float())
+        dh = ops.gemm_nt(dlogits, eng.ET[:, :eng.V] if eng.ET.shape[1] != eng.V else eng.ET)
+        return dh, None, None, None
 
 
 class _LogitsFn(torch.autograd.Function):
@@ -409,7 +436,8 @@
         return _StackFn.apply(x.contiguous(), anchor, self, meta, torch.is_grad_enabled())
 
     def hidden_states_shared(self, prompt_embeds: torch.Tensor, prompt_mask: torch.Tensor, completion_ids: torch.Tensor,
-                             completion_mask: torch.Tensor, copies: int, side=None):
+                             completion_mask: torch.Tensor, copies: int, side=None, with_ref: bool = False):
+        assert not with_ref or self._lora_enabled
         eng = self.ensure_packed()
         if self.arena is not None:
             self.arena.pack_if_stale()
@@ -436,7 +464,7 @@
         xc = torch.empty((B * C, H), dtype=BF16, device=dev)
         ops.embed_scatter_fwd(completion_ids.to(torch.int32).reshape(-1).contiguous(), None, eng.E, None, xc)
         anchor = self.arena.anchor if self.arena is not None else xp.new_zeros(1, dtype=torch.float32)
-        return _SharedStackFn.apply(xp.contiguous(), xc, anchor, self, mp, mc, copies, side, torch.is_grad_enabled())
+        return _SharedStackFn.apply(xp.contiguous(), xc, anchor, self, mp, mc, copies, side, torch.is_grad_enabled(), with_ref)
 
     def forward(self, input_ids=None, attention_mask=None, inputs_embeds=None, labels=None, position_ids=None,
                 return_logits: bool = True, **unused):
diff --git a/bioreason_amd/ops.py b/bioreason_amd/ops.py
--- a/bioreason_amd/ops.py
+++ b/bioreason_amd/ops.py
@@ -36,6 +36,7 @@
     alpha: float = 1.0,
     out_f32: bool = False,
     accumulate: bool = False,
+    a2_rows: Optional[int] = None,
 ) -> torch.Tensor:
     a = _as2d(a)
     M, K = a.shape
@@ -58,11 +59,17 @@
     if timed:
         e0 = torch.cuda.Event(enable_timing=True)
         e0.record()
-    get_lib().call(
-        "bra_gemm_bf16_nt", a, _ld(a), b, _ld(b), a2, _ld(a2) if a2 is not None else 0, b2,
-        _ld(b2) if b2 is not None else 0, K2, out, _ld(out), M, N, K, alpha, bias, res,
-        _ld(res) if res is not None else 0, int(out_f32), int(accumulate), current_stream(a),
-    )
+    if a2_rows is not None and a2 is not None:
+        get_lib().call(
+            "bra_gemm_bf16_nt_rows", a, _ld(a), b, _ld(b), a2, _ld(a2), b2, _ld(b2), K2, out, _ld(out), M, N, K, alpha, bias, res,
+            _ld(res) if res is not None else 0, int(out_f32), int(accumulate), int(a2_rows), current_stream(a),
+        )
+    else:
+        get_lib().call(
+            "bra_gemm_bf16_nt", a, _ld(a), b, _ld(b), a2, _ld(a2) if a2 is not None else 0, b2,
+            _ld(b2) if b2 is not None else 0, K2, out, _ld(out), M, N, K, alpha, bias, res,
+            _ld(res) if res is not None else 0, int(out_f32), int(accumulate), current_stream(a),
+        )
     if timed:
         e1 = torch.cuda.Event(enable_timing=True)
         e1.record()
@@ -163,13 +170,17 @@
 LORA_DOWN_SPLITK = os.environ.get("BRA_LORA_SPLITK", "1") != "0"
 
 
-def lora_down_drop(x: torch.Tensor, A: torch.Tensor, alpha: float, p: float, seeds, rank: int = 32) -> torch.Tensor:
+def lora_down_drop(x: torch.Tensor, A: torch.Tensor, alpha: float, p: float, seeds, rank: int = 32, live_m: Optional[int] = None) -> torch.Tensor:
     M, K = x.shape
     R = A.shape[0]
     t = torch.empty((M, R), dtype=BF16, device=x.device)
     lib = get_lib()
-    ks = int(lib._dll.bra_lora_down_splitk_plan(int(M), int(K))) if LORA_DOWN_SPLITK else 1
+    ks = int(lib._dll.bra_lora_down_splitk_plan(int(live_m) if live_m else int(M), int(K))) if LORA_DOWN_SPLITK else 1
     part = torch.empty((ks, M, R), dtype=torch.float32, device=x.device) if ks > 1 else None
+    if live_m is not None:
+        lib.call("bra_lora_down_drop_rows", x, _ld(x), A, _ld(A), t, _ld(t), M, K, R, alpha, p, *_group(seeds, rank, R), part, ks,
+                 int(live_m), current_stream(x))
+        return t
     lib.call("bra_lora_down_drop", x, _ld(x), A, _ld(A), t, _ld(t), M, K, R, alpha, p, *_group(seeds, rank, R), part, ks,
              current_stream(x))
     return t
@@ -232,13 +243,18 @@
     return y.view(x.shape)
 
 
-def gemm_swiglu(x: torch.Tensor, W: torch.Tensor, a2: Optional[torch.Tensor] = None, b2: Optional[torch.Tensor] = None) -> Optional[torch.Tensor]:
+def gemm_swiglu(x: torch.Tensor, W: torch.Tensor, a2: Optional[torch.Tensor] = None, b2: Optional[torch.Tensor] = None,
+                a2_rows: Optional[int] = None) -> Optional[torch.Tensor]:
     M, K = x.shape
     F = W.shape[0] // 2
     K2 = a2.shape[1] if a2 is not None else 0
     if M <= 16 or K % 64 or K2 % 64 or F % 128 or W.shape[0] != 2 * F:
         return None
     act = torch.empty((M, F), dtype=BF16, device=x.device)
+    if a2_rows is not None and a2 is not None:
+        rc = get_lib().call_rc("bra_gemm_swiglu_bf16_nt_rows", x, _ld(x), W, _ld(W), a2, _ld(a2), b2, _ld(b2), K2, act, _ld(act), M, F, K,
+                               1.0, int(a2_rows), current_stream(x))
+        return None if rc != 0 else act
     rc = get_lib().call_rc("bra_gemm_swiglu_bf16_nt", x, _ld(x), W, _ld(W), a2, _ld(a2) if a2 is not None else 0, b2,
                            _ld(b2) if b2 is not None else 0, K2, act, _ld(act), M, F, K, 1.0, current_stream(x))
     return None if rc != 0 else act
diff --git a/bioreason_amd/trainer.py b/bioreason_amd/trainer.py
--- a/bioreason_amd/trainer.py
+++ b/bioreason_amd/trainer.py
@@ -45,6 +45,7 @@
     share_policy_prompt: Optional[bool] = None
     overlap_ref_pass: bool = True
     overlap_policy_chains: bool = True
+    ref_in_policy_pass: bool = False
     overlap_ref_chains: bool = False
     overlap_rollout_weights: bool = True
 
@@ -229,12 +230,13 @@
             self._side[which] = torch.cuda.Stream(device=dev)
         return self._side[which]
 
-    def generate_and_score(self, batch: Dict, timing: bool = False, mark=lambda n: None, defer_ref_join: bool = False) -> Dict:
+    def generate_and_score(self, batch: Dict, timing: bool = False, mark=lambda n: None, defer_ref_join: bool = False,
+                           ref_in_policy_pass: bool = False) -> Dict:
         tm = self.model.text_model
         had, prev = hasattr(tm, "rollout_fp8"), getattr(tm, "rollout_fp8", False)
         tm.rollout_fp8 = bool(prev) or bool(self.cfg.rollout_fp8)
         try:
-            return self._generate_and_score(batch, timing, mark, defer_ref_join)
+            return self._generate_and_score(batch, timing, mark, defer_ref_join, ref_in_policy_pass)
         finally:
             if had:
                 tm.rollout_fp8 = prev
@@ -244,7 +246,8 @@
                 except AttributeError:
                     pass
 
-    def _generate_and_score(self, batch: Dict, timing: bool = False, mark=lambda n: None, defer_ref_join: bool = False) -> Dict:
+    def _generate_and_score(self, batch: Dict, timing: bool = False, mark=lambda n: None, defer_ref_join: bool = False,
+                            ref_in_policy_pass: bool = False) -> Dict:
         m, c = self.model, self.cfg
         dev = batch["input_ids"].device
         mm = {"dna_tokenized": batch["dna_tokenized"], "batch_idx_map": batch["batch_idx_map"], "dna_alias": batch.get("dna_alias")}
@@ -283,7 +286,8 @@
                 old_lp = grpo.per_token_logps(m, prompt_ids, prompt_mask, completion_ids, cmask, **mm).detach()
         ref_lp = None
         ref_join = None
-        if c.beta != 0.0:
+        ref_merged = bool(ref_in_policy_pass and self._ref_rides_in_policy_pass(batch, timing))
+        if c.beta != 0.0 and not ref_merged:
             def ref_pass():
                 eng_ = m.text_model.ensure_packed()
                 w8 = None
@@ -327,8 +331,20 @@
             ref_join = None
         return {"prompt_ids": prompt_ids, "prompt_mask": prompt_mask, "completion_ids": completion_ids, "completion_mask": cmask,
                 "old_per_token_logps": old_lp, "ref_per_token_logps": ref_lp, "advantages": adv, "multimodal_inputs": mm,
-                "prompt_alias": batch.get("prompt_alias"), "ref_join": ref_join,
+                "prompt_alias": batch.get("prompt_alias"), "ref_join": ref_join, "ref_in_policy_pass": ref_merged,
                 "rewards_per_func": all_rewards.mean(0), "roll_metrics": roll_metrics}
+
+    def _ref_rides_in_policy_pass(self, batch: Dict, timing: bool) -> bool:
+        c = self.cfg
+        if not c.ref_in_policy_pass or timing or c.beta == 0.0 or c.ref_fp8:
+            return False
+        if not self.shares_policy_prompt() or batch.get("prompt_alias") is None:
+            return False
+        if not getattr(self.model.text_model, "_lora_enabled", False) or getattr(self.model.text_model, "arena", None) is None:
+            return False
+        from .generation import _uniform_groups
+        grp = _uniform_groups(list(batch["prompt_alias"]))
+        return grp is not None and grp[1] >= 2
 
     def shares_policy_prompt(self) -> bool:
         want = self.cfg.share_policy_prompt
@@ -341,9 +357,13 @@
         lp = None
         if self.shares_policy_prompt() and inputs.get("prompt_alias") is not None:
             side2 = self._side_stream(inputs["prompt_ids"].device, 1) if c.overlap_policy_chains else None
+            with_ref = bool(inputs.get("ref_in_policy_pass")) and inputs.get("ref_per_token_logps") is None
             lp = grpo.per_token_logps_shared_policy(m, inputs["prompt_ids"], inputs["prompt_mask"], inputs["completion_ids"],
-                                                    inputs["completion_mask"], inputs["prompt_alias"], side=side2,
+                                                    inputs["completion_mask"], inputs["prompt_alias"], side=side2, with_ref=with_ref,
                                                     **inputs["multimodal_inputs"])
+            if with_ref:
+                assert lp is not None
+                lp, inputs["ref_per_token_logps"] = lp
         if lp is None:
             lp = grpo.per_token_logps(m, inputs["prompt_ids"], inputs["prompt_mask"], inputs["completion_ids"],
                                       inputs["completion_mask"], **inputs["multimodal_inputs"])
@@ -366,7 +386,7 @@
         slot = self._step % ga
         mark("start")
         if self.global_step % c.num_iterations == 0:
-            inputs = self.generate_and_score(batch, timing, mark, defer_ref_join=True)
+            inputs = self.generate_and_score(batch, timing, mark, defer_ref_join=True, ref_in_policy_pass=True)
             self._buffered_inputs[slot] = inputs
         else:
             inputs = self._buffered_inputs[slot]
@@ -381,7 +401,8 @@
             m.arena.grad(METRIC_SLOT).view(-1)[:3].add_(stats / ga)
         (loss / ga if ga > 1 else loss).backward()
         mark("policy_bwd")
-        out = {"loss_t": loss.detach(), "stats_t": stats, "reward_mean_t": inputs["roll_metrics"][1]}
+        out = {"loss_t": loss.detach(), "stats_t": stats, "reward_mean_t": inputs["roll_metrics"][1],
+               "ref_in_policy_pass": bool(inputs.get("ref_in_policy_pass"))}
         if slot == ga - 1:
             scale = self.reduce_gradients()
             if self.dp:
diff --git a/include/bioreason_hip.h b/include/bioreason_hip.h
--- a/include/bioreason_hip.h
+++ b/include/bioreason_hip.h
@@ -10,6 +10,9 @@
 int bra_gemm_bf16_nt(const void* A, long lda, const void* B, long ldb, const void* A2, long lda2, const void* B2,
                      long ldb2, int K2, void* C, long ldc, int M, int N, int K, float alpha, const void* bias,
                      const void* res, long ldres, int out_f32, int accumulate, void* stream);
+int bra_gemm_bf16_nt_rows(const void* A, long lda, const void* B, long ldb, const void* A2, long lda2, const void* B2,
+                          long ldb2, int K2, void* C, long ldc, int M, int N, int K, float alpha, const void* bias,
+                          const void* res, long ldres, int out_f32, int accumulate, int a2_rows, void* stream);
 
 int bra_gemm_bf16_nt_splitk(const void* A, long lda, const void* B, long ldb, void* C, long ldc, int M, int N, int K,
                             float alpha, int split_k, void* stream);
@@ -21,6 +24,9 @@
 int bra_lora_down_drop(const void* x, long ldx, const void* A, long lda, void* t, long ldt, int M, int K, int R, float alpha,
                        float p, unsigned s0, unsigned s1, unsigned s2, unsigned s3, int r, int nt, float* part, int ksplit,
                        void* stream);
+int bra_lora_down_drop_rows(const void* x, long ldx, const void* A, long lda, void* t, long ldt, int M, int K, int R, float alpha,
+                            float p, unsigned s0, unsigned s1, unsigned s2, unsigned s3, int r, int nt, float* part, int ksplit,
+                            int live_m, void* stream);
 int bra_lora_up_drop(const void* dts, long ldd, const void* AT, long ldat, void* out, long ldo, int M, int K, int R, float p,
                      unsigned s0, unsigned s1, unsigned s2, unsigned s3, int r, int nt, void* stream);
 int bra_wgrad_tn_drop(const void* Y, long ldy, const void* T, long ldt, float* C, long c_sn, long c_sr, int M, int N, int R,
@@ -115,6 +121,8 @@
 int bra_dec_gemm2_fp8_anyk_ok(int N, int K);
 int bra_gemm_swiglu_bf16_nt(const void* A, long lda, const void* W, long ldw, const void* A2, long lda2, const void* B2, long ldb2, int K2,
                             void* C, long ldc, int M, int F, int K, float alpha, void* stream);
+int bra_gemm_swiglu_bf16_nt_rows(const void* A, long lda, const void* W, long ldw, const void* A2, long lda2, const void* B2, long ldb2,
+                                 int K2, void* C, long ldc, int M, int F, int K, float alpha, int a2_rows, void* stream);
 int bra_quant_rows_fp8(const void* x, long ldx, int M, int K, const void* colw, void* q, long ldq, float* scale, int rms, float eps,
                        void* stream);
 int bra_swiglu_quant_fp8(const void* gu, long ldgu, int M, int F, void* q, long ldq, float* scale, void* stream);
```
